# tobiashepp/torch-mednet

Hardware: AMD Instinct MI355X
Metric: 128^3 patches/sec training, 3D U-Net 32-base-ch (higher is better)
Workload: dtype bf16; 1 GPU; ResidualUNet3D f_maps=[32, 64, 128, 256] 4-class, 128^3 patches, batch 4/GPU, fwd+DiceLoss+bwd+allreduce+Adam (BASELINE config 2); global_batch=4, parallelism=dp1, graph_replay=False, gradient_exchange=none (1 rank)

## Files before the change

### include/mednet_hip.h

```cpp
#ifndef MEDNET_HIP_H
#define MEDNET_HIP_H
#include <stddef.h>
#include <stdint.h>
#ifdef __cplusplus
extern "C" {
#endif

typedef void* mednet_stream;

enum { MEDNET_F32 = 0, MEDNET_BF16 = 1,
       MEDNET_F16 = 2,
       MEDNET_U8 = 3,
       MEDNET_I64 = 4   };
enum { MEDNET_NDHWC = 0, MEDNET_NCDHW = 1 };
enum { MEDNET_ACT_NONE = 0, MEDNET_ACT_RELU = 1, MEDNET_ACT_LEAKY = 2, MEDNET_ACT_ELU = 3 };
enum { MEDNET_POOL_MAX = 0, MEDNET_POOL_AVG = 1 };
enum { MEDNET_ALGO_AUTO = 0, MEDNET_ALGO_DIRECT = 1, MEDNET_ALGO_MFMA = 2, MEDNET_ALGO_EXACT = 3,
       MEDNET_ALGO_EXACT_BIT = 4,
       MEDNET_ALGO_SPLITW_BIT = 8 };
enum { MEDNET_PACK_LOW = 0x100,
       MEDNET_PACK_HIGH_ONLY = 0x200 };
enum { MEDNET_REG_L2 = 0, MEDNET_REG_L1 = 1 };
enum { MEDNET_CLASS_DICE = 0, MEDNET_CLASS_CE = 1 };
enum {
// ... 23 lines not shown
int mednet_conv3d_pack_many(const void* table_device, int njobs, unsigned blocks, int elt_dtype, mednet_stream stream);
int mednet_conv3d_stats_plan(int n, int d, int h, int w, int cin, int cout, int dtype, int gnb, int stride, int* out13);
int mednet_conv3d_fused_stats_chunks(int n, int d, int h, int w, int cin, int cout, int ksize, int x_dtype,
                                     int y_dtype, int algo);
int mednet_conv3d_fwd(const void* x, const void* packed, const float* bias, void* y, int n, int d, int h, int w,
                      int cin, int cout, int ksize, int x_dtype, int x_layout, int y_dtype, int y_layout,
                      int dgrad, int algo, float* gn_partial, mednet_stream stream);
int mednet_conv3d_cm_supported(int cin, int cout, int ksize, int x_dtype, int y_dtype, int algo);
int mednet_conv3d_act_supported(int n, int d, int h, int w, int cin, int cout, int algo);
int mednet_conv3d_act_fwd(const void* x, const void* packed, void* y, int n, int d, int h, int w, int cin, int cout,
                          int act, int algo, float* gn_partial, int dtype, mednet_stream stream);
int mednet_conv3d_dgrad_add(const void* dy, const void* packed, const void* add, void* dx, int n, int d, int h, int w,
                            int cin, int cout, int algo, int dtype, mednet_stream stream);
int mednet_conv3d_dgrad_gn_rows(int n, int d, int h, int w, int cin, int cout, int algo);
int mednet_conv3d_dgrad_gn_rows_dt(int n, int d, int h, int w, int cin, int cout, int algo, int dtype);
int mednet_conv3d_dgrad_add_supported(int n, int d, int h, int w, int cin, int cout, int algo, int dtype);
int mednet_conv3d_dgrad_gn(const void* dy, const void* packed, const void* add, void* dx, const void* gn_y,
                           const float* gn_coef, int gn_act, float* gn_partial, int n, int d, int h, int w, int cin,
                           int cout, int algo, int dtype, mednet_stream stream);
int mednet_head_dgrad_gn_rows(int n, int d, int h, int w, int cin, int dtype);
int mednet_head_dgrad_gn(const void* dy, const void* packed, void* dx, const void* gn_y, const void* gn_z, int gn_act,
                         float* gn_partial, int n, int d, int h, int w, int cin, int cout, int dtype, mednet_stream stream);
int mednet_convt3d_dgrad_gn_rows(int n, int d, int h, int w, int cin, int cout, int dtype, int algo);
int mednet_convt3d_dgrad_gn(const void* dy, const void* packed, void* dx, const void* gn_y, const void* gn_z, int gn_act,
                            float* gn_partial, int n, int d, int h, int w, int cin, int cout, int dtype, int algo,
                            mednet_stream stream);
int mednet_pool2_bwd_gn_rows(int n, int d, int h, int w, int c, int dtype);
int mednet_pool2_bwd_gn(const void* dy, const void* x, const void* add, void* dx, const void* gn_y, int gn_act,
                        float* gn_partial, int n, int d, int h, int w, int c, int mode, int dtype, mednet_stream stream);
size_t mednet_conv3d_wgrad_ws_bytes(int n, int d, int h, int w, int cin, int cout, int ksize, int workgroups);
int mednet_conv3d_wgrad_coresident(int n, int d, int h, int w, int cin, int cout, int ksize, int x_dtype, int dy_dtype, int algo);
int mednet_conv3d_wgrad_plan(int n, int d, int h, int w, int cin, int cout, int dtype, int workgroups, int* out10);
int mednet_conv3d_wgrad_c1_gn_supported(int cout, int x_dtype, int dtype);
int mednet_conv3d_wgrad_c1_gn(const void* x, const void* dz, const void* y, const float* coef, const float* bcoef, float* dw,
                              int n, int d, int h, int w, int cout, int act, int x_dtype, int dtype, void* ws, size_t ws_bytes,
                              mednet_stream stream);
int mednet_conv3d_wgrad_cm_gn_supported(int cin, int cout, int x_dtype, int dtype);
int mednet_conv3d_wgrad_cm_plan(int n, int d, int h, int w, int cin, int cout, int dtype, int gn, int* out4);
int mednet_conv3d_wgrad_cm_gn(const void* x, int x_layout, const void* dz, const void* y, const float* coef, const float* bcoef,
                              float* dw, int n, int d, int h, int w, int cin, int cout, int act, int x_dtype, int dtype, void* ws,
                              size_t ws_bytes, mednet_stream stream);
int mednet_conv3d_wgrad(const void* x, const void* dy, float* dw, float* dbias, int n, int d, int h, int w,
                        int cin, int cout, int ksize, int x_dtype, int x_layout, int dy_dtype, int dy_layout,
                        int algo, int workgroups, void* ws, size_t ws_bytes, mednet_stream stream);

int mednet_convt3d_fwd(const void* x, const void* packed, const float* bias, const void* skip, void* y, int n,
                       int d, int h, int w, int cin, int cout, int x_dtype, int y_dtype, int algo,
                       mednet_stream stream);
int mednet_convt3d_dgrad(const void* dy, const void* packed, void* dx, int n, int d, int h, int w, int cin,
                         int cout, int dy_dtype, int dx_dtype, int algo, mednet_stream stream);
size_t mednet_convt3d_wgrad_ws_bytes(int n, int d, int h, int w, int cin, int cout, int workgroups);
int mednet_convt3d_wgrad(const void* x, const void* dy, float* dw, float* dbias, int n, int d, int h, int w,
                         int cin, int cout, int x_dtype, int dy_dtype, int algo, int workgroups, void* ws,
                         size_t ws_bytes, mednet_stream stream);

size_t mednet_gn_ws_bytes(int n, int c, size_t spatial);
int mednet_gn_stats(const void* x, const float* gamma, const float* beta, float* stats, float* coef, int n,
                    size_t spatial, int c, int groups, float eps, int dtype, void* ws, size_t ws_bytes,
                    mednet_stream stream);
int mednet_gn_finalize(const float* partial, int chunks, const float* gamma, const float* beta, float* stats,
                       float* coef, int n, size_t spatial, int c, int groups, float eps, void* ws, size_t ws_bytes,
                       mednet_stream stream);
int mednet_gn_act_fwd(const void* x, const float* coef, const void* residual, void* z, int n, size_t spatial,
                      int c, int act, int x_dtype, int z_dtype, mednet_stream stream);
int mednet_gn_act_bwd(const void* dz, const void* dz2, const void* x, const void* z, const float* coef,
                      const float* stats, const float* gamma, void* dx, void* dres, float* dgamma, float* dbeta, int n,
                      size_t spatial, int c, int groups, int act, int in_act, int dtype, void* ws, size_t ws_bytes,
                      mednet_stream stream);
int mednet_gn_act_bwd_fused(const void* dz, const void* x, const float* coef, const float* stats, const float* gamma,
                            const float* partial, int rows, void* dx, float* dgamma, float* dbeta, int n,
                            size_t spatial, int c, int groups, int act, int in_act, int dtype, void* ws, size_t ws_bytes,
                            mednet_stream stream);
int mednet_gn_bwd_coefficients(const float* stats, const float* gamma, const float* partial, int rows, float* bcoef,
                               float* dgamma, float* dbeta, int n, size_t spatial, int c, int groups, void* ws,
                               size_t ws_bytes, mednet_stream stream);
int mednet_gn_act_bwd_fused_res(const void* dz, const void* x, const void* z, const float* coef, const float* stats,
                                const float* gamma, const float* fused_partial, int rows, void* dx, void* dres,
                                float* dgamma, float* dbeta, int n, size_t spatial, int c, int groups, int act, int dtype,
                                void* ws, size_t ws_bytes, mednet_stream stream);
int mednet_gn_act_bwd_fused_res_pool(const void* dy_pool, const void* skip_grad, const void* x, const void* z, const float* stats,
                                     const float* gamma, const float* fused_partial, int rows, void* dx, void* dres, float* dgamma,
                                     float* dbeta, int n, int d, int h, int w, int c, int groups, int act, int pool_mode, int dtype,
                                     void* ws, size_t ws_bytes, mednet_stream stream);
int mednet_bn_stats(const void* x, const float* gamma, const float* beta, float* running_mean, float* running_var,
                    long long* num_batches_tracked, float momentum, float* stats, float* coef, int n, size_t spatial, int c,
                    float eps, int dtype, void* ws, size_t ws_bytes, mednet_stream stream);
int mednet_bn_eval_coef(const float* running_mean, const float* running_var, const float* gamma, const float* beta, float* stats,
                        float* coef, int n, int c, float eps, mednet_stream stream);
int mednet_bn_act_bwd(const void* dz, const void* x, const void* z, const float* coef, const float* stats, const float* gamma,
                      void* dx, void* dres, float* dgamma, float* dbeta, int n, size_t spatial, int c, int act, int in_act,
                      int frozen, int dtype, void* ws, size_t ws_bytes, mednet_stream stream);
int mednet_bn_act_bwd_fused(const void* dz, const void* x, const float* coef, const float* stats, const float* gamma,
                            const float* partial, int rows, void* dx, float* dgamma, float* dbeta, int n, size_t spatial, int c,
                            int act, int in_act, int frozen, int dtype, void* ws, size_t ws_bytes, mednet_stream stream);

int mednet_act_fwd(const void* x, void* z, size_t count, int act, int dtype, mednet_stream stream);
int mednet_act_bwd(const void* dz, const void* z, void* dx, size_t count, int act, int dtype,
                   mednet_stream stream);
int mednet_add(const void* a, const void* b, void* out, size_t count, int dtype, mednet_stream stream);

int mednet_pool2_fwd(const void* x, void* y, int n, int d, int h, int w, int c, int mode, int dtype,
                     mednet_stream stream);
int mednet_gn_act_pool_supported(int d, int h, int w, int c, int dtype);
int mednet_gn_act_pool_fwd(const void* x, const float* coef, const void* residual, void* z, void* pooled, int n, int d, int h,
                           int w, int c, int act, int mode, int dtype, mednet_stream stream);
int mednet_pool2_bwd(const void* dy, const void* x, const void* add, void* dx, int n, int d, int h, int w, int c,
                     int mode, int dtype, mednet_stream stream);
int mednet_pool2_bwd_act(const void* dy, const void* x, const void* add, int add_channels, void* dx, int n, int d, int h, int w, int c,
                         int mode, int in_act, int dtype, mednet_stream stream);

int mednet_upcat_fwd(const void* enc, const void* x, void* out, int n, int d, int h, int w, int c_enc, int xd,
                     int xh, int xw, int c_x, int dtype, mednet_stream stream);
int mednet_upcat_stats_chunks(int n, int d, int h, int w, int c_enc, int c_x, int dtype);
int mednet_upcat_fwd_stats(const void* enc, const void* x, void* out, float* partial, int n, int d, int h, int w, int c_enc, int xd,
                           int xh, int xw, int c_x, int dtype, mednet_stream stream);
int mednet_upcat_bwd(const void* dout, void* denc, void* dx, int n, int d, int h, int w, int c_enc, int xd, int xh,
                     int xw, int c_x, int dtype, mednet_stream stream);

size_t mednet_loss_ws_bytes(int n, int c, size_t spatial);
int mednet_dice_fwd(const float* logits, const int64_t* labels, const float* weight, float* loss, float* saved,
                    float* dice_out, int n, int c, size_t spatial, int64_t stride_n, int64_t stride_c, float eps,
                    int sigmoid, int ignore_index, void* ws, size_t ws_bytes, mednet_stream stream);
int mednet_dice_bwd(const float* logits, const int64_t* labels, const float* weight, const float* saved,
                    const float* dloss, float* dlogits, int n, int c, size_t spatial, int64_t stride_n,
                    int64_t stride_c, float eps, int sigmoid, int ignore_index, mednet_stream stream);
int mednet_dice_fwd_lt(const float* logits, const void* labels, int label_dtype, int64_t label_stride_n, const float* weight,
                       float* loss, float* saved, float* dice_out, int n, int c, size_t spatial, int64_t stride_n,
                       int64_t stride_c, float eps, int sigmoid, int ignore_index, void* ws, size_t ws_bytes, mednet_stream stream);
int mednet_dice_bwd_lt(const float* logits, const void* labels, int label_dtype, int64_t label_stride_n, const float* weight,
                       const float* saved, const float* dloss, float* dlogits, int n, int c, size_t spatial, int64_t stride_n,
                       int64_t stride_c, float eps, int sigmoid, int ignore_index, mednet_stream stream);
int mednet_head_dice_supported(int cin, int cout, int dtype, int label_dtype);
size_t mednet_head_dice_ws_bytes(int n, size_t spatial, int cin, int cout);
int mednet_head_dice_gn_rows(int n, size_t spatial, int cin);
int mednet_head_dice_fwd(const void* z, const void* packed, const float* bias, const void* labels, int label_dtype,
                         int64_t label_stride_n, const float* weight, float* logits, float* loss, float* saved, int n,
                         size_t spatial, int cin, int cout, float eps, int sigmoid, int ignore_index, int z_dtype, void* ws,
                         size_t ws_bytes, mednet_stream stream);
int mednet_head_dice_bwd(const float* logits, const void* labels, int label_dtype, int64_t label_stride_n, const void* packed,
                         const float* weight, const float* saved, const float* dloss, void* dz, const void* gn_y, const void* z,
                         int gn_act, float* gn_partial, float* dw, float* dbias, int n, size_t spatial, int cin, int cout,
                         float eps, int sigmoid, int ignore_index, int z_dtype, void* ws, size_t ws_bytes, mednet_stream stream);

int mednet_head_landmark_supported(int cin, int nh, int ncls, int dtype, size_t spatial);
size_t mednet_head_landmark_ws_bytes(int n, size_t spatial, int nh, int ncls);
int mednet_head_landmark_gn_rows(size_t spatial);
int mednet_head_landmark_fwd(const void* z, const void* packed, const float* bias, const void* heatmaps, int64_t heatmap_stride_n,
                             const void* labels, int64_t label_stride_n, const float* class_weight, const float* reg_weight,
                             float* logits, float* class_loss, float* reg_loss, float* saved, int n, size_t spatial, int cin, int nh,
                             int ncls, int kind, float eps, int sigmoid, int ignore_index, int z_dtype, void* ws, size_t ws_bytes,
                             mednet_stream stream);
int mednet_head_landmark_bwd(const void* z, const void* packed, const float* bias, const void* heatmaps, int64_t heatmap_stride_n,
                             const void* labels, int64_t label_stride_n, const float* class_weight, const float* reg_weight,
                             const float* saved, const float* dclass_loss, const float* dreg_loss, void* dz, const void* gn_y,
                             int gn_act, float* gn_partial, float* dw, float* dbias, int n, size_t spatial, int cin, int nh, int ncls,
                             int kind, float eps, int sigmoid, int ignore_index, int z_dtype, void* ws, size_t ws_bytes,
                             mednet_stream stream);
int mednet_head_ce_supported(int cin, int cout, int dtype, int label_dtype);
size_t mednet_head_ce_ws_bytes(int n, size_t spatial, int cin, int cout);
int mednet_head_ce_gn_rows(int n, size_t spatial, int cin);
int mednet_head_ce_fwd(const void* z, const void* packed, const float* bias, const void* labels, int label_dtype,
                       int64_t label_stride_n, const float* weight, float* logits, float* loss, float* saved, int n, size_t spatial,
                       int cin, int cout, int ignore_index, int z_dtype, void* ws, size_t ws_bytes, mednet_stream stream);
int mednet_head_ce_bwd(const float* logits, const void* labels, int label_dtype, int64_t label_stride_n, const void* packed,
                       const float* weight, const float* saved, const float* dloss, void* dz, const void* gn_y, const void* z,
                       int gn_act, float* gn_partial, float* dw, float* dbias, int n, size_t spatial, int cin, int cout,
// ... 63 lines not shown
```

### torch-mednet_amd/csrc/conv.h

```cpp
#pragma once
#include "common.h"

namespace mednet {

enum { MAP_CONV = 0, MAP_CT_FWD = 1, MAP_CT_DG = 2 };

struct ConvGeom {
  int n, od, oh, ow;
  int id, ih, iw;
  int k, m;
  int ks;
  int in_planar, out_planar;
};

struct WgradGeom {
  int n, ad, ah, aw;
  int bd, bh, bw;
  int ka, kb, ks, stride2;
  int a_planar, b_planar;
  size_t chunk;
};


template <int MAP>
int launch_direct(const void* x, const float* P, const float* bias, const void* skip, void* y, const ConvGeom& g,
                  int x_dtype, int y_dtype, hipStream_t s);
size_t wgrad_direct_ws_bytes(size_t nvox, int ka, int kb, int ks);
int launch_wgrad_direct(const void* A, const void* B, float* dw, WgradGeom g, int a_dtype, int b_dtype, void* ws,
                        size_t ws_bytes, hipStream_t s);
size_t channel_sum_ws_bytes(int n, size_t spatial, int c);
int launch_channel_sum(const void* x, float* out, int n, size_t spatial, int c, int planar, int dtype, void* ws,
                       size_t ws_bytes, hipStream_t s);
bool head_dgrad_supported(int cin, int cout, int ksize, int x_dtype, int x_layout, int y_layout);
int launch_head_dgrad(const void* dy, const float* Pb, void* dz, int n, size_t spatial, int m, int k, int out_dtype,
                      hipStream_t s);
int head_dgrad_gn_rows(size_t spatial, int k, int dtype);
int launch_head_dgrad_gn(const void* dy, const float* Pb, void* dz, const void* gy, const void* gz, int act, float* partial,
                         int n, size_t spatial, int m, int k, int dtype, hipStream_t s);
bool head_vox_supported(int k);
int launch_head_fwd_vox(const void* z, const float* Pb, const float* bias, float* y, int n, size_t spatial, int k, int m,
                        int z_dtype, hipStream_t s);
bool wgrad_1x1_supported(int cin, int cout, int ksize, int x_layout, int dy_layout, int dy_dtype);
size_t wgrad_1x1_ws_bytes(int n, size_t spatial, int cin, int cout);
int launch_wgrad_1x1(const void* z, const void* dy, float* dw, int n, size_t spatial, int cin, int cout, int z_dtype,
                     void* ws, size_t ws_bytes, hipStream_t s);
bool wgrad_c1_supported(int cin, int cout, int ksize, int x_layout, int dy_layout);
size_t wgrad_c1_ws_bytes(int n, int d, int h, int w, int cout);
bool wgrad_c1_gn_supported(int cout, int x_dtype, int dtype);
int launch_wgrad_c1_gn(const void* x, const void* dz, const void* y, const float* coef, const float* bcoef, int act, float* dw,
                       int n, int d, int h, int w, int cout, int x_dtype, int dtype, void* ws, size_t ws_bytes, hipStream_t s);
int launch_wgrad_c1(const void* x, const void* dy, float* dw, int n, int d, int h, int w, int cout, int x_dtype,
                    int dy_dtype, void* ws, size_t ws_bytes, hipStream_t s, bool split_bf16 = false);
bool wgrad_cm_supported(int cin, int cout, int ksize, int x_dtype, int dy_dtype, int dy_layout);
bool wgrad_cm_gn_supported(int cin, int cout, int x_dtype, int dtype);
size_t wgrad_cm_ws_bytes(int n, int d, int h, int w, int cin, int cout);
int wgrad_cm_plan(int n, int d, int h, int w, int cin, int cout, int dtype, bool gn, int* out4);
int launch_wgrad_cm(const void* x, int x_layout, const void* dz, const void* y, const float* coef, const float* bcoef, int act,
                    float* dw, int n, int d, int h, int w, int cin, int cout, int dtype, void* ws, size_t ws_bytes, hipStream_t s);
int launch_pack_f32(const float* w, float* Pf, float* Pb, int cin, int cout, int T, int transposed_src, hipStream_t s);

int launch_hm_finalize(const float* partial, const float* cweight, float* loss, int n, int c, int nblocks, size_t spatial,
                       hipStream_t s);
int launch_dice_finalize(const float* partial, const float* weight, float* loss, float* saved, int c, int nblocks, float eps,
                         hipStream_t s, float* dice_out = nullptr);
int launch_ce_finalize(const float* partial, float* loss, float* saved, int nblocks, hipStream_t s);

#include "conv_mfma_decl.inc"

bool conv_f32_mfma_enabled();
int launch_conv_f32_mfma(const void* x, const float* P, const float* bias, void* y, int n, int d, int h, int w, int k, int m,
                         hipStream_t s);
int launch_convt_dgrad_f32_mfma(const void* dy, const float* Pb, void* dx, int n, int d, int h, int w, int cin, int cout,
                                hipStream_t s);
int launch_convt_fwd_f32_mfma(const void* x, const float* Pf, const float* bias, const void* skip, void* y, int n, int d, int h,
                              int w, int cin, int cout, hipStream_t s);
size_t wgrad_f32_mfma_ws_bytes(int n, int d, int h, int w, int ka, int kb, int stride2);
int launch_wgrad_f32_mfma(const void* x, const void* dy, float* dw, int n, int d, int h, int w, int cin, int cout, void* ws,
                          size_t ws_bytes, hipStream_t s);
int launch_convt_wgrad_f32_mfma(const void* x, const void* dy, float* dw, int n, int d, int h, int w, int cin, int cout, void* ws,
                                size_t ws_bytes, hipStream_t s);

bool conv_x3_enabled();
bool conv_x3_supported(int cin, int cout, int ksize);
bool conv_x3_fits(int d, int h, int w, int c);
int conv_x3_stats_rows(int n, int d, int h, int w, int cout);
int launch_conv_x3(const void* x, const void* sec_hi, size_t lo_delta, const float* bias, void* y, int n, int d, int h, int w, int k,
                   int m, float* stats, hipStream_t s);
bool conv_c1_x3_supported(int cin, int cout, int ksize);
int conv_c1_x3_stats_rows(int d, int h, int w);
int launch_conv_c1_x3(const void* x, const float* w_pf, const float* bias, void* y, int n, int d, int h, int w, int cout,
                      float* stats, hipStream_t s);
int launch_conv_x3_dgrad(const void* dy, const void* sec_hi, size_t lo_delta, void* dx, int n, int d, int h, int w, int k, int m,
                         const void* add, const void* gn_y, const float* gn_coef, int gn_act, float* gn_partial, hipStream_t s);
int launch_convt_dgrad_x3(const void* dy, const void* sec_hi, size_t lo_delta, void* dx, int n, int d, int h, int w, int cin,
                          int cout, hipStream_t s);
int launch_convt_fwd_x3(const void* x, const void* sec_hi, size_t lo_delta, const float* bias, const void* skip, void* y, int n,
                        int d, int h, int w, int cin, int cout, hipStream_t s);
size_t wgrad_x3_ws_bytes(int n, int d, int h, int w, int cin, int cout, int workgroups);
bool wgrad_c1_x3_supported(int cout, int x_dtype, int dy_dtype);
int wgrad_c1_x3_blocks(int n, int d, int h, int w);
int launch_wgrad_c1_x3(const void* x, const void* dy, float* part, int n, int d, int h, int w, hipStream_t s);
int launch_wgrad_x3(const void* x, const void* dy, float* dw, int n, int d, int h, int w, int cin, int cout, void* ws,
                    size_t ws_bytes, hipStream_t s, int workgroups);

size_t convt_wgrad_x3_ws_bytes(int n, int d, int h, int w, int cin, int cout, int workgroups);
int launch_convt_wgrad_x3(const void* x, const void* dy, float* dw, int n, int d, int h, int w, int cin, int cout, void* ws,
                          size_t ws_bytes, hipStream_t s, int workgroups);

}
```

### torch-mednet_amd/csrc/head_loss.hip

```cpp
#include "common.h"
#include "conv.h"

namespace mednet {

constexpr int HL_BLOCK_VOX = 256 * 8;
constexpr int HL_MAXC = 4;
constexpr int HL_VPT = 32;

template <typename T>
struct Raw8;
template <>
struct Raw8<bf16> {
  bf16x8 r;
  __device__ __forceinline__ void load(const bf16* p, size_t i) { r = *reinterpret_cast<const bf16x8*>(p + i); }
  __device__ __forceinline__ float at(int j) const { return (float)r[j]; }
};
template <>
struct Raw8<f16> {
  f16x8 r;
  __device__ __forceinline__ void load(const f16* p, size_t i) { r = *reinterpret_cast<const f16x8*>(p + i); }
  __device__ __forceinline__ float at(int j) const { return (float)r[j]; }
};
template <>
struct Raw8<float> {
// ... 51 lines not shown
  const size_t v0 = (size_t)blockIdx.x * HL_BLOCK_VOX;
  for (int it = 0; it < 8; ++it) {
    const size_t v = v0 + (size_t)it * 256 + threadIdx.x;
    if (v < spatial) {
      float zv[K];
#pragma unroll
      for (int q = 0; q < K / 8; ++q) {
        const F8 t = ld8(z, ((size_t)n * spatial + v) * K + q * 8);
#pragma unroll
        for (int j = 0; j < 8; ++j) zv[q * 8 + j] = t.v[j];
      }
      const int yl = label_at(lab, (size_t)n * lab_sn + v);
      float lg[HL_MAXC], p[HL_MAXC];
#pragma unroll
      for (int i = 0; i < HL_MAXC; ++i) {
        lg[i] = 0.f;
        if (i < m) {
          float s0 = bias ? bias[i] : 0.f, s1 = 0.f;
#pragma unroll
          for (int j = 0; j < K; j += 2) {
            s0 = fmaf(zv[j], Pb[(size_t)i * K + j], s0);
            s1 = fmaf(zv[j + 1], Pb[(size_t)i * K + j + 1], s1);
          }
          lg[i] = s0 + s1;
          y[((size_t)n * m + i) * spatial + v] = lg[i];
        }
      }
      if constexpr (CE) {
        if (yl != ignore && (unsigned)yl >= (unsigned)m) num = __builtin_nanf("");
        if (yl != ignore && yl >= 0 && yl < m) {
          float mx = -INFINITY, zy = 0.f;
#pragma unroll
          for (int k = 0; k < HL_MAXC; ++k)
            if (k < m) {
              mx = fmaxf(mx, lg[k]);
              if (k == yl) zy = lg[k];
            }
          float s = 0.f;
#pragma unroll
          for (int k = 0; k < HL_MAXC; ++k)
            if (k < m) s += expf(lg[k] - mx);
          const float w = cw ? cw[yl] : 1.f;
          num = fmaf(w, (mx + logf(s)) - zy, num);
          den += w;
        }
        continue;
      }
      probs_reg(lg, m, sigmoid, p);
      bad |= (unsigned)yl >= (unsigned)m;
#pragma unroll
      for (int k = 0; k < HL_MAXC; ++k)
        if (k < m) {
          const float t = (k == yl) ? 1.f : 0.f;
          const float mk = (ignore != MEDNET_NO_IGNORE && t == (float)ignore) ? 0.f : 1.f;
          I[k] = fmaf(p[k] * mk, t * mk, I[k]);
          D[k] += (p[k] + t) * mk;
        }
    }
  }
  if constexpr (CE) {
    num = block_sum<4>(num, scratch);
    den = block_sum<4>(den, scratch);
    if (threadIdx.x == 0) {
      float* o = partial + ((size_t)n * gridDim.x + blockIdx.x) * 2;
      o[0] = num;
      o[1] = den;
    }
    return;
  }
  if (bad) I[0] = D[0] = __builtin_nanf("");
  float* out = partial + ((size_t)n * gridDim.x + blockIdx.x) * m * 2;
#pragma unroll
  for (int k = 0; k < HL_MAXC; ++k)
    if (k < m) {
      const float a = block_sum<4>(I[k], scratch);
      const float b = block_sum<4>(D[k], scratch);
      if (threadIdx.x == 0) {
        out[2 * k] = a;
        out[2 * k + 1] = b;
      }
    }
}

template <typename TO, int K, typename TL, bool FOLD = false, bool CE = false>
__global__ __launch_bounds__(256, (sizeof(TO) == 2 && !FOLD) ? 3 : 2) void head_dice_bwd_kernel(const float* __restrict__ lgs, const TL* __restrict__ lab, int64_t lab_sn,
                                                            const float* __restrict__ Pb , const float* __restrict__ weight,
                                                            const float* __restrict__ saved, const float* __restrict__ dloss,
                                                            float eps, int sigmoid, int ignore, TO* __restrict__ dz,
                                                            const TO* __restrict__ gy , const TO* __restrict__ gz, int act,
                                                            float* __restrict__ gn_partial , float* __restrict__ wpart,
                                                            size_t spatial, int m) {
  constexpr int CG = K / 8, VPW = 256 / CG;
  const int n = blockIdx.y;
  const int cgi = threadIdx.x % CG, vi = threadIdx.x / CG;
  float wreg[HL_MAXC][8];
#pragma unroll
  for (int i = 0; i < HL_MAXC; ++i)
#pragma unroll
    for (int j = 0; j < 8; ++j) wreg[i][j] = i < m ? Pb[(size_t)i * K + cgi * 8 + j] : 0.f;
  const float go = *dloss;
  float gI[HL_MAXC], gD[HL_MAXC];
#pragma unroll
  for (int k = 0; k < HL_MAXC; ++k) {
    gI[k] = gD[k] = 0.f;
    if (CE && k < m) {
      gI[k] = (weight ? weight[k] : 1.f) * (go / saved[0]);
    } else if (k < m) {
      const float w = weight ? weight[k] : 1.f;
      const float I = saved[2 * k], D = saved[2 * k + 1];
      const float Dc = fmaxf(D, eps);
      gI[k] = -2.f * w / ((float)m * Dc) * go + ((I != I || D != D) ? __builtin_nanf("") : 0.f);
      gD[k] = (D >= eps ? 2.f * w * I / ((float)m * Dc * Dc) : 0.f) * go;
    }
  }
  auto dlogits_of = [&](const float* lg, int yl, float* dl) {
    if constexpr (CE) {
      float p[HL_MAXC];
      probs_reg(lg, m, 0, p);
      float w = 0.f;
#pragma unroll
      for (int k = 0; k < HL_MAXC; ++k)
        if (k < m && k == yl) w = gI[k];
      w = (yl != ignore && yl >= 0 && yl < m) ? w : 0.f;
#pragma unroll
      for (int k = 0; k < HL_MAXC; ++k) dl[k] = k < m ? w * (p[k] - (k == yl ? 1.f : 0.f)) : 0.f;
      return;
    }
    float p[HL_MAXC], g[HL_MAXC];
    probs_reg(lg, m, sigmoid, p);
    float dot = 0.f;
#pragma unroll
    for (int k = 0; k < HL_MAXC; ++k)
      if (k < m) {
        const float t = (k == yl) ? 1.f : 0.f;
        const float mk = (ignore != MEDNET_NO_IGNORE && t == (float)ignore) ? 0.f : 1.f;
        g[k] = mk * (gI[k] * t * mk + gD[k]);
        dot = fmaf(p[k], g[k], dot);
      }
#pragma unroll
    for (int k = 0; k < HL_MAXC; ++k) dl[k] = k < m ? (sigmoid ? g[k] * p[k] * (1.f - p[k]) : p[k] * (g[k] - dot)) : 0.f;
  };
  float ss[8], sq[8], wacc[HL_MAXC][8], bacc[HL_MAXC];
#pragma unroll
  for (int j = 0; j < 8; ++j) ss[j] = sq[j] = 0.f;
#pragma unroll
  for (int i = 0; i < HL_MAXC; ++i) {
    bacc[i] = 0.f;
#pragma unroll
    for (int j = 0; j < 8; ++j) wacc[i][j] = 0.f;
  }
  const size_t v0 = (size_t)blockIdx.x * (VPW * HL_VPT) + vi;
  for (int it = 0; it < HL_VPT; it += 2) {
    const size_t v = v0 + (size_t)it * VPW;
    if (v >= spatial) break;
    const size_t vb = v + VPW;
    const bool hb = (it + 1 < HL_VPT) && vb < spatial;
    const size_t vbs = hb ? vb : v;
    float la[HL_MAXC], lb[HL_MAXC];
    if constexpr (CG == 4) {
      const int cq = threadIdx.x & 3;
      const float oa = cq < m ? lgs[((size_t)n * m + cq) * spatial + v] : 0.f;
      const float ob = cq < m ? lgs[((size_t)n * m + cq) * spatial + vbs] : 0.f;
      la[0] = dpp_f32<(0) | (0 << 2) | (0 << 4) | (0 << 6)>(oa);
      la[1] = dpp_f32<(1) | (1 << 2) | (1 << 4) | (1 << 6)>(oa);
      la[2] = dpp_f32<(2) | (2 << 2) | (2 << 4) | (2 << 6)>(oa);
      la[3] = dpp_f32<(3) | (3 << 2) | (3 << 4) | (3 << 6)>(oa);
      lb[0] = dpp_f32<(0) | (0 << 2) | (0 << 4) | (0 << 6)>(ob);
      lb[1] = dpp_f32<(1) | (1 << 2) | (1 << 4) | (1 << 6)>(ob);
      lb[2] = dpp_f32<(2) | (2 << 2) | (2 << 4) | (2 << 6)>(ob);
      lb[3] = dpp_f32<(3) | (3 << 2) | (3 << 4) | (3 << 6)>(ob);
      static_assert(HL_MAXC == 4, "one class per lane of a quad");
    } else {
#pragma unroll
      for (int i = 0; i < HL_MAXC; ++i) {
        la[i] = i < m ? lgs[((size_t)n * m + i) * spatial + v] : 0.f;
        lb[i] = i < m ? lgs[((size_t)n * m + i) * spatial + vbs] : 0.f;
      }
    }
    const int ya = label_at(lab, (size_t)n * lab_sn + v), yb = label_at(lab, (size_t)n * lab_sn + vbs);
    const size_t rowa = ((size_t)n * spatial + v) * K + cgi * 8, rowb = ((size_t)n * spatial + vbs) * K + cgi * 8;
    Raw8<TO> zva, zvb, yva, yvb;
    zva.load(gz, rowa);
    zvb.load(gz, rowb);
    if (gy) {
      yva.load(gy, rowa);
      yvb.load(gy, rowb);
    } else {
      yva = zva;
      yvb = zvb;
    }
    float da[HL_MAXC], db[HL_MAXC];
    dlogits_of(la, ya, da);
    dlogits_of(lb, yb, db);
    if (!hb) {
#pragma unroll
      for (int i = 0; i < HL_MAXC; ++i) db[i] = 0.f;
    }
    F8 t, u;
#pragma unroll
    for (int j = 0; j < 8; ++j) t.v[j] = u.v[j] = 0.f;
#pragma unroll
    for (int i = 0; i < HL_MAXC; ++i) {
      if (i < m) {
#pragma unroll
        for (int j = 0; j < 8; ++j) {
          t.v[j] = fmaf(da[i], wreg[i][j], t.v[j]);
          u.v[j] = fmaf(db[i], wreg[i][j], u.v[j]);
          wacc[i][j] = fmaf(db[i], zvb.at(j), fmaf(da[i], zva.at(j), wacc[i][j]));
        }
        bacc[i] += da[i] + db[i];
      }
    }
#pragma unroll
    for (int j = 0; j < 8; ++j) {
      t.v[j] = (float)(TO)t.v[j];
      u.v[j] = (float)(TO)u.v[j];
    }
    if constexpr (FOLD) {
      float za[8], zb[8];
#pragma unroll
      for (int j = 0; j < 8; ++j) {
        za[j] = zva.at(j);
        zb[j] = zvb.at(j);
      }
      act_grad_n<8>(t.v, za, act);
      act_grad_n<8>(u.v, zb, act);
    }
    st8(dz, rowa, t);
    if (hb) st8(dz, rowb, u);
    if (!FOLD && gy) {
      float za[8], zb[8];
#pragma unroll
      for (int j = 0; j < 8; ++j) {
        za[j] = zva.at(j);
        zb[j] = zvb.at(j);
      }
      act_grad_n<8>(t.v, za, act);
      act_grad_n<8>(u.v, zb, act);
#pragma unroll
      for (int j = 0; j < 8; ++j) {
        ss[j] += t.v[j] + u.v[j];
        sq[j] = fmaf(u.v[j], yvb.at(j), fmaf(t.v[j], yva.at(j), sq[j]));
      }
    }
  }
  const int lane = threadIdx.x & 63, wave = threadIdx.x >> 6;
  const size_t wrow = ((size_t)n * gridDim.x + blockIdx.x) * 4 + wave;
  if (gn_partial) {
    float* out = gn_partial + wrow * K * 2 + cgi * 16;
#pragma unroll
    for (int j = 0; j < 8; ++j) {
      const float a = lane_class_sum<CG>(ss[j]), b = lane_class_sum<CG>(sq[j]);
      if (lane < CG) {
        out[2 * j] = a;
        out[2 * j + 1] = b;
      }
    }
  }
  float* wout = wpart + wrow * ((size_t)m * K + m);
#pragma unroll
  for (int i = 0; i < HL_MAXC; ++i) {
    if (i < m) {
#pragma unroll
      for (int j = 0; j < 8; ++j) {
        const float a = lane_class_sum<CG>(wacc[i][j]);
        if (lane < CG) wout[(size_t)i * K + cgi * 8 + j] = a;
      }
      const float b = lane_class_sum<CG>(bacc[i]);
      if (lane == 0) wout[(size_t)m * K + i] = b;
    }
  }
}

constexpr int HL_WF_GROUPS = 128;
__global__ __launch_bounds__(192) void head_dice_wfinal1_kernel(const float* __restrict__ wpart, double* __restrict__ part2, int rows,
                                                                int width) {
  const int per = (rows + HL_WF_GROUPS - 1) / HL_WF_GROUPS;
  const int r0 = blockIdx.x * per, r1 = r0 + per < rows ? r0 + per : rows;
  for (int e = threadIdx.x; e < width; e += 192) {
    double s0 = 0.0, s1 = 0.0, s2 = 0.0, s3 = 0.0;
    int r = r0;
    for (; r + 3 < r1; r += 4) {
      s0 += (double)wpart[(size_t)r * width + e];
      s1 += (double)wpart[(size_t)(r + 1) * width + e];
      s2 += (double)wpart[(size_t)(r + 2) * width + e];
      s3 += (double)wpart[(size_t)(r + 3) * width + e];
    }
    for (; r < r1; ++r) s0 += (double)wpart[(size_t)r * width + e];
    part2[(size_t)blockIdx.x * width + e] = (s0 + s1) + (s2 + s3);
  }
}
__global__ __launch_bounds__(192) void head_dice_wfinal2_kernel(const double* __restrict__ part2, float* __restrict__ dw,
                                                                float* __restrict__ dbias, int width, int mk) {
  for (int e = threadIdx.x; e < width; e += 192) {
    double s = 0.0;
    for (int g = 0; g < HL_WF_GROUPS; ++g) s += part2[(size_t)g * width + e];
    if (e < mk) dw[e] = (float)s;
    else if (dbias) dbias[e - mk] = (float)s;
  }
}

__global__ void dice_finalize_kernel(const float* __restrict__ partial, const float* __restrict__ weight, float* __restrict__ loss,
                                     float* __restrict__ saved, float* __restrict__ dice_out, int c, int nblocks, float eps);

static inline unsigned hl_fwd_blocks(size_t spatial) { return (unsigned)((spatial + HL_BLOCK_VOX - 1) / HL_BLOCK_VOX); }
static inline unsigned hl_bwd_blocks(size_t spatial, int k) {
  const size_t per_wg = (size_t)(256 / (k / 8)) * HL_VPT;
  return (unsigned)((spatial + per_wg - 1) / per_wg);
}

}

using namespace mednet;

extern "C" int mednet_head_dice_supported(int cin, int cout, int dtype, int label_dtype) {
  return (cin == 16 || cin == 32 || cin == 64) && cout >= 1 && cout <= HL_MAXC && dtype_ok(dtype) &&
         (label_dtype == MEDNET_U8 || label_dtype == MEDNET_I64) && tuning_option("head_loss_fuse", 1);
}
extern "C" size_t mednet_head_dice_ws_bytes(int n, size_t spatial, int cin, int cout) {
  const size_t fwd = ((size_t)n * hl_fwd_blocks(spatial) * cout * 2 + 64) * sizeof(float);
  const size_t width = (size_t)cout * cin + cout;
  const size_t bwd = ((size_t)n * hl_bwd_blocks(spatial, cin) * 4 * width + 64) * sizeof(float) + (size_t)HL_WF_GROUPS * width * sizeof(double) + 16;
  return fwd > bwd ? fwd : bwd;
}
extern "C" int mednet_head_dice_gn_rows(int n, size_t spatial, int cin) {
  (void)n;
  return 4 * (int)hl_bwd_blocks(spatial, cin);
}

template <bool CE>
static int head_loss_fwd(const char* what, const void* z, const void* packed, const float* bias, const void* labels, int label_dtype,
                         int64_t label_stride_n, const float* weight, float* logits, float* loss, float* saved, int n, size_t spatial,
                         int cin, int cout, float eps, int sigmoid, int ignore_index, int z_dtype, void* ws, size_t ws_bytes,
                         mednet_stream stream) {
  MEDNET_REQUIRE(mednet_head_dice_supported(cin, cout, z_dtype, label_dtype), MEDNET_E_UNSUPPORTED,
                 "%s: %d -> %d classes, dtype %d, labels %d", what, cin, cout, z_dtype, label_dtype);
  MEDNET_REQUIRE(n > 0 && spatial > 0 && z && packed && labels && logits && loss && saved, MEDNET_E_SHAPE, "%s: bad arguments", what);
  MEDNET_REQUIRE(ws_bytes >= mednet_head_dice_ws_bytes(n, spatial, cin, cout), MEDNET_E_WORKSPACE, "%s: workspace too small", what);
  const PackLayout L = pack_layout(cin, cout, 1);
  const float* Pb = (const float*)((const char*)packed + L.f32_bwd);
  hipStream_t s = (hipStream_t)stream;
  const unsigned nb = hl_fwd_blocks(spatial);
  float* partial = (float*)ws;
  const dim3 grid(nb, n);
#define HF(TI_, K_, TL_) hipLaunchKernelGGL((head_dice_fwd_kernel<TI_, K_, TL_, CE>), grid, dim3(256), 0, s, (const TI_*)z, Pb, bias, (const TL_*)labels, label_stride_n, logits, partial, spatial, cout, sigmoid, ignore_index, CE ? weight : nullptr)
#define HF_L(TI_, K_) do { if (label_dtype == MEDNET_U8) HF(TI_, K_, uint8_t); else HF(TI_, K_, int64_t); } while (0)
#define HF_K(TI_) do { if (cin == 16) HF_L(TI_, 16); else if (cin == 32) HF_L(TI_, 32); else HF_L(TI_, 64); } while (0)
  if (z_dtype == MEDNET_F32) HF_K(float);
  else if (z_dtype == MEDNET_BF16) HF_K(bf16);
  else HF_K(f16);
#undef HF_K
#undef HF_L
#undef HF
  int rc = check_launch(what);
  if (rc) return rc;
  if (CE) return launch_ce_finalize(partial, loss, saved, (int)(nb * n), s);
  hipLaunchKernelGGL(dice_finalize_kernel, dim3(1), dim3(256), 0, s, partial, weight, loss, saved, (float*)nullptr, cout, (int)(nb * n), eps);
  return check_launch("dice_finalize");
}

template <bool CE>
static int head_loss_bwd(const char* what, const float* logits, const void* labels, int label_dtype, int64_t label_stride_n,
                         const void* packed, const float* weight, const float* saved, const float* dloss, void* dz, const void* gn_y,
                         const void* z, int gn_act, float* gn_partial, float* dw, float* dbias, int n, size_t spatial, int cin, int cout,
                         float eps, int sigmoid, int ignore_index, int z_dtype, void* ws, size_t ws_bytes, mednet_stream stream) {
  MEDNET_REQUIRE(mednet_head_dice_supported(cin, cout, z_dtype, label_dtype), MEDNET_E_UNSUPPORTED,
                 "%s: %d -> %d classes, dtype %d, labels %d", what, cin, cout, z_dtype, label_dtype);
  MEDNET_REQUIRE(n > 0 && spatial > 0 && logits && labels && packed && saved && dloss && dz && z && dw, MEDNET_E_SHAPE, "%s: bad arguments", what);
  MEDNET_REQUIRE((gn_y == nullptr) == (gn_partial == nullptr), MEDNET_E_SHAPE, "%s: gn_y and gn_partial go together", what);
  MEDNET_REQUIRE(ws_bytes >= mednet_head_dice_ws_bytes(n, spatial, cin, cout), MEDNET_E_WORKSPACE, "%s: workspace too small", what);
  const PackLayout L = pack_layout(cin, cout, 1);
  const float* Pb = (const float*)((const char*)packed + L.f32_bwd);
  hipStream_t s = (hipStream_t)stream;
  const unsigned nb = hl_bwd_blocks(spatial, cin);
  float* wpart = (float*)ws;
  const dim3 grid(nb, n);
  const bool fold = gn_y == nullptr && gn_act != MEDNET_ACT_NONE;
#define HB_(TO_, K_, TL_, F_) hipLaunchKernelGGL((head_dice_bwd_kernel<TO_, K_, TL_, F_, CE>), grid, dim3(256), 0, s, logits, (const TL_*)labels, label_stride_n, Pb, weight, saved, dloss, eps, sigmoid, ignore_index, (TO_*)dz, (const TO_*)gn_y, (const TO_*)z, gn_act, gn_partial, wpart, spatial, cout)
#define HB(TO_, K_, TL_) do { if (fold) HB_(TO_, K_, TL_, true); else HB_(TO_, K_, TL_, false); } while (0)
#define HB_L(TO_, K_) do { if (label_dtype == MEDNET_U8) HB(TO_, K_, uint8_t); else HB(TO_, K_, int64_t); } while (0)
#define HB_K(TO_) do { if (cin == 16) HB_L(TO_, 16); else if (cin == 32) HB_L(TO_, 32); else HB_L(TO_, 64); } while (0)
  if (z_dtype == MEDNET_F32) HB_K(float);
  else if (z_dtype == MEDNET_BF16) HB_K(bf16);
  else HB_K(f16);
#undef HB_K
#undef HB_L
#undef HB_
#undef HB
  int rc = check_launch(what);
  if (rc) return rc;
  const int width = cout * cin + cout, rows = (int)(n * nb * 4);
  double* part2 = (double*)((char*)ws + (((size_t)rows * width + 64) * sizeof(float) + 7) / 8 * 8);
  hipLaunchKernelGGL(head_dice_wfinal1_kernel, dim3(HL_WF_GROUPS), dim3(192), 0, s, wpart, part2, rows, width);
  hipLaunchKernelGGL(head_dice_wfinal2_kernel, dim3(1), dim3(192), 0, s, part2, dw, dbias, width, cout * cin);
  return check_launch("head_dice_wfinal");
}

extern "C" int mednet_head_dice_fwd(const void* z, const void* packed, const float* bias, const void* labels, int label_dtype,
                                    int64_t label_stride_n, const float* weight, float* logits, float* loss, float* saved, int n,
                                    size_t spatial, int cin, int cout, float eps, int sigmoid, int ignore_index, int z_dtype,
                                    void* ws, size_t ws_bytes, mednet_stream stream) {
  return head_loss_fwd<false>("head_dice_fwd", z, packed, bias, labels, label_dtype, label_stride_n, weight, logits, loss, saved, n, spatial,
                              cin, cout, eps, sigmoid, ignore_index, z_dtype, ws, ws_bytes, stream);
}

extern "C" int mednet_head_dice_bwd(const float* logits, const void* labels, int label_dtype, int64_t label_stride_n,
                                    const void* packed, const float* weight, const float* saved, const float* dloss, void* dz,
                                    const void* gn_y, const void* z, int gn_act, float* gn_partial, float* dw, float* dbias, int n,
                                    size_t spatial, int cin, int cout, float eps, int sigmoid, int ignore_index, int z_dtype,
                                    void* ws, size_t ws_bytes, mednet_stream stream) {
  return head_loss_bwd<false>("head_dice_bwd", logits, labels, label_dtype, label_stride_n, packed, weight, saved, dloss, dz, gn_y, z, gn_act,
                              gn_partial, dw, dbias, n, spatial, cin, cout, eps, sigmoid, ignore_index, z_dtype, ws, ws_bytes, stream);
}

extern "C" int mednet_head_ce_supported(int cin, int cout, int dtype, int label_dtype) {
  return mednet_head_dice_supported(cin, cout, dtype, label_dtype);
}
extern "C" size_t mednet_head_ce_ws_bytes(int n, size_t spatial, int cin, int cout) {
  return mednet_head_dice_ws_bytes(n, spatial, cin, cout);
}
extern "C" int mednet_head_ce_gn_rows(int n, size_t spatial, int cin) { return mednet_head_dice_gn_rows(n, spatial, cin); }

extern "C" int mednet_head_ce_fwd(const void* z, const void* packed, const float* bias, const void* labels, int label_dtype,
                                  int64_t label_stride_n, const float* weight, float* logits, float* loss, float* saved, int n,
                                  size_t spatial, int cin, int cout, int ignore_index, int z_dtype, void* ws, size_t ws_bytes,
                                  mednet_stream stream) {
  return head_loss_fwd<true>("head_ce_fwd", z, packed, bias, labels, label_dtype, label_stride_n, weight, logits, loss, saved, n, spatial,
                             cin, cout, 0.f, 0, ignore_index, z_dtype, ws, ws_bytes, stream);
}

extern "C" int mednet_head_ce_bwd(const float* logits, const void* labels, int label_dtype, int64_t label_stride_n, const void* packed,
                                  const float* weight, const float* saved, const float* dloss, void* dz, const void* gn_y, const void* z,
                                  int gn_act, float* gn_partial, float* dw, float* dbias, int n, size_t spatial, int cin, int cout,
                                  int ignore_index, int z_dtype, void* ws, size_t ws_bytes, mednet_stream stream) {
  return head_loss_bwd<true>("head_ce_bwd", logits, labels, label_dtype, label_stride_n, packed, weight, saved, dloss, dz, gn_y, z, gn_act,
                             gn_partial, dw, dbias, n, spatial, cin, cout, 0.f, 0, ignore_index, z_dtype, ws, ws_bytes, stream);
}
```

### torch-mednet_amd/csrc/norm_act.hip

```cpp
#include "common.h"

#ifndef GN_NT
#define GN_NT 1
#endif
#ifndef GN_WAVES
#define GN_WAVES 3
#endif
namespace mednet {

template <int VEC>
struct Cols {
  int cols, rows, col, row;
  bool active;
  __device__ __forceinline__ Cols(int c) {
    cols = c / VEC;
    rows = 256 / cols;
    active = (int)threadIdx.x < rows * cols;
    col = threadIdx.x % cols;
    row = threadIdx.x / cols;
  }
};

template <typename T, int VEC>
struct VecIO;
template <typename T>
struct VecIO<T, 8> {
  static __device__ __forceinline__ F8 load(const T* p, size_t i) { return ld8(p, i); }
  static __device__ __forceinline__ F8 load_last(const T* p, size_t i) { return GN_NT ? ld8_nt(p, i) : ld8(p, i); }
  static __device__ __forceinline__ void store(T* p, size_t i, const F8& v) { st8(p, i, v); }
};
template <>
struct VecIO<float, 4> {
  static __device__ __forceinline__ F8 load(const float* p, size_t i) {
    F8 r;
    const f32x4 a = *reinterpret_cast<const f32x4*>(p + i);
#pragma unroll
    for (int k = 0; k < 4; ++k) r.v[k] = a[k];
    return r;
  }
  static __device__ __forceinline__ F8 load_last(const float* p, size_t i) {
    F8 r;
    const f32x4 a = GN_NT ? __builtin_nontemporal_load(reinterpret_cast<const f32x4*>(p + i)) : *reinterpret_cast<const f32x4*>(p + i);
#pragma unroll
    for (int k = 0; k < 4; ++k) r.v[k] = a[k];
    return r;
  }
  static __device__ __forceinline__ void store(float* p, size_t i, const F8& v) {
    const f32x4 a = {v.v[0], v.v[1], v.v[2], v.v[3]};
    *reinterpret_cast<f32x4*>(p + i) = a;
  }
};
template <typename T>
struct VecIO<T, 1> {
  static __device__ __forceinline__ F8 load(const T* p, size_t i) {
    F8 r;
    r.v[0] = ld(p, i);
    return r;
  }
  static __device__ __forceinline__ F8 load_last(const T* p, size_t i) { return load(p, i); }
  static __device__ __forceinline__ void store(T* p, size_t i, const F8& v) { st(p, i, v.v[0]); }
};

static inline void chunk_plan(size_t spatial, int c, int vec, size_t& chunk_vox, unsigned& chunks) {
  const int cols = c / vec;
  const int rows = 256 / cols;
  size_t cv = (spatial + 1023) / 1024;
  if (cv < (size_t)rows * 8) cv = (size_t)rows * 8;
  cv = (cv + rows - 1) / rows * rows;
  chunk_vox = cv;
  chunks = (unsigned)((spatial + cv - 1) / cv);
}

template <int NVAL>
__device__ __forceinline__ void column_reduce(const float* vals, int cols, int rows, int col, int row, bool active,
                                              float* lds, float* out) {
  __syncthreads();
  if (active) {
#pragma unroll
    for (int k = 0; k < NVAL; ++k) lds[(row * cols + col) * NVAL + k] = vals[k];
  }
  __syncthreads();
  if (active && row == 0) {
#pragma unroll
// ... 338 lines not shown
  const float k3 = (float)((rstd * rstd * s2 * mean - rstd * s1) / count);
  for (int i = threadIdx.x; i < cg; i += 64) {
    const int cc = g * cg + i;
    float* o = bcoef + ((size_t)n * c + cc) * 3;
    o[0] = (float)rstd * (gamma ? gamma[cc] : 1.f);
    o[1] = k2;
    o[2] = k3;
  }
}
template <bool DUX>
__global__ __launch_bounds__(256) void gn_bwd_reduce_finalize_kernel(const float* __restrict__ partial, const float* __restrict__ stats,
                                                                     const float* __restrict__ gamma, float* __restrict__ csum,
                                                                     float* __restrict__ bcoef, int c, int groups, int rows,
                                                                     double count) {
  __shared__ double sha[256], shb[256];
  const int n = blockIdx.x / groups, g = blockIdx.x % groups;
  const int cg = c / groups, t = threadIdx.x;
  const int i = t % cg, r0 = t / cg, rstep = 256 / cg;
  const float* base = partial + (size_t)n * rows * c * 2 + (size_t)(g * cg + i) * 2;
  const size_t rs = (size_t)c * 2;
  constexpr int U = 16;
  double a[U], b[U];
#pragma unroll
  for (int k = 0; k < U; ++k) a[k] = b[k] = 0.0;
  int r = r0;
  for (; r + (U - 1) * rstep < rows; r += U * rstep) {
    float2 p[U];
#pragma unroll
    for (int k = 0; k < U; ++k) p[k] = *reinterpret_cast<const float2*>(base + (size_t)(r + k * rstep) * rs);
#pragma unroll
    for (int k = 0; k < U; ++k) {
      a[k] += (double)p[k].x;
      b[k] += (double)p[k].y;
    }
  }
  for (; r < rows; r += rstep) {
    const float2 p0 = *reinterpret_cast<const float2*>(base + (size_t)r * rs);
    a[0] += (double)p0.x;
    b[0] += (double)p0.y;
  }
#pragma unroll
  for (int w = 1; w < U; w *= 2) {
#pragma unroll
    for (int k = 0; k < U; k += 2 * w) {
      a[k] += a[k + w];
      b[k] += b[k + w];
    }
  }
  sha[t] = a[0];
  shb[t] = b[0];
  __syncthreads();
  const double mean = stats[((size_t)n * groups + g) * 2], rstd = stats[((size_t)n * groups + g) * 2 + 1];
  if (t < cg) {
    double a = 0.0, b = 0.0;
    for (int k = 0; k < rstep; ++k) {
      a += sha[k * cg + t];
      b += shb[k * cg + t];
    }
    if (DUX) b = rstd * (b - mean * a);
    const float af = (float)a, bf = (float)b;
    csum[((size_t)n * c + g * cg + t) * 2] = af;
    csum[((size_t)n * c + g * cg + t) * 2 + 1] = bf;
    const double ga = gamma ? (double)gamma[g * cg + t] : 1.0;
    sha[t] = ga * (double)af;
    shb[t] = ga * (double)bf;
  }
  __syncthreads();
  if (t < cg) {
    double s1 = 0.0, s2 = 0.0;
    for (int k = 0; k < cg; ++k) {
      s1 += sha[k];
      s2 += shb[k];
    }
    float* o = bcoef + ((size_t)n * c + g * cg + t) * 3;
    o[0] = (float)rstd * (gamma ? gamma[g * cg + t] : 1.f);
    o[1] = (float)(-rstd * rstd * s2 / count);
    o[2] = (float)((rstd * rstd * s2 * mean - rstd * s1) / count);
  }
}
static bool gn_bwd_one_launch(int c, int groups) {
  const int cg = c / groups;
  return cg >= 1 && cg <= 256 && 256 % cg == 0 && tuning_option("gn_bwd_one_launch", 1);
}
struct GnParamGrad {
  const float* csum = nullptr;
  float* dgamma = nullptr;
  float* dbeta = nullptr;
  int n = 0;
};
__global__ __launch_bounds__(256) void gn_bwd_params_kernel(const float* __restrict__ csum, float* __restrict__ dgamma,
                                                            float* __restrict__ dbeta, int n, int c) {
  const int cc = blockIdx.x * 256 + threadIdx.x;
  if (cc >= c) return;
  double a = 0.0, b = 0.0;
  for (int i = 0; i < n; ++i) {
    a += (double)csum[((size_t)i * c + cc) * 2];
    b += (double)csum[((size_t)i * c + cc) * 2 + 1];
  }
  if (dbeta) dbeta[cc] = (float)a;
  if (dgamma) dgamma[cc] = (float)b;
}
template <typename T, int VEC>
__global__ __launch_bounds__(256, GN_WAVES) void gn_bwd_apply_kernel(const T* __restrict__ dz, const T* __restrict__ dz2,
                                                           const T* __restrict__ x, const T* __restrict__ z,
                                                           const float* __restrict__ coef,
                                                           const float* __restrict__ bcoef, T* __restrict__ dx,
                                                           T* __restrict__ dres, size_t spatial, int c, int act,
                                                           size_t chunk_vox, int in_act, GnParamGrad pg) {
  if (pg.csum && blockIdx.x == 0 && blockIdx.y == 0) {
    for (int cc = threadIdx.x; cc < c; cc += 256) {
      double a = 0.0, b = 0.0;
      for (int i = 0; i < pg.n; ++i) {
        a += (double)pg.csum[((size_t)i * c + cc) * 2];
        b += (double)pg.csum[((size_t)i * c + cc) * 2 + 1];
      }
      if (pg.dbeta) pg.dbeta[cc] = (float)a;
      if (pg.dgamma) pg.dgamma[cc] = (float)b;
    }
  }
  const Cols<VEC> L(c);
  if (!L.active) return;
  const int n = blockIdx.y;
  const size_t v0 = (size_t)blockIdx.x * chunk_vox;
  const size_t v1 = v0 + chunk_vox < spatial ? v0 + chunk_vox : spatial;
  float k1[VEC], k2[VEC], k3[VEC], ca[VEC], cb[VEC];
#pragma unroll
  for (int k = 0; k < VEC; ++k) {
    const float* o = bcoef + ((size_t)n * c + L.col * VEC + k) * 3;
    k1[k] = o[0];
    k2[k] = o[1];
    k3[k] = o[2];
    ca[k] = z ? 0.f : coef[((size_t)n * c + L.col * VEC + k) * 2];
    cb[k] = z ? 0.f : coef[((size_t)n * c + L.col * VEC + k) * 2 + 1];
  }
  const size_t off = (size_t)n * spatial * c + (size_t)L.col * VEC;
  auto one = [&](size_t i) {
    F8 g1 = VecIO<T, VEC>::load_last(dz, i);
    F8 g2, zv;
    if (dz2) g2 = VecIO<T, VEC>::load_last(dz2, i);
    if (act != MEDNET_ACT_NONE && z) zv = VecIO<T, VEC>::load(z, i);
    const F8 xv = VecIO<T, VEC>::load_last(x, i);
    if (dz2) {
#pragma unroll
      for (int k = 0; k < VEC; ++k) g1.v[k] += g2.v[k];
    }
    if (z) {
      act_grad_n<VEC>(g1.v, zv.v, act);
    } else {
#pragma unroll
      for (int k = 0; k < VEC; ++k) zv.v[k] = fmaf(ca[k], xv.v[k], cb[k]);
      act_grad_pre_n<VEC>(g1.v, zv.v, act);
    }
    F8 o;
#pragma unroll
    for (int k = 0; k < VEC; ++k) o.v[k] = fmaf(k1[k], g1.v[k], fmaf(k2[k], xv.v[k], k3[k]));
    if (in_act != MEDNET_ACT_NONE) act_grad_n<VEC>(o.v, xv.v, in_act);
    VecIO<T, VEC>::store(dx, i, o);
    if (dres) VecIO<T, VEC>::store(dres, i, g1);
  };
  size_t v = v0 + L.row;
  for (; v + (size_t)L.rows < v1; v += 2 * (size_t)L.rows) {
    one(off + v * c);
    one(off + (v + L.rows) * c);
  }
  for (; v < v1; v += L.rows) one(off + v * c);
}

template <typename T>
__global__ __launch_bounds__(256) void act_fwd_kernel(const T* __restrict__ x, T* __restrict__ z, size_t count, int act) {
  const size_t stride = (size_t)gridDim.x * 256 * 8;
  for (size_t i = ((size_t)blockIdx.x * 256 + threadIdx.x) * 8; i < count; i += stride) {
    if (i + 8 <= count) {
      F8 v = ld8(x, i);
#pragma unroll
      for (int k = 0; k < 8; ++k) v.v[k] = act_apply(v.v[k], act);
      st8(z, i, v);
    } else {
      for (size_t j = i; j < count; ++j) st(z, j, act_apply(ld(x, j), act));
    }
  }
}
template <typename T>
__global__ __launch_bounds__(256) void act_bwd_kernel(const T* __restrict__ dz, const T* __restrict__ z,
                                                      T* __restrict__ dx, size_t count, int act) {
  const size_t stride = (size_t)gridDim.x * 256 * 8;
  for (size_t i = ((size_t)blockIdx.x * 256 + threadIdx.x) * 8; i < count; i += stride) {
    if (i + 8 <= count) {
      F8 g = ld8(dz, i);
      const F8 zv = ld8(z, i);
#pragma unroll
      for (int k = 0; k < 8; ++k) g.v[k] *= act_grad_from_out(zv.v[k], act);
      st8(dx, i, g);
    } else {
      for (size_t j = i; j < count; ++j) st(dx, j, ld(dz, j) * act_grad_from_out(ld(z, j), act));
    }
  }
}
template <typename T>
__global__ __launch_bounds__(256) void add_kernel(const T* __restrict__ a, const T* __restrict__ b, T* __restrict__ o,
                                                  size_t count) {
  const size_t stride = (size_t)gridDim.x * 256 * 8;
  for (size_t i = ((size_t)blockIdx.x * 256 + threadIdx.x) * 8; i < count; i += stride) {
// ... 167 lines not shown
    }
    VecIO<T, VEC>::store(dx, dst, o);
  }
}

constexpr int POOL_GN_PV = 4;
template <typename T>
__global__ __launch_bounds__(256) void pool2_bwd_gn_kernel(const T* __restrict__ dy, const T* __restrict__ x,
                                                           const T* __restrict__ add, T* __restrict__ dx,
                                                           const T* __restrict__ gy, float* __restrict__ partial, int d,
                                                           int h, int w, int c, int mode, int act) {
  constexpr int VEC = 8;
  const int od = d / 2, oh = h / 2, ow = w / 2, cv = c / VEC;
  const size_t per = (size_t)od * oh * ow * cv;
  const int nn = blockIdx.y;
  const int cc = (int)(threadIdx.x % cv);
  float acc[2 * VEC];
#pragma unroll
  for (int k = 0; k < 2 * VEC; ++k) acc[k] = 0.f;
  for (int it = 0; it < POOL_GN_PV; ++it) {
    const size_t i = ((size_t)blockIdx.x * POOL_GN_PV + it) * 256 + threadIdx.x;
    if (i >= per) break;
    size_t v = i / cv;
    const int ox = (int)(v % ow);
    v /= ow;
    const int oy = (int)(v % oh);
    const int oz = (int)(v / oh);
    const F8 g = VecIO<T, VEC>::load(dy, ((size_t)nn * per + i) * VEC);
    F8 xv[8];
    int arg[VEC];
    float best[VEC];
#pragma unroll
    for (int k = 0; k < VEC; ++k) {
      best[k] = -INFINITY;
      arg[k] = 0;
    }
#pragma unroll
    for (int t = 0; t < 8; ++t) {
      const int iz = 2 * oz + (t >> 2), iy = 2 * oy + ((t >> 1) & 1), ix = 2 * ox + (t & 1);
      const size_t src = ((((size_t)nn * d + iz) * h + iy) * w + ix) * c + (size_t)cc * VEC;
      xv[t] = VecIO<T, VEC>::load(x, src);
#pragma unroll
      for (int k = 0; k < VEC; ++k) {
        if (xv[t].v[k] > best[k] || xv[t].v[k] != xv[t].v[k]) {
          best[k] = xv[t].v[k];
          arg[k] = t;
        }
      }
    }
#pragma unroll
    for (int t = 0; t < 8; ++t) {
      const int iz = 2 * oz + (t >> 2), iy = 2 * oy + ((t >> 1) & 1), ix = 2 * ox + (t & 1);
      const size_t dst = ((((size_t)nn * d + iz) * h + iy) * w + ix) * c + (size_t)cc * VEC;
      F8 o;
#pragma unroll
      for (int k = 0; k < VEC; ++k) o.v[k] = mode == MEDNET_POOL_MAX ? (arg[k] == t ? g.v[k] : 0.f) : 0.125f * g.v[k];
      if (add) {
        const F8 a = VecIO<T, VEC>::load(add, dst);
#pragma unroll
        for (int k = 0; k < VEC; ++k) o.v[k] += a.v[k];
      }
#pragma unroll
      for (int k = 0; k < VEC; ++k) o.v[k] = (float)(T)o.v[k];
      if (dx) VecIO<T, VEC>::store(dx, dst, o);
      const F8 yv = VecIO<T, VEC>::load(gy, dst);
      act_grad_n<VEC>(o.v, xv[t].v, act);
#pragma unroll
      for (int k = 0; k < VEC; ++k) {
        acc[2 * k] += o.v[k];
        acc[2 * k + 1] = fmaf(o.v[k], yv.v[k], acc[2 * k + 1]);
      }
    }
  }
  float* out = partial + (((size_t)nn * gridDim.x + blockIdx.x) * 4) * c * 2;
  column_reduce_lds_free<2 * VEC>(acc, cv, cc, true, out, c * 2);
}

template <typename T, int VEC>
__global__ __launch_bounds__(256) void gn_bwd_apply_pool_kernel(const T* __restrict__ dyp, const T* __restrict__ add,
                                                                const T* __restrict__ x, const T* __restrict__ z,
                                                                const float* __restrict__ bcoef, T* __restrict__ dx,
                                                                T* __restrict__ dres, int n, int d, int h, int w, int c, int act,
                                                                int mode, GnParamGrad pg) {
  if (pg.csum && blockIdx.x == 0) {
    for (int cc = threadIdx.x; cc < c; cc += 256) {
      double a = 0.0, b = 0.0;
      for (int i = 0; i < pg.n; ++i) {
        a += (double)pg.csum[((size_t)i * c + cc) * 2];
        b += (double)pg.csum[((size_t)i * c + cc) * 2 + 1];
      }
      if (pg.dbeta) pg.dbeta[cc] = (float)a;
      if (pg.dgamma) pg.dgamma[cc] = (float)b;
    }
  }
  const int od = d / 2, oh = h / 2, ow = w / 2, cv = c / VEC;
  const size_t total = (size_t)n * od * oh * ow * cv;
  const size_t i = (size_t)blockIdx.x * 256 + threadIdx.x;
  if (i >= total) return;
  const int cc = (int)(i % cv);
  size_t v = i / cv;
  const int ox = (int)(v % ow);
  v /= ow;
  const int oy = (int)(v % oh);
  v /= oh;
  const int oz = (int)(v % od);
  const int nn = (int)(v / od);
  float k1[VEC], k2[VEC], k3[VEC];
#pragma unroll
  for (int k = 0; k < VEC; ++k) {
    const float* o = bcoef + ((size_t)nn * c + cc * VEC + k) * 3;
    k1[k] = o[0];
    k2[k] = o[1];
    k3[k] = o[2];
  }
  const F8 g = VecIO<T, VEC>::load(dyp, i * VEC);
  size_t src[8];
  F8 zv[8];
#pragma unroll
  for (int t = 0; t < 8; ++t) {
    const int iz = 2 * oz + (t >> 2), iy = 2 * oy + ((t >> 1) & 1), ix = 2 * ox + (t & 1);
    src[t] = ((((size_t)nn * d + iz) * h + iy) * w + ix) * c + (size_t)cc * VEC;
    zv[t] = VecIO<T, VEC>::load(z, src[t]);
  }
  int arg[VEC];
  float best[VEC];
#pragma unroll
  for (int k = 0; k < VEC; ++k) {
    best[k] = -INFINITY;
    arg[k] = 0;
  }
#pragma unroll
  for (int t = 0; t < 8; ++t)
#pragma unroll
    for (int k = 0; k < VEC; ++k)
      if (zv[t].v[k] > best[k] || zv[t].v[k] != zv[t].v[k]) {
        best[k] = zv[t].v[k];
        arg[k] = t;
      }
#pragma unroll
  for (int t = 0; t < 8; ++t) {
    const F8 xv = VecIO<T, VEC>::load(x, src[t]);
    F8 g1;
#pragma unroll
    for (int k = 0; k < VEC; ++k) g1.v[k] = mode == MEDNET_POOL_MAX ? (arg[k] == t ? g.v[k] : 0.f) : 0.125f * g.v[k];
    if (add) {
      const F8 a = VecIO<T, VEC>::load(add, src[t]);
#pragma unroll
      for (int k = 0; k < VEC; ++k) g1.v[k] += a.v[k];
    }
#pragma unroll
    for (int k = 0; k < VEC; ++k) g1.v[k] = (float)(T)g1.v[k];
    act_grad_n<VEC>(g1.v, zv[t].v, act);
    F8 o;
#pragma unroll
    for (int k = 0; k < VEC; ++k) {
      float xf = xv.v[k];
      if (sizeof(T) == 2) asm volatile("" : "+v"(xf));
      o.v[k] = fmaf(k1[k], g1.v[k], fmaf(k2[k], xf, k3[k]));
      if (sizeof(T) == 2) asm volatile("" : "+v"(o.v[k]));
    }
    VecIO<T, VEC>::store(dx, src[t], o);
    VecIO<T, VEC>::store(dres, src[t], g1);
  }
}

__device__ __forceinline__ int nearest_src(int dst, int in, int out) {
  const float scale = (float)in / (float)out;
  const int s = (int)floorf((float)dst * scale);
  return s < in - 1 ? s : in - 1;
}
template <typename T, int VEC>
__global__ __launch_bounds__(256) void upcat_fwd_kernel(const T* __restrict__ enc, const T* __restrict__ x,
                                                        T* __restrict__ out, int n, int d, int h, int w, int ce, int xd,
                                                        int xh, int xw, int cx) {
  const int ct = ce + cx, pv = ct / VEC;
  const size_t total = (size_t)n * d * h * w * pv;
  const size_t i = (size_t)blockIdx.x * 256 + threadIdx.x;
// ... 336 lines not shown
  unsigned chunks;
  chunk_plan(spatial, c, vec, cv, chunks);
  float* bcoef = (float*)ws + (size_t)n * gn_partial_rows_max(c) * c * 2;
  float* csum = bcoef + (size_t)n * c * 3;
  hipStream_t s = (hipStream_t)stream;
  const int skip = tuning_option("gn_bwd_skip", 0);
  GnParamGrad pg;
  int rc;
  if (gn_bwd_one_launch(c, groups) && !skip) {
    hipLaunchKernelGGL(gn_bwd_reduce_finalize_kernel<true>, dim3(n * groups), dim3(256), 0, s, fused_partial, stats, gamma, csum, bcoef,
                       c, groups, rows, (double)spatial * (c / groups));
    rc = check_launch("gn_bwd_reduce_finalize");
    if (rc) return rc;
    if (dgamma || dbeta) pg = GnParamGrad{csum, dgamma, dbeta, n};
  } else {
    if (!(skip & 1))
      hipLaunchKernelGGL(reduce_partials_dux_kernel, dim3(n * c), dim3(64), 0, s, fused_partial, stats, csum, c, groups, rows);
    if (!(skip & 2))
      hipLaunchKernelGGL(gn_bwd_finalize_kernel, dim3(n * groups), dim3(64), 0, s, csum, stats, gamma, bcoef, c, groups,
                         (double)spatial * (c / groups));
    rc = check_launch("gn_bwd_finalize");
    if (rc) return rc;
    if (skip & 8) return MEDNET_OK;
    if ((dgamma || dbeta) && !(skip & 4)) {
      hipLaunchKernelGGL(gn_bwd_params_kernel, dim3((c + 255) / 256), dim3(256), 0, s, csum, dgamma, dbeta, n, c);
      rc = check_launch("gn_bwd_params");
      if (rc) return rc;
    }
  }
  const dim3 grid(chunks, n);
#define GO(T, V) hipLaunchKernelGGL((gn_bwd_apply_kernel<T, V>), grid, dim3(256), 0, s, (const T*)dz, (const T*)nullptr, (const T*)x, (const T*)z, coef, bcoef, (T*)dx, (T*)dres, spatial, c, act, cv, in_act, pg)
  if (dtype == MEDNET_F32) { if (vec == 4) GO(float, 4); else if (vec == 8) GO(float, 8); else GO(float, 1); }
  else if (dtype == MEDNET_BF16) { if (vec == 8) GO(bf16, 8); else GO(bf16, 1); }
  else { if (vec == 8) GO(f16, 8); else GO(f16, 1); }
#undef GO
  return check_launch("gn_bwd_apply");
}

extern "C" int mednet_gn_act_bwd_fused(const void* dz, const void* x, const float* coef, const float* stats,
                                       const float* gamma, const float* fused_partial, int rows, void* dx, float* dgamma,
                                       float* dbeta, int n, size_t spatial, int c, int groups, int act, int in_act, int dtype,
                                       void* ws, size_t ws_bytes, mednet_stream stream) {
  return gn_act_bwd_fused_impl(dz, x, nullptr, coef, stats, gamma, fused_partial, rows, dx, nullptr, dgamma, dbeta, n, spatial, c,
                               groups, act, in_act, dtype, ws, ws_bytes, stream);
}
extern "C" int mednet_gn_bwd_coefficients(const float* stats, const float* gamma, const float* fused_partial, int rows,
                                          float* bcoef, float* dgamma, float* dbeta, int n, size_t spatial, int c, int groups,
                                          void* ws, size_t ws_bytes, mednet_stream stream) {
  MEDNET_REQUIRE(c % groups == 0 && rows > 0 && fused_partial && bcoef && stats && gamma, MEDNET_E_SHAPE,
                 "gn_bwd_coefficients: bad arguments");
  MEDNET_REQUIRE(ws_bytes >= mednet_gn_ws_bytes(n, c, spatial), MEDNET_E_WORKSPACE, "gn_bwd_coefficients: workspace too small");
  float* csum = (float*)ws;
  hipStream_t s = (hipStream_t)stream;
  int rc;
  if (gn_bwd_one_launch(c, groups)) {
    hipLaunchKernelGGL(gn_bwd_reduce_finalize_kernel<true>, dim3(n * groups), dim3(256), 0, s, fused_partial, stats, gamma, csum, bcoef,
                       c, groups, rows, (double)spatial * (c / groups));
    rc = check_launch("gn_bwd_reduce_finalize");
    if (rc) return rc;
  } else {
    hipLaunchKernelGGL(reduce_partials_dux_kernel, dim3(n * c), dim3(64), 0, s, fused_partial, stats, csum, c, groups, rows);
    hipLaunchKernelGGL(gn_bwd_finalize_kernel, dim3(n * groups), dim3(64), 0, s, csum, stats, gamma, bcoef, c, groups,
                       (double)spatial * (c / groups));
    rc = check_launch("gn_bwd_finalize");
    if (rc) return rc;
  }
  if (dgamma || dbeta) {
    hipLaunchKernelGGL(gn_bwd_params_kernel, dim3((c + 255) / 256), dim3(256), 0, s, csum, dgamma, dbeta, n, c);
    rc = check_launch("gn_bwd_params");
    if (rc) return rc;
  }
  return MEDNET_OK;
}

extern "C" int mednet_gn_act_bwd_fused_res(const void* dz, const void* x, const void* z, const float* coef, const float* stats,
                                           const float* gamma, const float* fused_partial, int rows, void* dx, void* dres,
                                           float* dgamma, float* dbeta, int n, size_t spatial, int c, int groups, int act,
                                           int dtype, void* ws, size_t ws_bytes, mednet_stream stream) {
  MEDNET_REQUIRE(z && dres, MEDNET_E_SHAPE, "gn_act_bwd_fused_res: z and dres are required");
  return gn_act_bwd_fused_impl(dz, x, z, coef, stats, gamma, fused_partial, rows, dx, dres, dgamma, dbeta, n, spatial, c, groups,
                               act, MEDNET_ACT_NONE, dtype, ws, ws_bytes, stream);
}

extern "C" int mednet_gn_act_bwd_fused_res_pool(const void* dy_pool, const void* skip_grad, const void* x, const void* z,
                                                const float* stats, const float* gamma, const float* fused_partial, int rows,
                                                void* dx, void* dres, float* dgamma, float* dbeta, int n, int d, int h, int w, int c,
                                                int groups, int act, int pool_mode, int dtype, void* ws, size_t ws_bytes,
                                                mednet_stream stream) {
  MEDNET_REQUIRE(dtype_ok(dtype), MEDNET_E_DTYPE, "gn_act_bwd_fused_res_pool: bad dtype");
  MEDNET_REQUIRE(c % groups == 0 && rows > 0 && fused_partial && dy_pool && x && z && dx && dres, MEDNET_E_SHAPE,
                 "gn_act_bwd_fused_res_pool: bad arguments");
  MEDNET_REQUIRE(d % 2 == 0 && h % 2 == 0 && w % 2 == 0 && c % 8 == 0, MEDNET_E_UNSUPPORTED,
                 "gn_act_bwd_fused_res_pool: even extents and C %% 8 == 0 (%dx%dx%d, C=%d)", d, h, w, c);
  const size_t spatial = (size_t)d * h * w;
  MEDNET_REQUIRE(ws_bytes >= mednet_gn_ws_bytes(n, c, spatial), MEDNET_E_WORKSPACE, "gn_act_bwd_fused_res_pool: workspace too small");
  float* bcoef = (float*)ws + (size_t)n * gn_partial_rows_max(c) * c * 2;
  float* csum = bcoef + (size_t)n * c * 3;
  hipStream_t s = (hipStream_t)stream;
  GnParamGrad pg;
  int rc;
  if (gn_bwd_one_launch(c, groups)) {
    hipLaunchKernelGGL(gn_bwd_reduce_finalize_kernel<true>, dim3(n * groups), dim3(256), 0, s, fused_partial, stats, gamma, csum, bcoef,
                       c, groups, rows, (double)spatial * (c / groups));
    rc = check_launch("gn_bwd_reduce_finalize");
    if (rc) return rc;
    if (dgamma || dbeta) pg = GnParamGrad{csum, dgamma, dbeta, n};
  } else {
    hipLaunchKernelGGL(reduce_partials_dux_kernel, dim3(n * c), dim3(64), 0, s, fused_partial, stats, csum, c, groups, rows);
    hipLaunchKernelGGL(gn_bwd_finalize_kernel, dim3(n * groups), dim3(64), 0, s, csum, stats, gamma, bcoef, c, groups,
                       (double)spatial * (c / groups));
    rc = check_launch("gn_bwd_finalize");
    if (rc) return rc;
    if (dgamma || dbeta) {
      hipLaunchKernelGGL(gn_bwd_params_kernel, dim3((c + 255) / 256), dim3(256), 0, s, csum, dgamma, dbeta, n, c);
      rc = check_launch("gn_bwd_params");
      if (rc) return rc;
    }
  }
  const int vec = dtype == MEDNET_F32 ? 4 : 8;
  const size_t total = (size_t)n * (d / 2) * (h / 2) * (w / 2) * (c / vec);
  const dim3 grid((unsigned)((total + 255) / 256));
#define GO(T, V) hipLaunchKernelGGL((gn_bwd_apply_pool_kernel<T, V>), grid, dim3(256), 0, s, (const T*)dy_pool, (const T*)skip_grad, (const T*)x, (const T*)z, bcoef, (T*)dx, (T*)dres, n, d, h, w, c, act, pool_mode, pg)
  if (dtype == MEDNET_F32) GO(float, 4);
  else if (dtype == MEDNET_BF16) GO(bf16, 8);
  else GO(f16, 8);
#undef GO
  return check_launch("gn_bwd_apply_pool");
}


namespace mednet {
constexpr int BN_NT = 1024;
__device__ __forceinline__ void bn_column_sums(const float* __restrict__ partial, int rows, int c, int c0, int cw, double* sha,
                                               double* shb, double& ra, double& rb) {
  const int t = threadIdx.x, i = t % cw, r0 = t / cw, rstep = BN_NT / cw;
  const float* base = partial + (size_t)(c0 + i) * 2;
  const size_t rs = (size_t)c * 2;
  constexpr int U = 8;
  double a[U], b[U];
#pragma unroll
  for (int k = 0; k < U; ++k) a[k] = b[k] = 0.0;
  int r = r0;
  for (; r + (U - 1) * rstep < rows; r += U * rstep) {
    float2 p[U];
#pragma unroll
    for (int k = 0; k < U; ++k) p[k] = *reinterpret_cast<const float2*>(base + (size_t)(r + k * rstep) * rs);
#pragma unroll
    for (int k = 0; k < U; ++k) {
      a[k] += (double)p[k].x;
      b[k] += (double)p[k].y;
    }
  }
  for (; r < rows; r += rstep) {
    const float2 p0 = *reinterpret_cast<const float2*>(base + (size_t)r * rs);
    a[0] += (double)p0.x;
    b[0] += (double)p0.y;
  }
#pragma unroll
  for (int w = 1; w < U; w *= 2) {
#pragma unroll
    for (int k = 0; k < U; k += 2 * w) {
      a[k] += a[k + w];
      b[k] += b[k + w];
    }
  }
  sha[t] = a[0];
  shb[t] = b[0];
  __syncthreads();
  ra = rb = 0.0;
  if (t < cw) {
    for (int k = 0; k < rstep; ++k) {
      ra += sha[k * cw + t];
      rb += shb[k * cw + t];
    }
  }
}
static inline int bn_cw(int c) { return c % 4 == 0 ? 4 : 1; }

__global__ __launch_bounds__(BN_NT) void bn_finalize_kernel(const float* __restrict__ partial, const float* __restrict__ gamma,
                                                            const float* __restrict__ beta, float* __restrict__ running_mean,
                                                            float* __restrict__ running_var, long long* __restrict__ num_batches,
                                                            float* __restrict__ stats, float* __restrict__ coef, int n, int c,
                                                            int cw, int rows, double count, float eps, float momentum) {
  __shared__ double sha[BN_NT], shb[BN_NT];
  const int c0 = blockIdx.x * cw, t = threadIdx.x;
  double s, q;
  bn_column_sums(partial, rows, c, c0, cw, sha, shb, s, q);
  if (t < cw) {
    const int cc = c0 + t;
    const double mean = s / count;
    double var = q / count - mean * mean;
    if (var < 0.0) var = 0.0;
    const float rstd = (float)(1.0 / sqrt(var + (double)eps));
    const float ga = gamma ? gamma[cc] : 1.f, be = beta ? beta[cc] : 0.f;
    const float a = ga * rstd, b = be - (float)mean * a;
    for (int i = 0; i < n; ++i) {
      stats[((size_t)i * c + cc) * 2] = (float)mean;
      stats[((size_t)i * c + cc) * 2 + 1] = rstd;
      coef[((size_t)i * c + cc) * 2] = a;
      coef[((size_t)i * c + cc) * 2 + 1] = b;
    }
// ... 369 lines not shown
```

### torch-mednet_amd/mednet_hip/_lib.py

```python
from __future__ import annotations

import ctypes as C
import os

import torch

_HERE = os.path.dirname(os.path.abspath(__file__))
LIB_PATH = os.environ.get("MEDNET_LIB_PATH") or os.path.join(_HERE, "libmednet_hip.so")

F32, BF16 = 0, 1
NDHWC, NCDHW = 0, 1
ACT_NONE, ACT_RELU, ACT_LEAKY, ACT_ELU = 0, 1, 2, 3
POOL_MAX, POOL_AVG = 0, 1
ALGO_AUTO, ALGO_DIRECT, ALGO_MFMA, ALGO_EXACT = 0, 1, 2, 3
ALGO_EXACT_BIT = 4
ALGO_SPLITW_BIT = 8
PACK_LOW = 0x100
PACK_HIGH_ONLY = 0x200
REG_L2, REG_L1 = 0, 1
CLASS_DICE, CLASS_CE = 0, 1
PAD_CONSTANT, PAD_SYMMETRIC = 0, 1
MIP_MEAN, MIP_MAX = 0, 1
F16, U8, I64 = 2, 3, 4
NO_IGNORE = -(2 ** 31)

_vp, _i, _sz, _f, _i64 = C.c_void_p, C.c_int, C.c_size_t, C.c_float, C.c_int64

SIGNATURES = {
    "mednet_abi_version": (_i, []),
    "mednet_last_error": (C.c_char_p, []),
    "mednet_device_ok": (_i, []),
    "mednet_set_option": (_i, [C.c_char_p, _i]),
    "mednet_get_option": (_i, [C.c_char_p, _i]),
    "mednet_conv3d_pack_bytes": (_sz, [_i, _i, _i]),
    "mednet_conv3d_pack": (_i, [_vp, _vp, _i, _i, _i, _i, _vp]),
    "mednet_conv3d_pack_elt": (_i, [_vp, _vp, _i, _i, _i, _i, _i, _vp]),
    "mednet_conv3d_pack_table_bytes": (_sz, [_i]),
    "mednet_conv3d_pack_table": (_i, [_vp, _i, _vp, _vp]),
    "mednet_conv3d_pack_many": (_i, [_vp, _i, C.c_uint, _i, _vp]),
    "mednet_conv3d_stats_plan": (_i, [_i] * 9 + [_vp]),
    "mednet_conv3d_fused_stats_chunks": (_i, [_i] * 10),
    "mednet_conv3d_fwd": (_i, [_vp, _vp, _vp, _vp] + [_i] * 13 + [_vp, _vp]),
    "mednet_gn_finalize": (_i, [_vp, _i, _vp, _vp, _vp, _vp, _i, _sz, _i, _i, _f, _vp, _sz, _vp]),
    "mednet_conv3d_act_supported": (_i, [_i] * 7),
    "mednet_conv3d_act_fwd": (_i, [_vp, _vp, _vp] + [_i] * 8 + [_vp, _i, _vp]),
    "mednet_conv3d_dgrad_add": (_i, [_vp, _vp, _vp, _vp] + [_i] * 8 + [_vp]),
    "mednet_conv3d_dgrad_gn_rows": (_i, [_i] * 7),
    "mednet_conv3d_dgrad_gn_rows_dt": (_i, [_i] * 8),
    "mednet_conv3d_dgrad_add_supported": (_i, [_i] * 8),
    "mednet_conv3d_dgrad_gn": (_i, [_vp, _vp, _vp, _vp, _vp, _vp, _i, _vp] + [_i] * 8 + [_vp]),
    "mednet_gn_act_bwd_fused": (_i, [_vp] * 6 + [_i, _vp, _vp, _vp, _i, _sz, _i, _i, _i, _i, _i, _vp, _sz, _vp]),
    "mednet_gn_bwd_coefficients": (_i, [_vp, _vp, _vp, _i, _vp, _vp, _vp, _i, _sz, _i, _i, _vp, _sz, _vp]),
    "mednet_gn_act_bwd_fused_res": (_i, [_vp] * 7 + [_i, _vp, _vp, _vp, _vp, _i, _sz, _i, _i, _i, _i, _vp, _sz, _vp]),
    "mednet_gn_act_bwd_fused_res_pool": (_i, [_vp] * 7 + [_i, _vp, _vp, _vp, _vp] + [_i] * 9 + [_vp, _sz, _vp]),
    "mednet_head_dgrad_gn_rows": (_i, [_i] * 6),
    "mednet_head_dgrad_gn": (_i, [_vp] * 5 + [_i, _vp] + [_i] * 7 + [_vp]),
    "mednet_pool2_bwd_gn_rows": (_i, [_i] * 6),
    "mednet_convt3d_dgrad_gn_rows": (_i, [_i] * 8),
    "mednet_convt3d_dgrad_gn": (_i, [_vp] * 5 + [_i, _vp] + [_i] * 8 + [_vp]),
    "mednet_pool2_bwd_gn": (_i, [_vp] * 5 + [_i, _vp] + [_i] * 7 + [_vp]),
    "mednet_conv3d_wgrad_ws_bytes": (_sz, [_i] * 8),
    "mednet_conv3d_wgrad_coresident": (_i, [_i] * 10),
    "mednet_conv3d_wgrad_plan": (_i, [_i] * 8 + [_vp]),
    "mednet_conv3d_wgrad_c1_gn_supported": (_i, [_i] * 3),
    "mednet_conv3d_wgrad_c1_gn": (_i, [_vp] * 6 + [_i] * 8 + [_vp, _sz, _vp]),
    "mednet_conv3d_cm_supported": (_i, [_i] * 6),
    "mednet_conv3d_wgrad_cm_gn_supported": (_i, [_i] * 4),
    "mednet_conv3d_wgrad_cm_plan": (_i, [_i] * 8 + [_vp]),
    "mednet_conv3d_wgrad_cm_gn": (_i, [_vp, _i] + [_vp] * 5 + [_i] * 9 + [_vp, _sz, _vp]),
    "mednet_conv3d_wgrad": (_i, [_vp, _vp, _vp, _vp] + [_i] * 13 + [_vp, _sz, _vp]),
    "mednet_convt3d_fwd": (_i, [_vp, _vp, _vp, _vp, _vp] + [_i] * 9 + [_vp]),
    "mednet_convt3d_dgrad": (_i, [_vp, _vp, _vp] + [_i] * 9 + [_vp]),
    "mednet_convt3d_wgrad_ws_bytes": (_sz, [_i] * 7),
    "mednet_convt3d_wgrad": (_i, [_vp, _vp, _vp, _vp] + [_i] * 10 + [_vp, _sz, _vp]),
    "mednet_gn_ws_bytes": (_sz, [_i, _i, _sz]),
    "mednet_gn_stats": (_i, [_vp, _vp, _vp, _vp, _vp, _i, _sz, _i, _i, _f, _i, _vp, _sz, _vp]),
    "mednet_gn_act_fwd": (_i, [_vp, _vp, _vp, _vp, _i, _sz, _i, _i, _i, _i, _vp]),
    "mednet_gn_act_bwd": (_i, [_vp] * 11 + [_i, _sz, _i, _i, _i, _i, _i, _vp, _sz, _vp]),
    "mednet_act_fwd": (_i, [_vp, _vp, _sz, _i, _i, _vp]),
    "mednet_act_bwd": (_i, [_vp, _vp, _vp, _sz, _i, _i, _vp]),
    "mednet_add": (_i, [_vp, _vp, _vp, _sz, _i, _vp]),
    "mednet_pool2_fwd": (_i, [_vp, _vp] + [_i] * 7 + [_vp]),
    "mednet_bn_stats": (_i, [_vp] * 6 + [_f, _vp, _vp, _i, _sz, _i, _f, _i, _vp, _sz, _vp]),
    "mednet_bn_eval_coef": (_i, [_vp] * 6 + [_i, _i, _f, _vp]),
    "mednet_bn_act_bwd": (_i, [_vp] * 10 + [_i, _sz, _i, _i, _i, _i, _i, _vp, _sz, _vp]),
    "mednet_bn_act_bwd_fused": (_i, [_vp] * 6 + [_i, _vp, _vp, _vp, _i, _sz, _i, _i, _i, _i, _i, _vp, _sz, _vp]),
    "mednet_gn_act_pool_supported": (_i, [_i] * 5),
    "mednet_gn_act_pool_fwd": (_i, [_vp] * 5 + [_i] * 8 + [_vp]),
    "mednet_pool2_bwd": (_i, [_vp, _vp, _vp, _vp] + [_i] * 7 + [_vp]),
    "mednet_pool2_bwd_act": (_i, [_vp, _vp, _vp, _i, _vp] + [_i] * 8 + [_vp]),
    "mednet_upcat_fwd": (_i, [_vp, _vp, _vp] + [_i] * 10 + [_vp]),
    "mednet_upcat_stats_chunks": (_i, [_i] * 7),
    "mednet_upcat_fwd_stats": (_i, [_vp, _vp, _vp, _vp] + [_i] * 10 + [_vp]),
    "mednet_upcat_bwd": (_i, [_vp, _vp, _vp] + [_i] * 10 + [_vp]),
    "mednet_loss_ws_bytes": (_sz, [_i, _i, _sz]),
    "mednet_dice_fwd": (_i, [_vp] * 6 + [_i, _i, _sz, _i64, _i64, _f, _i, _i, _vp, _sz, _vp]),
    "mednet_dice_bwd": (_i, [_vp] * 6 + [_i, _i, _sz, _i64, _i64, _f, _i, _i, _vp]),
    "mednet_head_landmark_supported": (_i, [_i, _i, _i, _i, _sz]),
    "mednet_head_landmark_ws_bytes": (_sz, [_i, _sz, _i, _i]),
    "mednet_head_landmark_gn_rows": (_i, [_sz]),
    "mednet_head_landmark_fwd": (_i, [_vp, _vp, _vp, _vp, _i64, _vp, _i64] + [_vp] * 6 + [_i, _sz, _i, _i, _i, _i, _f, _i, _i, _i,
                                      _vp, _sz, _vp]),
    "mednet_head_landmark_bwd": (_i, [_vp, _vp, _vp, _vp, _i64, _vp, _i64] + [_vp] * 7 + [_i, _vp, _vp, _vp, _i, _sz, _i, _i, _i,
                                      _i, _f, _i, _i, _i, _vp, _sz, _vp]),
    "mednet_head_landmark_cls_fwd": (_i, [_vp, _vp, _vp, _vp, _i64, _vp, _i64] + [_vp] * 7 + [_i, _sz, _i, _i, _i, _i, _i, _f, _i,
                                          _i, _i, _vp, _sz, _vp]),
    "mednet_head_landmark_cls_bwd": (_i, [_vp, _vp, _vp, _vp, _i64, _vp, _i64] + [_vp] * 7 + [_i, _vp, _vp, _vp, _i, _sz, _i, _i,
                                          _i, _i, _i, _f, _i, _i, _i, _vp, _sz, _vp]),
    "mednet_head_ce_supported": (_i, [_i] * 4),
    "mednet_head_ce_ws_bytes": (_sz, [_i, _sz, _i, _i]),
    "mednet_head_ce_gn_rows": (_i, [_i, _sz, _i]),
    "mednet_head_ce_fwd": (_i, [_vp] * 4 + [_i, _i64, _vp, _vp, _vp, _vp, _i, _sz, _i, _i, _i, _i, _vp, _sz, _vp]),
    "mednet_head_ce_bwd": (_i, [_vp, _vp, _i, _i64] + [_vp] * 7 + [_i, _vp, _vp, _vp, _i, _sz, _i, _i, _i, _i, _vp, _sz, _vp]),
    "mednet_head_dice_supported": (_i, [_i] * 4),
    "mednet_head_dice_ws_bytes": (_sz, [_i, _sz, _i, _i]),
    "mednet_head_dice_gn_rows": (_i, [_i, _sz, _i]),
    "mednet_head_dice_fwd": (_i, [_vp] * 4 + [_i, _i64, _vp, _vp, _vp, _vp, _i, _sz, _i, _i, _f, _i, _i, _i, _vp, _sz, _vp]),
    "mednet_head_dice_bwd": (_i, [_vp, _vp, _i, _i64] + [_vp] * 7 + [_i, _vp, _vp, _vp, _i, _sz, _i, _i, _f, _i, _i, _i, _vp, _sz, _vp]),
    "mednet_dice_fwd_lt": (_i, [_vp, _vp, _i, _i64] + [_vp] * 4 + [_i, _i, _sz, _i64, _i64, _f, _i, _i, _vp, _sz, _vp]),
    "mednet_dice_bwd_lt": (_i, [_vp, _vp, _i, _i64] + [_vp] * 4 + [_i, _i, _sz, _i64, _i64, _f, _i, _i, _vp]),
    "mednet_heatmap_loss_fwd_strided": (_i, [_vp, _vp, _i64, _vp, _vp] + [_i, _i, _sz, _i64, _i64, _i, _i, _vp, _sz, _vp]),
    "mednet_heatmap_loss_bwd_strided": (_i, [_vp, _vp, _i64, _vp, _vp, _vp] + [_i, _i, _sz, _i64, _i64, _i, _i, _vp]),
    "mednet_ce_fwd": (_i, [_vp] * 5 + [_i, _i, _sz, _i64, _i64, _i, _vp, _sz, _vp]),
    "mednet_ce_bwd": (_i, [_vp] * 6 + [_i, _i, _sz, _i64, _i64, _i, _vp]),
    "mednet_heatmap_loss_fwd": (_i, [_vp] * 4 + [_i, _i, _sz, _i64, _i64, _i, _i, _vp, _sz, _vp]),
    "mednet_heatmap_loss_bwd": (_i, [_vp] * 5 + [_i, _i, _sz, _i64, _i64, _i, _i, _vp]),
    "mednet_adam_step": (_i, [_vp, _vp, _vp, _vp, _sz, _f, _f, _f, _f, _f, _i, _f, _vp]),
    "mednet_adam_step_scaled": (_i, [_vp, _vp, _vp, _vp, _sz, _f, _f, _f, _f, _f, _f, _vp, _f, _f, _i, _vp]),
    "mednet_grid_gather": (_i, [_vp, _vp, _vp] + [_i] * 12 + [_vp]),
    "mednet_predict_assemble": (_i, [_vp, _vp, _vp] + [_i] * 15 + [_vp]),
    "mednet_crop_patches": (_i, [_vp, _i, _vp, _vp, _i, _vp] + [_i] * 10 + [_vp]),
    "mednet_augment_ws_bytes": (_sz, [_i, _i, _sz]),
    "mednet_augment_patches": (_i, [_vp, _vp, _i, _i, _sz, _vp, _sz, _vp]),
    "mednet_sample_panels_ws_bytes": (_sz, [_i] * 5),
    "mednet_sample_panels": (_i, [_vp, _i64, _i, _i, _vp, _i, _vp, _i, _vp] + [_vp] * 5 + [_i] * 5 + [_vp, _sz, _vp]),
}

# ... 68 lines not shown
```

### torch-mednet_amd/mednet_hip/block.py

```python
from __future__ import annotations

import torch
from torch.autograd import Function

import os

from . import _lib as L
from . import config, debug, ops

ENABLED = os.environ.get("MEDNET_BLOCK_NODE", "1") == "1"
WGRAD_FIRST = os.environ.get("MEDNET_WGRAD_FIRST", "1") == "1"


def _conv_fwd(x, packed, cout, want_stats, x_layout=L.NDHWC):
    n, cin, d, h, w = x.shape
    lib = L.lib()
    y = ops.empty_cl(n, cout, d, h, w, config.act_dtype(), x.device)
    partial = None
    if want_stats:
        chunks = lib.mednet_conv3d_fused_stats_chunks(n, d, h, w, cin, cout, 3, L.dt(x), L.dt(y), config.conv_algo())
        if chunks > 0:
            partial = torch.empty((n, chunks, cout, 2), dtype=torch.float32, device=x.device)
    with ops.profiled_conv(3, cin, cout, n, d, h, w):
        L.check(lib.mednet_conv3d_fwd(x.data_ptr(), packed.data_ptr(), None, y.data_ptr(), n, d, h, w, cin, cout, 3, L.dt(x),
                                      x_layout, L.dt(y), L.NDHWC, 0, config.conv_algo(), L.ptr(partial), L.stream()), "conv3d_fwd")
    return y, partial


FUSE_POOL = os.environ.get("MEDNET_FUSE_POOL", "1") == "1"


def _gn_fwd(y, partial, gamma, beta, groups, eps, act, residual, pool_mode=None):
    n, c, d, h, w = y.shape
    spatial = d * h * w
    lib = L.lib()
    stats = torch.empty((n, groups, 2), dtype=torch.float32, device=y.device)
    coef = torch.empty((n, c, 2), dtype=torch.float32, device=y.device)
    ws = L.workspace(lib.mednet_gn_ws_bytes(n, c, spatial), y.device)
    if partial is not None:
        L.check(lib.mednet_gn_finalize(partial.data_ptr(), partial.shape[1], gamma.data_ptr(), beta.data_ptr(), stats.data_ptr(),
                                       coef.data_ptr(), n, spatial, c, groups, eps, ws.data_ptr(), ws.numel(), L.stream()),
                "gn_finalize")
    else:
        L.check(lib.mednet_gn_stats(y.data_ptr(), gamma.data_ptr(), beta.data_ptr(), stats.data_ptr(), coef.data_ptr(), n,
                                    spatial, c, groups, eps, L.dt(y), ws.data_ptr(), ws.numel(), L.stream()), "gn_stats")
    z = torch.empty_like(y, memory_format=ops.CL)
    if pool_mode is not None and FUSE_POOL and lib.mednet_gn_act_pool_supported(d, h, w, c, L.dt(y)):
        pooled = ops.empty_cl(n, c, d // 2, h // 2, w // 2, y.dtype, y.device)
        L.check(lib.mednet_gn_act_pool_fwd(y.data_ptr(), coef.data_ptr(), L.ptr(residual), z.data_ptr(), pooled.data_ptr(), n, d, h, w,
                                           c, act, pool_mode, L.dt(y), L.stream()), "gn_act_pool_fwd")
        return z, stats, coef, pooled
    L.check(lib.mednet_gn_act_fwd(y.data_ptr(), coef.data_ptr(), L.ptr(residual), z.data_ptr(), n, spatial, c, act, L.dt(y),
                                  L.dt(z), L.stream()), "gn_act_fwd")
    return (z, stats, coef, None) if pool_mode is not None else (z, stats, coef)


def _gn_bwd(dz, dz2, y, z, coef, stats, gamma_p, beta_p, groups, act, want_dres, partial=None, lazy=None):
    n, c, d, h, w = y.shape
    spatial = d * h * w
    lib = L.lib()
    dy = torch.empty_like(y, memory_format=ops.CL)
    dres = torch.empty_like(y, memory_format=ops.CL) if want_dres else None
    dgamma, dg_direct = ops._grad_target(gamma_p, (c,))
    dbeta, db_direct = ops._grad_target(beta_p, (c,))
    ws = L.workspace(lib.mednet_gn_ws_bytes(n, c, spatial), y.device)
    if partial is not None and z is not None and lazy is not None:
        dy_pool, dskip, pool_mode = lazy
        assert dz2 is None and want_dres
        L.check(lib.mednet_gn_act_bwd_fused_res_pool(dy_pool.data_ptr(), L.ptr(dskip), y.data_ptr(), z.data_ptr(), stats.data_ptr(),
                                                     gamma_p.data_ptr(), partial.data_ptr(), partial.shape[1], dy.data_ptr(),
                                                     dres.data_ptr(), dgamma.data_ptr(), dbeta.data_ptr(), n, d, h, w, c, groups,
                                                     act, pool_mode, L.dt(y), ws.data_ptr(), ws.numel(), L.stream()),
                "gn_act_bwd_fused_res_pool")
        return dy, dres, (None if dg_direct else dgamma), (None if db_direct else dbeta)
    if partial is not None and z is not None:
        assert dz2 is None and want_dres
        L.check(lib.mednet_gn_act_bwd_fused_res(dz.data_ptr(), y.data_ptr(), z.data_ptr(), coef.data_ptr(), stats.data_ptr(),
                                                gamma_p.data_ptr(), partial.data_ptr(), partial.shape[1], dy.data_ptr(),
                                                dres.data_ptr(), dgamma.data_ptr(), dbeta.data_ptr(), n, spatial, c, groups, act,
                                                L.dt(y), ws.data_ptr(), ws.numel(), L.stream()), "gn_act_bwd_fused_res")
        return dy, dres, (None if dg_direct else dgamma), (None if db_direct else dbeta)
    if partial is not None:
        assert dz2 is None and z is None and not want_dres
        L.check(lib.mednet_gn_act_bwd_fused(dz.data_ptr(), y.data_ptr(), coef.data_ptr(), stats.data_ptr(), gamma_p.data_ptr(),
                                            partial.data_ptr(), partial.shape[1], dy.data_ptr(), dgamma.data_ptr(),
                                            dbeta.data_ptr(), n, spatial, c, groups, act, L.ACT_NONE, L.dt(y), ws.data_ptr(),
                                            ws.numel(), L.stream()), "gn_act_bwd_fused")
        return dy, None, (None if dg_direct else dgamma), (None if db_direct else dbeta)
    L.check(lib.mednet_gn_act_bwd(dz.data_ptr(), L.ptr(dz2), y.data_ptr(), L.ptr(z), coef.data_ptr(), stats.data_ptr(),
                                  gamma_p.data_ptr(), dy.data_ptr(), L.ptr(dres), dgamma.data_ptr(), dbeta.data_ptr(), n,
                                  spatial, c, groups, act, L.ACT_NONE, L.dt(y), ws.data_ptr(), ws.numel(), L.stream()),
            "gn_act_bwd")
    return dy, dres, (None if dg_direct else dgamma), (None if db_direct else dbeta)


FUSE_C1GN = os.environ.get("MEDNET_FUSE_C1GN", "1") == "1"
C1GN_COUNT = {"fused": 0}


def _c1_gn_applies(xin, y, partial, need_dx):
    if not (FUSE_C1GN and partial is not None and not need_dx and y.dtype != torch.float32 and config.conv_algo() != L.ALGO_DIRECT):
        return False
    cin = xin.shape[1]
    if cin == 1:
        return bool(L.lib().mednet_conv3d_wgrad_c1_gn_supported(y.shape[1], L.dt(xin), L.dt(y)))
    return bool(L.lib().mednet_conv3d_wgrad_cm_gn_supported(cin, y.shape[1], L.dt(xin), L.dt(y)))


def _c1_gn_bwd(xin, dz, y, coef, stats, gamma_p, beta_p, weight_p, groups, act, partial, x_layout=L.NDHWC):
    n, c, d, h, w = y.shape
    cin = xin.shape[1]
    lib = L.lib()
    C1GN_COUNT["fused"] += 1
    dgamma, dg_direct = ops._grad_target(gamma_p, (c,))
    dbeta, db_direct = ops._grad_target(beta_p, (c,))
    dw, dw_direct = ops._grad_target(weight_p, (c, cin, 3, 3, 3))
    bcoef = torch.empty((n, c, 3), dtype=torch.float32, device=y.device)
    ws = L.workspace(max(lib.mednet_gn_ws_bytes(n, c, d * h * w), lib.mednet_conv3d_wgrad_ws_bytes(n, d, h, w, cin, c, 3, 0)), y.device)
    L.check(lib.mednet_gn_bwd_coefficients(stats.data_ptr(), gamma_p.data_ptr(), partial.data_ptr(), partial.shape[1],
                                           bcoef.data_ptr(), dgamma.data_ptr(), dbeta.data_ptr(), n, d * h * w, c, groups,
                                           ws.data_ptr(), ws.numel(), L.stream()), "gn_bwd_coefficients")
    if cin == 1:
        L.check(lib.mednet_conv3d_wgrad_c1_gn(xin.data_ptr(), dz.data_ptr(), y.data_ptr(), coef.data_ptr(), bcoef.data_ptr(),
                                              dw.data_ptr(), n, d, h, w, c, act, L.dt(xin), L.dt(y), ws.data_ptr(), ws.numel(),
                                              L.stream()), "conv3d_wgrad_c1_gn")
    else:
        L.check(lib.mednet_conv3d_wgrad_cm_gn(xin.data_ptr(), x_layout, dz.data_ptr(), y.data_ptr(), coef.data_ptr(), bcoef.data_ptr(),
                                              dw.data_ptr(), n, d, h, w, cin, c, act, L.dt(xin), L.dt(y), ws.data_ptr(), ws.numel(),
                                              L.stream()), "conv3d_wgrad_cm_gn")
    return (None if dw_direct else dw), (None if dg_direct else dgamma), (None if db_direct else dbeta)


FUSE_DRES = os.environ.get("MEDNET_FUSE_DRES", "1") == "1"


FUSE_GNB = os.environ.get("MEDNET_FUSE_GNB", "1") == "1"


def _conv_bwd(x, dy, packed, weight_p, need_dx, add=None, gnb=None, x_layout=L.NDHWC):
    n, cin, d, h, w = x.shape
    cout = dy.shape[1]
    lib = L.lib()
    dx = None
    partial = None

    def dgrad():
        nonlocal dx, partial
        if need_dx:
            dx = ops.empty_cl(n, cin, d, h, w, x.dtype if x.dtype in (torch.float32, config.act_dtype()) else config.act_dtype(), dy.device)
            rows = 0
# ... 114 lines not shown
```

### torch-mednet_amd/mednet_hip/ops.py

```python
from __future__ import annotations

import os

import torch
from torch.autograd import Function

from . import _lib as L
from . import config, debug

CL = torch.channels_last_3d

PROFILE = {"enabled": False, "events": [], "match": None}


SIDE = {"enabled": False, "stream": None, "keepalive": [], "wgrad_wgs": int(os.environ.get("MEDNET_SIDE_WGRAD_WGS", "128"))}


SIDE_MIN_VOXELS = int(os.environ.get("MEDNET_SIDE_MIN_VOXELS", "0"))
SIDE_CORESIDENT = os.environ.get("MEDNET_SIDE_CORESIDENT", "1") == "1"


def wgrad_coresident(n, d, h, w, cin, cout, ksize, x, dy) -> bool:
    return bool(L.lib().mednet_conv3d_wgrad_coresident(n, d, h, w, cin, cout, ksize, L.dt(x), L.dt(dy), config.conv_algo()))

# ... 114 lines not shown
            PROFILE["dgrad_events"].append((self.e0, self.e1, self.flops, self.variant))
        return False


def _with_algo(backward):
    def wrapped(ctx, *grads):
        with config.algo_scope(getattr(ctx, "algo", None)):
            return backward(ctx, *grads)
    return wrapped


def _grad_target(param, shape):
    tgt = getattr(param, "_mednet_grad", None)
    if tgt is not None:
        assert tuple(tgt.shape) == tuple(shape) and tgt.dtype == torch.float32 and tgt.is_contiguous()
        return tgt, True
    return torch.empty(shape, dtype=torch.float32, device=param.device), False


def to_cl(x: torch.Tensor) -> torch.Tensor:
    return x.contiguous(memory_format=CL)


def empty_cl(n, c, d, h, w, dtype, device):
    return torch.empty((n, c, d, h, w), dtype=dtype, device=device, memory_format=CL)


def _storage_dtype(x: torch.Tensor) -> torch.dtype:
    return config.act_dtype()


def _as_act(x: torch.Tensor) -> torch.Tensor:
    if x.dtype == torch.float32 or x.dtype == config.act_dtype():
        return x
    return x.to(config.act_dtype())


def first_layer_input(x, cout, ksize, out_dtype, plain=True):
    cin = x.shape[1]
    if cin == 1:
        return x.contiguous(), L.NDHWC
    if (plain and 2 <= cin <= 4 and x.dtype == torch.float32 and out_dtype in config.HALF_TYPES
            and L.lib().mednet_conv3d_cm_supported(cin, cout, ksize, L.F32, L.dt_of(out_dtype), config.conv_algo())):
        if x.is_contiguous(memory_format=CL) and not x.is_contiguous():
            return x, L.NDHWC
        return x.contiguous(), L.NCDHW
    return to_cl(x), L.NDHWC


def pack_conv_weight(weight: torch.Tensor, ksize: int, transposed: bool, out: torch.Tensor = None) -> torch.Tensor:
    L.require_gpu(weight, "pack_conv_weight")
    w = weight.detach()
    if w.dtype != torch.float32 or not w.is_contiguous():
        w = w.float().contiguous()
    cin, cout = (w.shape[0], w.shape[1]) if transposed else (w.shape[1], w.shape[0])
    nbytes = L.lib().mednet_conv3d_pack_bytes(cin, cout, ksize)
    if out is not None and (out.numel() != nbytes or out.device != w.device):
        raise RuntimeError("pack_conv_weight: `out` is not this layer's pack buffer")
    buf = out if out is not None else torch.empty(nbytes, dtype=torch.uint8, device=w.device)
    elt = config.pack_elt()
    L.check(L.lib().mednet_conv3d_pack_elt(w.data_ptr(), buf.data_ptr(), cin, cout, ksize, int(transposed), elt, L.stream()),
            "conv3d_pack")
    return buf


class GN3Hook:
    __slots__ = ("gn_in", "act", "partial", "dx", "version", "lazy")

    def __init__(self):
        self.gn_in = None
        self.act = 0
        self.partial = self.dx = None
        self.version = -1
        self.lazy = None

    def offer(self, dx, partial, lazy=None):
        self.dx, self.partial, self.version, self.lazy = dx, partial, dx._version, lazy

    def take(self, dout):
        partial, dx, version, lazy = self.partial, self.dx, self.version, self.lazy
        self.partial = self.dx = self.lazy = None
        ok = partial is not None and dout is dx and dout._version == version
        if lazy is not None and not ok:
            raise RuntimeError("mednet_hip: the block output handed to skip_pool2(sole_consumer=True) has another consumer (or its "
                               "gradient was replaced by a hook): the pooling backward did not materialise its gradient (MEDNET_LAZY_POOL=0 turns "
                               "the optimisation off)")
        GN3_COUNT["taken" if ok else ("declined" if partial is not None else "absent")] += 1
        self.lazy = lazy if ok else None
        return partial if ok else None


FUSE_GN3 = os.environ.get("MEDNET_FUSE_GN3", "1") == "1"


class GNBHook(GN3Hook):
    __slots__ = ("coef",)

    def __init__(self):
        super().__init__()
        self.coef = None


class BNBHook(GNBHook):
    __slots__ = ()


class ActMaskHook:
    __slots__ = ("act", "dx", "version")

    def __init__(self, act):
        self.act, self.dx, self.version = act, None, -1

    def offer(self, dx):
        self.dx, self.version = dx, dx._version

    def take(self, dz):
        dx, version = self.dx, self.version
        self.dx = None
        ok = dx is not None and dz is dx and dz._version == version
        GN3_COUNT["masked"] += int(ok)
        return ok


def _gnb_hook_of(x, dtype):
    h = getattr(x, "_mednet_gnb", None) if FUSE_GN3 else None
    if h is None or h.gn_in is None or h.gn_in.shape != x.shape or h.gn_in.dtype != dtype or dtype not in config.HALF_TYPES:
        return None
    return h
GN3_COUNT = {"taken": 0, "declined": 0, "absent": 0, "masked": 0}


def _gn3_hook_of(x, dtype):
    h = getattr(x, "_mednet_gn3", None) if FUSE_GN3 else None
    if h is None or h.gn_in is None or h.gn_in.shape != x.shape or h.gn_in.dtype != dtype:
        return None
    return h


class Conv3dFn(Function):

    @staticmethod
    def forward(ctx, x, weight, bias, packed, ksize, out_planar, out_dtype, want_stats=False):
        L.require_gpu(x, "conv3d")
        ctx.algo = config.conv_algo()
        x = _as_act(x)
        n, cin, d, h, w = x.shape
        cout = weight.shape[0]
        xin, x_layout = first_layer_input(x, cout, ksize, out_dtype, plain=bias is None and not out_planar)
        if out_planar:
            y = torch.empty((n, cout, d, h, w), dtype=out_dtype, device=x.device)
        else:
            y = empty_cl(n, cout, d, h, w, out_dtype, x.device)
        partial = None
        if want_stats and bias is None and not out_planar:
            chunks = L.lib().mednet_conv3d_fused_stats_chunks(n, d, h, w, cin, cout, ksize, L.dt(xin), L.dt(y), config.conv_algo())
            if chunks > 0:
                partial = torch.empty((n, chunks, cout, 2), dtype=torch.float32, device=x.device)
        with profiled_conv(ksize, cin, cout, n, d, h, w):
            L.check(L.lib().mednet_conv3d_fwd(xin.data_ptr(), packed.data_ptr(), L.ptr(bias), y.data_ptr(), n, d, h, w, cin,
                                              cout, ksize, L.dt(xin), x_layout, L.dt(y), L.NCDHW if out_planar else L.NDHWC,
                                              0, config.conv_algo(), L.ptr(partial), L.stream()), "conv3d_fwd")
        ctx.save_for_backward(xin, packed)
        ctx.x_layout = x_layout
        ctx.meta = (ksize, out_planar, cin, cout, bias is not None, x.dtype)
        ctx.params = (weight, bias)
        ctx.gn3 = _gn3_hook_of(x, xin.dtype) if (ksize == 1 and out_planar and xin is x) else None
        ctx.gnb = None
        if ksize == 3 and not out_planar and xin is x:
            hook = _gnb_hook_of(x, xin.dtype)
            ctx.gnb = hook if isinstance(hook, BNBHook) else None
        if debug.TRACE is not None:
            debug.trace(f"conv3d.fwd k{ksize} {cin}->{cout}", y, partial)
        if not want_stats:
            return y
        if partial is None:
            partial = torch.empty(0, device=x.device)
        ctx.mark_non_differentiable(partial)
        return y, partial

    @staticmethod
    @_with_algo
    def backward(ctx, dy, _dpartial=None):
        xin, packed = ctx.saved_tensors
        ksize, out_planar, cin, cout, has_bias, x_dtype = ctx.meta
        n, _, d, h, w = xin.shape
        dy = dy.contiguous() if out_planar else to_cl(dy)
        lib = L.lib()
        dx = dw = db = None
        if ctx.needs_input_grad[0]:
            dx = empty_cl(n, cin, d, h, w, x_dtype, dy.device)
            hook = ctx.gn3
            rows = 0
            if hook is not None and dy.dtype == torch.float32 and dx.dtype == xin.dtype and config.conv_algo() != L.ALGO_DIRECT:
                rows = lib.mednet_head_dgrad_gn_rows(n, d, h, w, cin, L.dt(dx))
            bnb = ctx.gnb
            bn_rows = 0
            if bnb is not None and dx.dtype == dy.dtype:
                bn_rows = lib.mednet_conv3d_dgrad_gn_rows_dt(n, d, h, w, cin, cout, config.conv_algo(), L.dt(dy))
            if rows > 0:
                partial = torch.empty((n, rows, cin, 2), dtype=torch.float32, device=dy.device)
                L.check(lib.mednet_head_dgrad_gn(dy.data_ptr(), packed.data_ptr(), dx.data_ptr(), hook.gn_in.data_ptr(),
                                                 xin.data_ptr(), hook.act, partial.data_ptr(), n, d, h, w, cin, cout, L.dt(dx),
                                                 L.stream()), "head_dgrad_gn")
                hook.offer(dx, partial)
            elif bn_rows > 0:
                partial = torch.empty((n, bn_rows, cin, 2), dtype=torch.float32, device=dy.device)
                L.check(lib.mednet_conv3d_dgrad_gn(dy.data_ptr(), packed.data_ptr(), None, dx.data_ptr(), bnb.gn_in.data_ptr(),
                                                   bnb.coef.data_ptr(), bnb.act, partial.data_ptr(), n, d, h, w, cin, cout,
                                                   config.conv_algo(), L.dt(dy), L.stream()), "conv3d_dgrad_gn")
                bnb.offer(dx, partial)
            else:
                L.check(lib.mednet_conv3d_fwd(dy.data_ptr(), packed.data_ptr(), None, dx.data_ptr(), n, d, h, w, cout, cin,
# ... 446 lines not shown


class Pool2Fn(Function):

    @staticmethod
    def forward(ctx, x, mode):
        L.require_gpu(x, "pool3d")
        x0 = x
        x = to_cl(_as_act(x))
        n, c, d, h, w = x.shape
        stash = getattr(x0, "_mednet_pooled", None) if x is x0 else None
        if (stash is not None and stash.mode == mode and stash.pooled is not None and stash.pooled.dtype == x.dtype
                and stash.version == x0._version):
            y, stash.pooled = stash.pooled, None
        else:
            y = empty_cl(n, c, d // 2, h // 2, w // 2, x.dtype, x.device)
            L.check(L.lib().mednet_pool2_fwd(x.data_ptr(), y.data_ptr(), n, d, h, w, c, mode, L.dt(x), L.stream()), "pool2_fwd")
        ctx.save_for_backward(x)
        ctx.mode = mode
        return y

    @staticmethod
    def backward(ctx, dy):
        (x,) = ctx.saved_tensors
        n, c, d, h, w = x.shape
        dy = to_cl(dy.to(x.dtype))
        dx = torch.empty_like(x, memory_format=CL)
        L.check(L.lib().mednet_pool2_bwd(dy.data_ptr(), x.data_ptr(), None, dx.data_ptr(), n, d, h, w, c, ctx.mode, L.dt(x),
                                         L.stream()), "pool2_bwd")
        return dx, None


def pool2(x, mode=L.POOL_MAX):
    return Pool2Fn.apply(x, mode)


class SkipPool2Fn(Function):

    @staticmethod
    def forward(ctx, x, mode, sole_consumer=False):
        L.require_gpu(x, "pool3d")
        x0 = x
        x = to_cl(_as_act(x))
        n, c, d, h, w = x.shape
        stash = getattr(x0, "_mednet_pooled", None) if x is x0 else None
        if (stash is not None and stash.mode == mode and stash.pooled is not None and stash.pooled.dtype == x.dtype
                and stash.version == x0._version):
            y, stash.pooled = stash.pooled, None
        else:
            y = empty_cl(n, c, d // 2, h // 2, w // 2, x.dtype, x.device)
            L.check(L.lib().mednet_pool2_fwd(x.data_ptr(), y.data_ptr(), n, d, h, w, c, mode, L.dt(x), L.stream()), "pool2_fwd")
        ctx.save_for_backward(x)
        ctx.mode = mode
        ctx.gn3 = _gn3_hook_of(x0, x.dtype) if x is x0 else None
        ctx.inmask = getattr(x0, "_mednet_actmask", None) if (x is x0 and FUSE_GN3 and POOL_ACT_MASK and not ((d | h | w) & 1)) else None
        ctx.lazy_ok = (bool(sole_consumer) and LAZY_POOL and ctx.gn3 is not None and not x0._backward_hooks
                       and not getattr(x0, "retains_grad", False))
        if debug.TRACE is not None:
            debug.trace(f"skip_pool2.fwd c{c}", y)
        return x.view_as(x), y

    @staticmethod
    def backward(ctx, dskip, dy):
        (x,) = ctx.saved_tensors
        n, c, d, h, w = x.shape
        if dy is None:
            return dskip, None, None
        dy = to_cl(dy.to(x.dtype))
        hook = ctx.gn3
        add_c = 0
        if dskip is not None:
            add_c = _channel_slice_of_cl(dskip, c) if (hook is None and dskip.dtype == x.dtype and c % 8 == 0 and not ((d | h | w) & 1)) else 0
            if add_c == 0 or add_c % 8:
                add_c = 0
                dskip = to_cl(dskip.to(x.dtype))
        dx = torch.empty_like(x, memory_format=CL)
        rows = L.lib().mednet_pool2_bwd_gn_rows(n, d, h, w, c, L.dt(x)) if hook is not None else 0
        if rows > 0:
            partial = torch.empty((n, rows, c, 2), dtype=torch.float32, device=x.device)
            lazy = ctx.lazy_ok and bool(L.lib().mednet_gn_act_pool_supported(d, h, w, c, L.dt(x)))
            L.check(L.lib().mednet_pool2_bwd_gn(dy.data_ptr(), x.data_ptr(), L.ptr(dskip), None if lazy else dx.data_ptr(),
                                                hook.gn_in.data_ptr(), hook.act, partial.data_ptr(), n, d, h, w, c, ctx.mode, L.dt(x),
                                                L.stream()), "pool2_bwd_gn")
            hook.offer(dx, partial, (dy, dskip, ctx.mode) if lazy else None)
            if debug.TRACE is not None:
                debug.trace(f"skip_pool2.bwd c{c}", None if lazy else dx, partial)
            return dx, None, None
        mask = ctx.inmask
        L.check(L.lib().mednet_pool2_bwd_act(dy.data_ptr(), x.data_ptr(), L.ptr(dskip), add_c, dx.data_ptr(), n, d, h, w, c, ctx.mode,
                                             L.ACT_NONE if mask is None else mask.act, L.dt(x), L.stream()), "pool2_bwd")
        if mask is not None:
            mask.offer(dx)
        if debug.TRACE is not None:
            debug.trace(f"skip_pool2.bwd c{c}", dx)
        return dx, None, None


POOL_ACT_MASK = os.environ.get("MEDNET_POOL_ACT_MASK", "1") == "1"
LAZY_POOL = os.environ.get("MEDNET_LAZY_POOL", "1") == "1"


def skip_pool2(x, mode=L.POOL_MAX, sole_consumer=False):
    return SkipPool2Fn.apply(x, mode, sole_consumer)


class UpCatFn(Function):

    @staticmethod
    def forward(ctx, enc, x, want_stats=False):
        L.require_gpu(x, "upsample_concat")
        enc = to_cl(_as_act(enc))
        x = to_cl(_as_act(x)).to(enc.dtype)
        n, ce, d, h, w = enc.shape
        _, cx, xd, xh, xw = x.shape
        out = empty_cl(n, ce + cx, d, h, w, enc.dtype, enc.device)
        lib = L.lib()
        chunks = lib.mednet_upcat_stats_chunks(n, d, h, w, ce, cx, L.dt(enc)) if want_stats else 0
        if chunks > 0:
            partial = torch.empty((n, chunks, ce + cx, 2), dtype=torch.float32, device=enc.device)
            L.check(lib.mednet_upcat_fwd_stats(enc.data_ptr(), x.data_ptr(), out.data_ptr(), partial.data_ptr(), n, d, h, w, ce, xd, xh,
                                               xw, cx, L.dt(enc), L.stream()), "upcat_fwd_stats")
        else:
            partial = torch.empty(0, device=enc.device)
            L.check(lib.mednet_upcat_fwd(enc.data_ptr(), x.data_ptr(), out.data_ptr(), n, d, h, w, ce, xd, xh, xw, cx,
                                         L.dt(enc), L.stream()), "upcat_fwd")
        ctx.dims = (n, ce, d, h, w, cx, xd, xh, xw)
        if not want_stats:
            return out
        ctx.mark_non_differentiable(partial)
        return out, partial

    @staticmethod
    def backward(ctx, dout, _dpartial=None):
        n, ce, d, h, w, cx, xd, xh, xw = ctx.dims
        dout = to_cl(dout)
        view = UPCAT_VIEW and ce % 8 == 0 and cx % 8 == 0
        denc = dout.narrow(1, 0, ce) if view else empty_cl(n, ce, d, h, w, dout.dtype, dout.device)
        dx = empty_cl(n, cx, xd, xh, xw, dout.dtype, dout.device)
        L.check(L.lib().mednet_upcat_bwd(dout.data_ptr(), None if view else denc.data_ptr(), dx.data_ptr(), n, d, h, w, ce, xd, xh,
                                         xw, cx, L.dt(dout), L.stream()), "upcat_bwd")
        return denc, dx, None


UPCAT_VIEW = os.environ.get("MEDNET_UPCAT_VIEW", "1") == "1"


def _channel_slice_of_cl(t, c):
    if t.dim() != 5 or t.shape[1] != c:
        return 0
    n, _, d, h, w = t.shape
    sn, sc, sd, sh, sw = t.stride()
    ct = sw
    if sc == 1 and ct > c and sh == w * ct and sd == h * w * ct and sn == d * h * w * ct:
        return ct
    return 0


def upsample_concat(enc, x, want_stats=False):
    if not want_stats:
        return UpCatFn.apply(enc, x)
    out, partial = UpCatFn.apply(enc, x, True)
    return out, (partial if partial.numel() else None)


def _planar_logits(logits: torch.Tensor):
    t = logits if logits.dtype == torch.float32 else logits.float()
    sp = t.shape[2:]
    dense = []
    acc = 1
    for s in reversed(sp):
        dense.insert(0, acc)
        acc *= s
    if tuple(t.stride()[2:]) != tuple(dense):
        t = t.contiguous()
    return t, t.stride(0), t.stride(1)


def _labels_i64(labels: torch.Tensor, shape):
    if labels.dtype != torch.int64:
        labels = labels.long()
    if tuple(labels.shape) != tuple(shape):
        raise AssertionError("'input' and 'target' must have the same shape")
    return labels.contiguous()


class DiceLossFn(Function):

    @staticmethod
    def forward(ctx, logits, labels, weight, eps, sigmoid, ignore_index):
        L.require_gpu(logits, "dice_loss")
        lg, sn, sc = _planar_logits(logits)
        n, c = lg.shape[:2]
        spatial = lg[0, 0].numel()
        lab, lab_sn, lab_dt = _label_view(labels, n, tuple(lg.shape[2:]))
        wt = None if weight is None else weight.to(device=lg.device, dtype=torch.float32).contiguous()
        loss = torch.empty((), dtype=torch.float32, device=lg.device)
        saved = torch.empty((c, 2), dtype=torch.float32, device=lg.device)
        lib = L.lib()
        ws = L.workspace(lib.mednet_loss_ws_bytes(n, c, spatial), lg.device)
        ii = L.NO_IGNORE if ignore_index is None else int(ignore_index)
        L.check(lib.mednet_dice_fwd_lt(lg.data_ptr(), lab.data_ptr(), lab_dt, lab_sn, L.ptr(wt), loss.data_ptr(), saved.data_ptr(),
                                       None, n, c, spatial, sn, sc, eps, int(sigmoid), ii, ws.data_ptr(), ws.numel(), L.stream()),
                "dice_fwd")
        ctx.save_for_backward(lg, lab, wt, saved)
        ctx.meta = (eps, int(sigmoid), ii, sn, sc, logits.dtype, lab_sn, lab_dt)
        ctx.split = getattr(logits, "_mednet_split", None) if lg is logits else None
        if debug.TRACE is not None:
            debug.trace("dice.fwd", lg, loss, saved)
        return loss

    @staticmethod
    def backward(ctx, dloss):
        lg, lab, wt, saved = ctx.saved_tensors
        eps, sigmoid, ii, sn, sc, in_dtype, lab_sn, lab_dt = ctx.meta
        n, c = lg.shape[:2]
        spatial = lg[0, 0].numel()
        dl = dloss.to(torch.float32).contiguous()
        dlogits = _loss_grad_like(lg, ctx.split)
        L.check(L.lib().mednet_dice_bwd_lt(lg.data_ptr(), lab.data_ptr(), lab_dt, lab_sn, L.ptr(wt), saved.data_ptr(), dl.data_ptr(),
                                           dlogits.data_ptr(), n, c, spatial, sn, sc, eps, sigmoid, ii, L.stream()),
                "dice_bwd")
        if debug.TRACE is not None:
            debug.trace("dice.bwd", dlogits)
        return dlogits.to(in_dtype), None, None, None, None, None


def dice_loss(logits, labels, weight=None, eps=1e-5, sigmoid=False, ignore_index=None):
    return DiceLossFn.apply(logits, labels, weight, eps, sigmoid, ignore_index)


FUSE_HEAD_LOSS = os.environ.get("MEDNET_FUSE_HEAD_LOSS", "1") == "1"


def _label_view(labels: torch.Tensor, n: int, spatial_shape):
    if labels.dtype not in (torch.uint8, torch.int64):
        labels = labels.long()
    if tuple(labels.shape) != (n,) + tuple(spatial_shape):
        raise AssertionError("'input' and 'target' must have the same shape")
    dense, acc = [], 1
    for sdim in reversed(spatial_shape):
        dense.insert(0, acc)
        acc *= sdim
    if tuple(labels.stride()[1:]) != tuple(dense) or (n > 1 and labels.stride(0) < acc):
        labels = labels.contiguous()
    return labels, (labels.stride(0) if n > 1 else acc), (L.U8 if labels.dtype == torch.uint8 else L.I64)


def head_dice_supported(x: torch.Tensor, cin: int, cout: int, labels: torch.Tensor) -> bool:
    if not (FUSE_HEAD_LOSS and x.is_cuda and x.dim() == 5 and labels.is_cuda):
        return False
    if x.dtype != config.act_dtype() or not x.is_contiguous(memory_format=CL):
        return False
    ld = L.U8 if labels.dtype == torch.uint8 else L.I64
    return bool(L.lib().mednet_head_dice_supported(cin, cout, L.dt(x), ld))


class HeadDiceFn(Function):

    @staticmethod
    def forward(ctx, x, weight, bias, packed, labels, loss_weight, eps, sigmoid, ignore_index):
        L.require_gpu(x, "head_dice")
        n, cin, d, h, w = x.shape
        cout = weight.shape[0]
        spatial = d * h * w
        lab, lab_sn, lab_dt = _label_view(labels, n, (d, h, w))
        wt = None if loss_weight is None else loss_weight.to(device=x.device, dtype=torch.float32).contiguous()
        logits = torch.empty((n, cout, d, h, w), dtype=torch.float32, device=x.device)
        loss = torch.empty((), dtype=torch.float32, device=x.device)
        saved = torch.empty((cout, 2), dtype=torch.float32, device=x.device)
        lib = L.lib()
        ws = L.workspace(lib.mednet_head_dice_ws_bytes(n, spatial, cin, cout), x.device)
        ii = L.NO_IGNORE if ignore_index is None else int(ignore_index)
        L.check(lib.mednet_head_dice_fwd(x.data_ptr(), packed.data_ptr(), L.ptr(bias), lab.data_ptr(), lab_dt, lab_sn, L.ptr(wt),
                                         logits.data_ptr(), loss.data_ptr(), saved.data_ptr(), n, spatial, cin, cout, eps,
                                         int(sigmoid), ii, L.dt(x), ws.data_ptr(), ws.numel(), L.stream()), "head_dice_fwd")
        ctx.save_for_backward(x, packed, logits, lab, wt, saved)
        ctx.meta = (eps, int(sigmoid), ii, lab_sn, lab_dt, cin, cout)
        ctx.params = (weight, bias)
        ctx.gn3 = _gn3_hook_of(x, x.dtype)
        ctx.inmask = getattr(x, "_mednet_actmask", None) if (ctx.gn3 is None and FUSE_GN3 and POOL_ACT_MASK) else None
        ctx.mark_non_differentiable(logits)
        if debug.TRACE is not None:
            debug.trace("head_dice.fwd", logits, loss, saved)
        return logits, loss

    @staticmethod
    def backward(ctx, _dlogits, dloss):
        x, packed, logits, lab, wt, saved = ctx.saved_tensors
        eps, sigmoid, ii, lab_sn, lab_dt, cin, cout = ctx.meta
        weight, bias = ctx.params
        n, _, d, h, w = x.shape
        spatial = d * h * w
        lib = L.lib()
        dl = dloss.to(torch.float32).contiguous()
        dx = torch.empty_like(x, memory_format=CL)
        dw, direct_w = _grad_target(weight, (cout, cin, 1, 1, 1))
        db, direct_b = (None, True) if bias is None else _grad_target(bias, (cout,))
        hook = ctx.gn3
        partial = None
        if hook is not None:
            partial = torch.empty((n, lib.mednet_head_dice_gn_rows(n, spatial, cin), cin, 2), dtype=torch.float32, device=x.device)
        ws = L.workspace(lib.mednet_head_dice_ws_bytes(n, spatial, cin, cout), x.device)
        L.check(lib.mednet_head_dice_bwd(logits.data_ptr(), lab.data_ptr(), lab_dt, lab_sn, packed.data_ptr(), L.ptr(wt),
                                         saved.data_ptr(), dl.data_ptr(), dx.data_ptr(),
                                         None if hook is None else hook.gn_in.data_ptr(), x.data_ptr(),
                                         hook.act if hook is not None else (ctx.inmask.act if ctx.inmask is not None else 0),
                                         L.ptr(partial), dw.data_ptr(), L.ptr(db), n, spatial, cin,
                                         cout, eps, sigmoid, ii, L.dt(x), ws.data_ptr(), ws.numel(), L.stream()), "head_dice_bwd")
        if hook is not None:
            hook.offer(dx, partial)
        elif ctx.inmask is not None:
            ctx.inmask.offer(dx)
        if debug.TRACE is not None:
            debug.trace("head_dice.bwd", dx, partial, dw, db)
        return dx, (None if direct_w else dw), (None if (bias is None or direct_b) else db), None, None, None, None, None, None


def head_dice(x, weight, bias, packed, labels, loss_weight=None, eps=1e-5, sigmoid=False, ignore_index=None):
    return HeadDiceFn.apply(x, weight, bias, packed, labels, loss_weight, eps, sigmoid, ignore_index)


def head_ce_supported(x: torch.Tensor, cin: int, cout: int, labels: torch.Tensor) -> bool:
    if not (FUSE_HEAD_LOSS and x.is_cuda and x.dim() == 5 and labels.is_cuda):
        return False
    if x.dtype != config.act_dtype() or not x.is_contiguous(memory_format=CL):
        return False
    ld = L.U8 if labels.dtype == torch.uint8 else L.I64
    return bool(L.lib().mednet_head_ce_supported(cin, cout, L.dt(x), ld))


class HeadCEFn(Function):

    @staticmethod
    def forward(ctx, x, weight, bias, packed, labels, loss_weight, ignore_index):
        L.require_gpu(x, "head_ce")
        n, cin, d, h, w = x.shape
        cout = weight.shape[0]
        spatial = d * h * w
        lab, lab_sn, lab_dt = _label_view(labels, n, (d, h, w))
        wt = None if loss_weight is None else loss_weight.to(device=x.device, dtype=torch.float32).contiguous()
        logits = torch.empty((n, cout, d, h, w), dtype=torch.float32, device=x.device)
        loss = torch.empty((), dtype=torch.float32, device=x.device)
        saved = torch.empty((2,), dtype=torch.float32, device=x.device)
        lib = L.lib()
        ws = L.workspace(lib.mednet_head_ce_ws_bytes(n, spatial, cin, cout), x.device)
        ii = int(ignore_index)
        L.check(lib.mednet_head_ce_fwd(x.data_ptr(), packed.data_ptr(), L.ptr(bias), lab.data_ptr(), lab_dt, lab_sn, L.ptr(wt),
                                       logits.data_ptr(), loss.data_ptr(), saved.data_ptr(), n, spatial, cin, cout, ii, L.dt(x),
                                       ws.data_ptr(), ws.numel(), L.stream()), "head_ce_fwd")
        ctx.save_for_backward(x, packed, logits, lab, wt, saved)
        ctx.meta = (ii, lab_sn, lab_dt, cin, cout)
        ctx.params = (weight, bias)
        ctx.gn3 = _gn3_hook_of(x, x.dtype)
        ctx.inmask = getattr(x, "_mednet_actmask", None) if (ctx.gn3 is None and FUSE_GN3 and POOL_ACT_MASK) else None
        ctx.mark_non_differentiable(logits)
        if debug.TRACE is not None:
            debug.trace("head_ce.fwd", logits, loss, saved)
        return logits, loss

    @staticmethod
    def backward(ctx, _dlogits, dloss):
        x, packed, logits, lab, wt, saved = ctx.saved_tensors
        ii, lab_sn, lab_dt, cin, cout = ctx.meta
        weight, bias = ctx.params
        n, _, d, h, w = x.shape
        spatial = d * h * w
        lib = L.lib()
        dl = dloss.to(torch.float32).contiguous()
        dx = torch.empty_like(x, memory_format=CL)
        dw, direct_w = _grad_target(weight, (cout, cin, 1, 1, 1))
        db, direct_b = (None, True) if bias is None else _grad_target(bias, (cout,))
        hook = ctx.gn3
        partial = None
        if hook is not None:
            partial = torch.empty((n, lib.mednet_head_ce_gn_rows(n, spatial, cin), cin, 2), dtype=torch.float32, device=x.device)
        ws = L.workspace(lib.mednet_head_ce_ws_bytes(n, spatial, cin, cout), x.device)
        L.check(lib.mednet_head_ce_bwd(logits.data_ptr(), lab.data_ptr(), lab_dt, lab_sn, packed.data_ptr(), L.ptr(wt),
                                       saved.data_ptr(), dl.data_ptr(), dx.data_ptr(),
                                       None if hook is None else hook.gn_in.data_ptr(), x.data_ptr(),
                                       hook.act if hook is not None else (ctx.inmask.act if ctx.inmask is not None else 0),
                                       L.ptr(partial), dw.data_ptr(), L.ptr(db), n, spatial, cin, cout, ii, L.dt(x),
                                       ws.data_ptr(), ws.numel(), L.stream()), "head_ce_bwd")
        if hook is not None:
            hook.offer(dx, partial)
        elif ctx.inmask is not None:
            ctx.inmask.offer(dx)
        if debug.TRACE is not None:
            debug.trace("head_ce.bwd", dx, partial, dw, db)
        return dx, (None if direct_w else dw), (None if (bias is None or direct_b) else db), None, None, None, None


def head_ce(x, weight, bias, packed, labels, loss_weight=None, ignore_index=-100):
    return HeadCEFn.apply(x, weight, bias, packed, labels, loss_weight, ignore_index)


def _heatmap_view(heatmaps: torch.Tensor, n: int, nh: int, spatial_shape):
    if tuple(heatmaps.shape) != (n, nh) + tuple(spatial_shape):
        raise RuntimeError(f"heatmap_loss: target shape {tuple(heatmaps.shape)} != output {(n, nh) + tuple(spatial_shape)}")
    dense, acc = [], 1
    for sdim in reversed((nh,) + tuple(spatial_shape)):
        dense.insert(0, acc)
        acc *= sdim
    if tuple(heatmaps.stride()[1:]) != tuple(dense) or (n > 1 and heatmaps.stride(0) < acc):
        heatmaps = heatmaps.contiguous()
    return heatmaps, (heatmaps.stride(0) if n > 1 else acc)


def head_landmark_supported(x: torch.Tensor, cin: int, nh: int, ncls: int, heatmaps: torch.Tensor, labels: torch.Tensor) -> bool:
    if not (FUSE_HEAD_LOSS and x.is_cuda and x.dim() == 5 and labels.is_cuda and heatmaps.is_cuda):
        return False
    if x.dtype != config.act_dtype() or x.dtype == torch.float32 or not x.is_contiguous(memory_format=CL):
        return False
    if heatmaps.dtype != torch.uint8 or labels.dtype != torch.uint8:
        return False
    if getattr(x, "_mednet_actmask", None) is not None and _gn3_hook_of(x, x.dtype) is None:
        return False
    return bool(L.lib().mednet_head_landmark_supported(cin, nh, ncls, L.dt(x), x[0, 0].numel()))


class HeadLandmarkFn(Function):

    @staticmethod
    def forward(ctx, x, weight, bias, packed, heatmaps, labels, class_weight, reg_weight, kind, eps, sigmoid, ignore_index,
                class_kind=L.CLASS_DICE):
        L.require_gpu(x, "head_landmark")
        n, cin = x.shape[:2]
        nh = heatmaps.shape[1]
        ncls = weight.shape[0] - nh
        hm, hm_sn, lab, lab_sn, cw, rw, ii = _landmark_operands(x, heatmaps, labels, class_weight, reg_weight, ignore_index)
        closs, rloss, saved, _ = _landmark_fwd(x, packed, bias, hm, hm_sn, lab, lab_sn, cw, rw, nh, ncls, kind, eps, sigmoid, ii,
                                               class_kind, False)
        ctx.save_for_backward(x, packed, hm, lab, cw, rw, saved)
        ctx.meta = (kind, eps, int(sigmoid), ii, hm_sn, lab_sn, cin, nh, ncls, class_kind)
        ctx.params = (weight, bias)
        ctx.gn3 = _gn3_hook_of(x, x.dtype)
        if debug.TRACE is not None:
            debug.trace("head_landmark.fwd", closs, rloss, saved)
        return closs, rloss

    @staticmethod
    def backward(ctx, dclass, dreg):
        x, packed, hm, lab, cw, rw, saved = ctx.saved_tensors
        kind, eps, sigmoid, ii, hm_sn, lab_sn, cin, nh, ncls, class_kind = ctx.meta
        weight, bias = ctx.params
        n, _, d, h, w = x.shape
        spatial = d * h * w
        lib = L.lib()
        zero = None
        if dclass is None or dreg is None:
            zero = torch.zeros((), dtype=torch.float32, device=x.device)
        dc = zero if dclass is None else dclass.to(torch.float32).contiguous()
        dr = zero if dreg is None else dreg.to(torch.float32).contiguous()
        dx = torch.empty_like(x, memory_format=CL)
        dw, direct_w = _grad_target(weight, (nh + ncls, cin, 1, 1, 1))
        db, direct_b = (None, True) if bias is None else _grad_target(bias, (nh + ncls,))
        hook = ctx.gn3
        partial = None
        if hook is not None:
            partial = torch.empty((n, lib.mednet_head_landmark_gn_rows(spatial), cin, 2), dtype=torch.float32, device=x.device)
        ws = L.workspace(lib.mednet_head_landmark_ws_bytes(n, spatial, nh, ncls), x.device)
        if class_kind == L.CLASS_DICE:
            L.check(lib.mednet_head_landmark_bwd(x.data_ptr(), packed.data_ptr(), L.ptr(bias), hm.data_ptr(), hm_sn, lab.data_ptr(), lab_sn,
                                                 L.ptr(cw), L.ptr(rw), saved.data_ptr(), dc.data_ptr(), dr.data_ptr(), dx.data_ptr(),
                                                 None if hook is None else hook.gn_in.data_ptr(), hook.act if hook is not None else 0,
                                                 L.ptr(partial), dw.data_ptr(), L.ptr(db), n, spatial, cin, nh, ncls, kind, eps, sigmoid,
                                                 ii, L.dt(x), ws.data_ptr(), ws.numel(), L.stream()), "head_landmark_bwd")
        else:
            L.check(lib.mednet_head_landmark_cls_bwd(x.data_ptr(), packed.data_ptr(), L.ptr(bias), hm.data_ptr(), hm_sn, lab.data_ptr(),
                                                     lab_sn, L.ptr(cw), L.ptr(rw), saved.data_ptr(), dc.data_ptr(), dr.data_ptr(),
                                                     dx.data_ptr(), None if hook is None else hook.gn_in.data_ptr(),
                                                     hook.act if hook is not None else 0, L.ptr(partial), dw.data_ptr(), L.ptr(db), n,
                                                     spatial, cin, nh, ncls, kind, class_kind, eps, sigmoid, ii, L.dt(x), ws.data_ptr(),
                                                     ws.numel(), L.stream()), "head_landmark_cls_bwd")
        if hook is not None:
            hook.offer(dx, partial)
        if debug.TRACE is not None:
# ... 174 lines not shown
```

### torch-mednet_amd/mednet_hip/train.py

```python
from __future__ import annotations

import os

import torch
import torch.distributed as dist

from . import ops, vis
from .unet import loss as HL


class FlatParams:

    def __init__(self, module: torch.nn.Module):
        self.params = [p for p in module.parameters() if p.requires_grad]
        dev = self.params[0].device
        self.offsets = []
        total = 0
        for p in self.params:
            self.offsets.append(total)
            total += (p.numel() + 63) // 64 * 64
        self.total = total
        self.flat = torch.zeros(total, dtype=torch.float32, device=dev)
        self.grad = torch.zeros(total, dtype=torch.float32, device=dev)
        for p, off in zip(self.params, self.offsets):
# ... 229 lines not shown
                 and not torch.cuda.is_current_stream_capturing())
        if timed:
            e0, e1 = torch.cuda.Event(enable_timing=True), torch.cuda.Event(enable_timing=True)
            e0.record()
        scale = self._finish()
        if timed:
            e1.record()
            BucketedExchange.TIMING.append((e0, e1))
        return scale

    def _finish(self):
        if self.work is not None:
            dist.all_reduce(self.flat.grad[:self.split], op=dist.ReduceOp.SUM)
            self.work.wait()
            self.work = None
        elif self.world > 1 or self.force:
            dist.all_reduce(self.flat.grad, op=dist.ReduceOp.SUM)
        return 1.0 / self.world


class _GraphedStep:

    GRAPH_DEFAULT = os.environ.get("MEDNET_GRAPH", "0") == "1"

    def _init_graph(self, graph, warm=2):
        self.use_graph = self.GRAPH_DEFAULT if graph is None else bool(graph)
        self._calls, self._warm, self._graph, self._static = 0, warm, None, None

    def _run(self, batch):
        if not self.use_graph:
            return self._fwd_bwd(batch)
        self._calls += 1
        if self._graph is None:
            if self._calls <= self._warm:
                return self._fwd_bwd(batch)
            ops.PROFILE["enabled"] = False
            self._static = {k: v for k, v in batch.items()}
            torch.cuda.synchronize()
            self._graph = torch.cuda.CUDAGraph()
            with torch.cuda.graph(self._graph):
                self._out = self._fwd_bwd(self._static)
        for k, v in batch.items():
            if v is not self._static[k]:
                self._static[k].copy_(v)
        self._graph.replay()
        return self._out


def use_side_stream():
    ops.SIDE["enabled"] = os.environ.get("MEDNET_SIDE_STREAM", "1") == "1"


def _call_is_hooked(model, final_conv) -> bool:
    import torch.nn.modules.module as M
    for name in ("_global_forward_hooks", "_global_forward_pre_hooks", "_global_forward_hooks_always_called"):
        if getattr(M, name, None):
            return True
    return any(bool(getattr(mod, attr, None)) for mod in (model, final_conv) for attr in ("_forward_hooks", "_forward_pre_hooks"))


class SegmentationStep(_GraphedStep):

    def __init__(self, model, loss_weight=None, lr=1e-3, loss="DICE", world_size=1, graph=None):
        self.model = model
        dev = next(model.parameters()).device
        w = None if loss_weight is None else torch.tensor(loss_weight, dtype=torch.float32, device=dev)
        self.loss = (HL.DiceLoss(weight=w) if loss == "DICE" else HL.CrossEntropyLoss(weight=w)).to(dev)
        self.flat = FlatParams(model)
        self.opt = FlatAdam(self.flat, lr=lr)
        self.repack = BatchedRepack(model)
        self.world = world_size
        use_side_stream()
        self.scaler = make_scaler(dev)
        self._init_graph(graph)
        self._exchange = None

    def _head_loss(self, inputs, label_u8):
        from .unet.model import _UNetCore
        m, fc = self.model, getattr(self.model, "final_conv", None)
        dice = isinstance(self.loss, HL.DiceLoss)
        if (isinstance(m, _UNetCore) and not m.testing and (isinstance(self.loss, HL.CrossEntropyLoss) or (dice and not self.loss.skip_last_target))
                and fc is not None and getattr(fc, "planar_output", False) and fc.kernel_size[0] == 1 and inputs.is_cuda
                and not _call_is_hooked(m, fc)):
            feats = m.forward_features(inputs)
            if dice and ops.head_dice_supported(feats, fc.in_channels, fc.out_channels, label_u8):
                return ops.head_dice(feats, fc.weight, fc.bias, fc._packed(), label_u8, self.loss.weight, self.loss.epsilon,
                                     self.loss.sigmoid_normalization, self.loss.ignore_index)
            if not dice and ops.head_ce_supported(feats, fc.in_channels, fc.out_channels, label_u8):
                return ops.head_ce(feats, fc.weight, fc.bias, fc._packed(), label_u8, self.loss.weight, self.loss.ignore_index)
            outputs = fc(feats)
        else:
            outputs = m(inputs)
        return outputs, self.loss(outputs, label_u8.long())

    def _fwd_bwd(self, batch):
        inputs = batch["data"].float()
        _, loss = self._head_loss(inputs, batch["label"][:, -1, ...])
        (loss if self.scaler is None else self.scaler.scale_loss(loss)).backward()
        finish_backward()
        return (loss.detach(),)

    def __call__(self, batch):
        force = getattr(self, "force_allreduce", False)
        if self._exchange is None:
            self._exchange = BucketedExchange(self.model, self.flat, self.world, force)
        (loss,) = self._run(batch)
        scale = self._exchange.finish()
        if self.scaler is None:
            self.opt.step(grad_scale=scale)
        else:
            self.opt.step_scaled(self.scaler, inv_world=scale)
        self.repack.run()
        return loss


class SegmentationValidation:

    def __init__(self, model, loss_weight=None, loss="DICE", log_interval=None, log_vis_mip="mean", on_samples=None):
        self.model = model
        dev = next(model.parameters()).device
        w = None if loss_weight is None else torch.tensor(loss_weight, dtype=torch.float32, device=dev)
        self.loss = (HL.DiceLoss(weight=w) if loss == "DICE" else HL.CrossEntropyLoss(weight=w)).to(dev)
        self.log_interval, self.log_vis_mip, self.on_samples = log_interval, log_vis_mip, on_samples

    @torch.no_grad()
    def validation_step(self, batch, batch_nb=0):
        inputs = batch["data"].float()
        labels = batch["label"][:, -1, ...].long()
        was_training = self.model.training
        self.model.eval()
        try:
            outputs = self.model(inputs)
        finally:
            self.model.train(was_training)
        if _logs_samples(self, batch_nb):
            self.on_samples(vis.sample_panels(outputs, _class_map(batch["label"], labels), inputs, 0,
                                              projection_type=self.log_vis_mip), batch_nb)
        results = {"val_loss": self.loss(outputs, labels)}
        per_channel_dice = HL.dice_metric(outputs, labels)
        for c in range(outputs.shape[1]):
            results[f"val_dice{c}"] = per_channel_dice[c]
        return results

    @staticmethod
    def validation_epoch_end(outputs):
        logs = {k: torch.stack([o[k] for o in outputs]).mean() for k in outputs[0]}
        return {"val_loss": logs["val_loss"], "log": logs, "progress_bar": logs}


def _logs_samples(validation, batch_nb) -> bool:
    return bool(validation.log_interval) and validation.on_samples is not None and batch_nb % validation.log_interval == 0


def _class_map(label, labels_long):
    return label[:, -1, ...] if label.dtype in (torch.uint8, torch.int64) else labels_long


def _landmark_losses(class_weight, regression_weight, class_loss, regression, dev):
    if class_loss not in ("DICE", "CE"):
        raise ValueError(f"class_loss must be 'DICE' or 'CE', not {class_loss!r}")
    w = torch.tensor(class_weight, dtype=torch.float32, device=dev)
    loss_class = (HL.DiceLoss(weight=w) if class_loss == "DICE" else HL.CrossEntropyLoss(weight=w)).to(dev)
    return loss_class, HL.HeatmapRegressionLoss(regression_weight, regression).to(dev)


def _landmark_head_fusable(model, loss_class, loss_reg, inputs) -> bool:
    from .unet.model import _UNetCore
    fc = getattr(model, "final_conv", None)
    return (isinstance(model, _UNetCore) and not model.testing and fc is not None and getattr(fc, "planar_output", False)
            and fc.kernel_size[0] == 1 and inputs.is_cuda and not getattr(loss_class, "skip_last_target", False)
            and loss_reg.kind in ("L1", "L2") and not _call_is_hooked(model, fc))

# ... 123 lines not shown
```

Before: 210.2 patches/s.

## Recompute head dice/CE gradient inside GN backward apply instead of storing dx

The head loss backward can now skip writing the full-resolution dx tensor when the final decoder output is consumed only by the head. A new GN-backward apply kernel recomputes the logit gradient and the 1x1 head projection per voxel from logits and labels, then applies the GN coefficients directly. This removes one large bf16 write and one read of a 32-channel 128^3 activation, at the cost of recomputing softmax and projection work and adding a lazy-offer path with more code complexity.

```diff
diff --git a/include/mednet_hip.h b/include/mednet_hip.h
--- a/include/mednet_hip.h
+++ b/include/mednet_hip.h
@@ -129,6 +129,13 @@
                                      const float* gamma, const float* fused_partial, int rows, void* dx, void* dres, float* dgamma,
                                      float* dbeta, int n, int d, int h, int w, int c, int groups, int act, int pool_mode, int dtype,
                                      void* ws, size_t ws_bytes, mednet_stream stream);
+int mednet_gn_act_bwd_fused_res_head_supported(int cin, int cout, int dtype, int label_dtype);
+int mednet_gn_act_bwd_fused_res_head(const float* logits, const void* labels, int label_dtype, int64_t label_stride_n,
+                                     const void* packed, const float* weight, const float* saved, const float* dloss, float eps,
+                                     int sigmoid, int ignore_index, int loss_kind, const void* x, const void* z, const float* stats,
+                                     const float* gamma, const float* fused_partial, int rows, void* dx, void* dres, float* dgamma,
+                                     float* dbeta, int n, size_t spatial, int cin, int cout, int groups, int act, int dtype, void* ws,
+                                     size_t ws_bytes, mednet_stream stream);
 int mednet_bn_stats(const void* x, const float* gamma, const float* beta, float* running_mean, float* running_var,
                     long long* num_batches_tracked, float momentum, float* stats, float* coef, int n, size_t spatial, int c,
                     float eps, int dtype, void* ws, size_t ws_bytes, mednet_stream stream);
diff --git a/torch-mednet_amd/csrc/conv.h b/torch-mednet_amd/csrc/conv.h
--- a/torch-mednet_amd/csrc/conv.h
+++ b/torch-mednet_amd/csrc/conv.h
@@ -59,6 +59,27 @@
                     float* dw, int n, int d, int h, int w, int cin, int cout, int dtype, void* ws, size_t ws_bytes, hipStream_t s);
 int launch_pack_f32(const float* w, float* Pf, float* Pb, int cin, int cout, int T, int transposed_src, hipStream_t s);
 
+struct GnParamGrad {
+  const float* csum = nullptr;
+  float* dgamma = nullptr;
+  float* dbeta = nullptr;
+  int n = 0;
+};
+int gn_bwd_fused_coefficients(const float* fused_partial, int rows, const float* stats, const float* gamma, float* dgamma,
+                              float* dbeta, int n, size_t spatial, int c, int groups, void* ws, hipStream_t s, float** bcoef,
+                              GnParamGrad* pg);
+__device__ __forceinline__ void gn_param_grad_tail(const GnParamGrad& pg, int c) {
+  for (int cc = threadIdx.x; cc < c; cc += 256) {
+    double a = 0.0, b = 0.0;
+    for (int i = 0; i < pg.n; ++i) {
+      a += (double)pg.csum[((size_t)i * c + cc) * 2];
+      b += (double)pg.csum[((size_t)i * c + cc) * 2 + 1];
+    }
+    if (pg.dbeta) pg.dbeta[cc] = (float)a;
+    if (pg.dgamma) pg.dgamma[cc] = (float)b;
+  }
+}
+
 int launch_hm_finalize(const float* partial, const float* cweight, float* loss, int n, int c, int nblocks, size_t spatial,
                        hipStream_t s);
 int launch_dice_finalize(const float* partial, const float* weight, float* loss, float* saved, int c, int nblocks, float eps,
diff --git a/torch-mednet_amd/csrc/head_loss.hip b/torch-mednet_amd/csrc/head_loss.hip
--- a/torch-mednet_amd/csrc/head_loss.hip
+++ b/torch-mednet_amd/csrc/head_loss.hip
@@ -157,8 +157,117 @@
     }
 }
 
-template <typename TO, int K, typename TL, bool FOLD = false, bool CE = false>
-__global__ __launch_bounds__(256, (sizeof(TO) == 2 && !FOLD) ? 3 : 2) void head_dice_bwd_kernel(const float* __restrict__ lgs, const TL* __restrict__ lab, int64_t lab_sn,
+__device__ __forceinline__ void probs_quad(const float* lg, int c, int sigmoid, float* p) {
+  static_assert(HL_MAXC == 4, "one class per lane of a quad");
+  const int q = threadIdx.x & 3;
+  const float own = q == 0 ? lg[0] : q == 1 ? lg[1] : q == 2 ? lg[2] : lg[3];
+  float e;
+  if (sigmoid) {
+    e = 1.f / (1.f + expf(-own));
+  } else {
+    float mx = -INFINITY;
+#pragma unroll
+    for (int k = 0; k < HL_MAXC; ++k)
+      if (k < c) mx = fmaxf(mx, lg[k]);
+    e = expf(own - mx);
+  }
+  p[0] = dpp_f32<(0) | (0 << 2) | (0 << 4) | (0 << 6)>(e);
+  p[1] = dpp_f32<(1) | (1 << 2) | (1 << 4) | (1 << 6)>(e);
+  p[2] = dpp_f32<(2) | (2 << 2) | (2 << 4) | (2 << 6)>(e);
+  p[3] = dpp_f32<(3) | (3 << 2) | (3 << 4) | (3 << 6)>(e);
+  if (!sigmoid) {
+    float den = 0.f;
+#pragma unroll
+    for (int k = 0; k < HL_MAXC; ++k)
+      if (k < c) den += p[k];
+    const float inv = 1.f / den;
+#pragma unroll
+    for (int k = 0; k < HL_MAXC; ++k)
+      if (k < c) p[k] *= inv;
+  }
+}
+
+template <bool CE>
+struct HeadLogitGrad {
+  float gI[HL_MAXC], gD[HL_MAXC];
+  int m, sigmoid, ignore;
+  __device__ __forceinline__ HeadLogitGrad(const float* __restrict__ weight, const float* __restrict__ saved,
+                                           const float* __restrict__ dloss, float eps, int m_, int sigmoid_, int ignore_)
+      : m(m_), sigmoid(CE ? 0 : sigmoid_), ignore(ignore_) {
+    const float go = *dloss;
+#pragma unroll
+    for (int k = 0; k < HL_MAXC; ++k) {
+      gI[k] = gD[k] = 0.f;
+      if (CE && k < m) {
+        gI[k] = (weight ? weight[k] : 1.f) * (go / saved[0]);
+      } else if (k < m) {
+        const float w = weight ? weight[k] : 1.f;
+        const float I = saved[2 * k], D = saved[2 * k + 1];
+        const float Dc = fmaxf(D, eps);
+        gI[k] = -2.f * w / ((float)m * Dc) * go + ((I != I || D != D) ? __builtin_nanf("") : 0.f);
+        gD[k] = (D >= eps ? 2.f * w * I / ((float)m * Dc * Dc) : 0.f) * go;
+      }
+      gI[k] = __builtin_bit_cast(float, __builtin_amdgcn_readfirstlane(__builtin_bit_cast(int, gI[k])));
+      gD[k] = __builtin_bit_cast(float, __builtin_amdgcn_readfirstlane(__builtin_bit_cast(int, gD[k])));
+    }
+  }
+  template <bool QUAD>
+  __device__ __forceinline__ void at(const float* lg, int yl, float* dl) const {
+    float p[HL_MAXC];
+    if constexpr (QUAD) probs_quad(lg, m, sigmoid, p);
+    else probs_reg(lg, m, sigmoid, p);
+    if constexpr (CE) {
+      float w = 0.f;
+#pragma unroll
+      for (int k = 0; k < HL_MAXC; ++k)
+        if (k < m && k == yl) w = gI[k];
+      w = (yl != ignore && yl >= 0 && yl < m) ? w : 0.f;
+#pragma unroll
+      for (int k = 0; k < HL_MAXC; ++k) dl[k] = k < m ? w * (p[k] - (k == yl ? 1.f : 0.f)) : 0.f;
+      return;
+    }
+    float g[HL_MAXC];
+    float dot = 0.f;
+#pragma unroll
+    for (int k = 0; k < HL_MAXC; ++k)
+      if (k < m) {
+        const float t = (k == yl) ? 1.f : 0.f;
+        const float mk = (ignore != MEDNET_NO_IGNORE && t == (float)ignore) ? 0.f : 1.f;
+        g[k] = mk * (gI[k] * t * mk + gD[k]);
+        dot = fmaf(p[k], g[k], dot);
+      }
+#pragma unroll
+    for (int k = 0; k < HL_MAXC; ++k) dl[k] = k < m ? (sigmoid ? g[k] * p[k] * (1.f - p[k]) : p[k] * (g[k] - dot)) : 0.f;
+  }
+};
+
+template <bool QUAD>
+__device__ __forceinline__ void load_logits2(const float* __restrict__ lgs, size_t spatial, int m, size_t v, size_t vbs, float* la,
+                                             float* lb) {
+  if constexpr (QUAD) {
+    const int cq = threadIdx.x & 3;
+    const float oa = cq < m ? lgs[(size_t)cq * spatial + v] : 0.f;
+    const float ob = cq < m ? lgs[(size_t)cq * spatial + vbs] : 0.f;
+    la[0] = dpp_f32<(0) | (0 << 2) | (0 << 4) | (0 << 6)>(oa);
+    la[1] = dpp_f32<(1) | (1 << 2) | (1 << 4) | (1 << 6)>(oa);
+    la[2] = dpp_f32<(2) | (2 << 2) | (2 << 4) | (2 << 6)>(oa);
+    la[3] = dpp_f32<(3) | (3 << 2) | (3 << 4) | (3 << 6)>(oa);
+    lb[0] = dpp_f32<(0) | (0 << 2) | (0 << 4) | (0 << 6)>(ob);
+    lb[1] = dpp_f32<(1) | (1 << 2) | (1 << 4) | (1 << 6)>(ob);
+    lb[2] = dpp_f32<(2) | (2 << 2) | (2 << 4) | (2 << 6)>(ob);
+    lb[3] = dpp_f32<(3) | (3 << 2) | (3 << 4) | (3 << 6)>(ob);
+    static_assert(HL_MAXC == 4, "one class per lane of a quad");
+  } else {
+#pragma unroll
+    for (int i = 0; i < HL_MAXC; ++i) {
+      la[i] = i < m ? lgs[(size_t)i * spatial + v] : 0.f;
+      lb[i] = i < m ? lgs[(size_t)i * spatial + vbs] : 0.f;
+    }
+  }
+}
+
+template <typename TO, int K, typename TL, bool FOLD = false, bool CE = false, bool STORE = true>
+__global__ __launch_bounds__(256, (sizeof(TO) == 2 && !FOLD && STORE) ? 3 : 2) void head_dice_bwd_kernel(const float* __restrict__ lgs, const TL* __restrict__ lab, int64_t lab_sn,
                                                             const float* __restrict__ Pb , const float* __restrict__ weight,
                                                             const float* __restrict__ saved, const float* __restrict__ dloss,
                                                             float eps, int sigmoid, int ignore, TO* __restrict__ dz,
@@ -166,6 +275,7 @@
                                                             float* __restrict__ gn_partial , float* __restrict__ wpart,
                                                             size_t spatial, int m) {
   constexpr int CG = K / 8, VPW = 256 / CG;
+  constexpr bool QS = CG == 4 && !FOLD;
   const int n = blockIdx.y;
   const int cgi = threadIdx.x % CG, vi = threadIdx.x / CG;
   float wreg[HL_MAXC][8];
@@ -173,48 +283,7 @@
   for (int i = 0; i < HL_MAXC; ++i)
 #pragma unroll
     for (int j = 0; j < 8; ++j) wreg[i][j] = i < m ? Pb[(size_t)i * K + cgi * 8 + j] : 0.f;
-  const float go = *dloss;
-  float gI[HL_MAXC], gD[HL_MAXC];
-#pragma unroll
-  for (int k = 0; k < HL_MAXC; ++k) {
-    gI[k] = gD[k] = 0.f;
-    if (CE && k < m) {
-      gI[k] = (weight ? weight[k] : 1.f) * (go / saved[0]);
-    } else if (k < m) {
-      const float w = weight ? weight[k] : 1.f;
-      const float I = saved[2 * k], D = saved[2 * k + 1];
-      const float Dc = fmaxf(D, eps);
-      gI[k] = -2.f * w / ((float)m * Dc) * go + ((I != I || D != D) ? __builtin_nanf("") : 0.f);
-      gD[k] = (D >= eps ? 2.f * w * I / ((float)m * Dc * Dc) : 0.f) * go;
-    }
-  }
-  auto dlogits_of = [&](const float* lg, int yl, float* dl) {
-    if constexpr (CE) {
-      float p[HL_MAXC];
-      probs_reg(lg, m, 0, p);
-      float w = 0.f;
-#pragma unroll
-      for (int k = 0; k < HL_MAXC; ++k)
-        if (k < m && k == yl) w = gI[k];
-      w = (yl != ignore && yl >= 0 && yl < m) ? w : 0.f;
-#pragma unroll
-      for (int k = 0; k < HL_MAXC; ++k) dl[k] = k < m ? w * (p[k] - (k == yl ? 1.f : 0.f)) : 0.f;
-      return;
-    }
-    float p[HL_MAXC], g[HL_MAXC];
-    probs_reg(lg, m, sigmoid, p);
-    float dot = 0.f;
-#pragma unroll
-    for (int k = 0; k < HL_MAXC; ++k)
-      if (k < m) {
-        const float t = (k == yl) ? 1.f : 0.f;
-        const float mk = (ignore != MEDNET_NO_IGNORE && t == (float)ignore) ? 0.f : 1.f;
-        g[k] = mk * (gI[k] * t * mk + gD[k]);
-        dot = fmaf(p[k], g[k], dot);
-      }
-#pragma unroll
-    for (int k = 0; k < HL_MAXC; ++k) dl[k] = k < m ? (sigmoid ? g[k] * p[k] * (1.f - p[k]) : p[k] * (g[k] - dot)) : 0.f;
-  };
+  const HeadLogitGrad<CE> dlogits_of(weight, saved, dloss, eps, m, sigmoid, ignore);
   float ss[8], sq[8], wacc[HL_MAXC][8], bacc[HL_MAXC];
 #pragma unroll
   for (int j = 0; j < 8; ++j) ss[j] = sq[j] = 0.f;
@@ -232,26 +301,7 @@
     const bool hb = (it + 1 < HL_VPT) && vb < spatial;
     const size_t vbs = hb ? vb : v;
     float la[HL_MAXC], lb[HL_MAXC];
-    if constexpr (CG == 4) {
-      const int cq = threadIdx.x & 3;
-      const float oa = cq < m ? lgs[((size_t)n * m + cq) * spatial + v] : 0.f;
-      const float ob = cq < m ? lgs[((size_t)n * m + cq) * spatial + vbs] : 0.f;
-      la[0] = dpp_f32<(0) | (0 << 2) | (0 << 4) | (0 << 6)>(oa);
-      la[1] = dpp_f32<(1) | (1 << 2) | (1 << 4) | (1 << 6)>(oa);
-      la[2] = dpp_f32<(2) | (2 << 2) | (2 << 4) | (2 << 6)>(oa);
-      la[3] = dpp_f32<(3) | (3 << 2) | (3 << 4) | (3 << 6)>(oa);
-      lb[0] = dpp_f32<(0) | (0 << 2) | (0 << 4) | (0 << 6)>(ob);
-      lb[1] = dpp_f32<(1) | (1 << 2) | (1 << 4) | (1 << 6)>(ob);
-      lb[2] = dpp_f32<(2) | (2 << 2) | (2 << 4) | (2 << 6)>(ob);
-      lb[3] = dpp_f32<(3) | (3 << 2) | (3 << 4) | (3 << 6)>(ob);
-      static_assert(HL_MAXC == 4, "one class per lane of a quad");
-    } else {
-#pragma unroll
-      for (int i = 0; i < HL_MAXC; ++i) {
-        la[i] = i < m ? lgs[((size_t)n * m + i) * spatial + v] : 0.f;
-        lb[i] = i < m ? lgs[((size_t)n * m + i) * spatial + vbs] : 0.f;
-      }
-    }
+    load_logits2<CG == 4>(lgs + (size_t)n * m * spatial, spatial, m, v, vbs, la, lb);
     const int ya = label_at(lab, (size_t)n * lab_sn + v), yb = label_at(lab, (size_t)n * lab_sn + vbs);
     const size_t rowa = ((size_t)n * spatial + v) * K + cgi * 8, rowb = ((size_t)n * spatial + vbs) * K + cgi * 8;
     Raw8<TO> zva, zvb, yva, yvb;
@@ -265,8 +315,8 @@
       yvb = zvb;
     }
     float da[HL_MAXC], db[HL_MAXC];
-    dlogits_of(la, ya, da);
-    dlogits_of(lb, yb, db);
+    dlogits_of.template at<QS>(la, ya, da);
+    dlogits_of.template at<QS>(lb, yb, db);
     if (!hb) {
 #pragma unroll
       for (int i = 0; i < HL_MAXC; ++i) db[i] = 0.f;
@@ -301,8 +351,10 @@
       act_grad_n<8>(t.v, za, act);
       act_grad_n<8>(u.v, zb, act);
     }
-    st8(dz, rowa, t);
-    if (hb) st8(dz, rowb, u);
+    if constexpr (STORE) {
+      st8(dz, rowa, t);
+      if (hb) st8(dz, rowb, u);
+    }
     if (!FOLD && gy) {
       float za[8], zb[8];
 #pragma unroll
@@ -343,6 +395,98 @@
       }
       const float b = lane_class_sum<CG>(bacc[i]);
       if (lane == 0) wout[(size_t)m * K + i] = b;
+    }
+  }
+}
+
+template <typename T, int K, typename TL, bool CE>
+__global__ __launch_bounds__(256) void gn_bwd_apply_head_kernel(const float* __restrict__ lgs, const TL* __restrict__ lab, int64_t lab_sn,
+                                                                const float* __restrict__ Pb , const float* __restrict__ weight,
+                                                                const float* __restrict__ saved, const float* __restrict__ dloss,
+                                                                float eps, int sigmoid, int ignore, const T* __restrict__ gy,
+                                                                const T* __restrict__ gz, int act, const float* __restrict__ bcoef,
+                                                                T* __restrict__ dy3, T* __restrict__ dres, size_t spatial, int m,
+                                                                GnParamGrad pg) {
+  static_assert(sizeof(T) == 2, "16-bit storage");
+  if (pg.csum && blockIdx.x == 0 && blockIdx.y == 0) gn_param_grad_tail(pg, K);
+  constexpr int CG = K / 8, VPW = 256 / CG;
+  const int n = blockIdx.y;
+  const int cgi = threadIdx.x % CG, vi = threadIdx.x / CG;
+  float wreg[HL_MAXC][8], k1[8], k2[8], k3[8];
+#pragma unroll
+  for (int i = 0; i < HL_MAXC; ++i)
+#pragma unroll
+    for (int j = 0; j < 8; ++j) wreg[i][j] = i < m ? Pb[(size_t)i * K + cgi * 8 + j] : 0.f;
+#pragma unroll
+  for (int j = 0; j < 8; ++j) {
+    const float* o = bcoef + ((size_t)n * K + cgi * 8 + j) * 3;
+    k1[j] = o[0];
+    k2[j] = o[1];
+    k3[j] = o[2];
+  }
+  const HeadLogitGrad<CE> dlogits_of(weight, saved, dloss, eps, m, sigmoid, ignore);
+  const size_t v0 = (size_t)blockIdx.x * (VPW * HL_VPT) + vi;
+  for (int it = 0; it < HL_VPT; it += 2) {
+    const size_t v = v0 + (size_t)it * VPW;
+    if (v >= spatial) break;
+    const size_t vb = v + VPW;
+    const bool hb = (it + 1 < HL_VPT) && vb < spatial;
+    const size_t vbs = hb ? vb : v;
+    float la[HL_MAXC], lb[HL_MAXC];
+    load_logits2<CG == 4>(lgs + (size_t)n * m * spatial, spatial, m, v, vbs, la, lb);
+    const int ya = label_at(lab, (size_t)n * lab_sn + v), yb = label_at(lab, (size_t)n * lab_sn + vbs);
+    const size_t rowa = ((size_t)n * spatial + v) * K + cgi * 8, rowb = ((size_t)n * spatial + vbs) * K + cgi * 8;
+    Raw8<T> zva, zvb, yva, yvb;
+    zva.load(gz, rowa);
+    zvb.load(gz, rowb);
+    yva.load(gy, rowa);
+    yvb.load(gy, rowb);
+    float da[HL_MAXC], db[HL_MAXC];
+    dlogits_of.template at<CG == 4>(la, ya, da);
+    dlogits_of.template at<CG == 4>(lb, yb, db);
+    F8 t, u;
+#pragma unroll
+    for (int j = 0; j < 8; ++j) t.v[j] = u.v[j] = 0.f;
+#pragma unroll
+    for (int i = 0; i < HL_MAXC; ++i) {
+      if (i < m) {
+#pragma unroll
+        for (int j = 0; j < 8; ++j) {
+          t.v[j] = fmaf(da[i], wreg[i][j], t.v[j]);
+          u.v[j] = fmaf(db[i], wreg[i][j], u.v[j]);
+        }
+      }
+    }
+    float za[8], zb[8];
+#pragma unroll
+    for (int j = 0; j < 8; ++j) {
+      asm volatile("" : "+v"(t.v[j]));
+      asm volatile("" : "+v"(u.v[j]));
+      t.v[j] = (float)(T)t.v[j];
+      u.v[j] = (float)(T)u.v[j];
+      za[j] = zva.at(j);
+      zb[j] = zvb.at(j);
+    }
+    act_grad_n<8>(t.v, za, act);
+    act_grad_n<8>(u.v, zb, act);
+    F8 oa8, ob8;
+#pragma unroll
+    for (int j = 0; j < 8; ++j) {
+      float xa = yva.at(j), xb = yvb.at(j);
+      asm volatile("" : "+v"(xa));
+      asm volatile("" : "+v"(xb));
+      asm volatile("" : "+v"(t.v[j]));
+      asm volatile("" : "+v"(u.v[j]));
+      oa8.v[j] = fmaf(k1[j], t.v[j], fmaf(k2[j], xa, k3[j]));
+      ob8.v[j] = fmaf(k1[j], u.v[j], fmaf(k2[j], xb, k3[j]));
+      asm volatile("" : "+v"(oa8.v[j]));
+      asm volatile("" : "+v"(ob8.v[j]));
+    }
+    st8(dy3, rowa, oa8);
+    st8(dres, rowa, t);
+    if (hb) {
+      st8(dy3, rowb, ob8);
+      st8(dres, rowb, u);
     }
   }
 }
@@ -441,8 +585,9 @@
                          float eps, int sigmoid, int ignore_index, int z_dtype, void* ws, size_t ws_bytes, mednet_stream stream) {
   MEDNET_REQUIRE(mednet_head_dice_supported(cin, cout, z_dtype, label_dtype), MEDNET_E_UNSUPPORTED,
                  "%s: %d -> %d classes, dtype %d, labels %d", what, cin, cout, z_dtype, label_dtype);
-  MEDNET_REQUIRE(n > 0 && spatial > 0 && logits && labels && packed && saved && dloss && dz && z && dw, MEDNET_E_SHAPE, "%s: bad arguments", what);
+  MEDNET_REQUIRE(n > 0 && spatial > 0 && logits && labels && packed && saved && dloss && z && dw, MEDNET_E_SHAPE, "%s: bad arguments", what);
   MEDNET_REQUIRE((gn_y == nullptr) == (gn_partial == nullptr), MEDNET_E_SHAPE, "%s: gn_y and gn_partial go together", what);
+  MEDNET_REQUIRE(dz || gn_y, MEDNET_E_SHAPE, "%s: dz == NULL (sums only) needs gn_y and gn_partial", what);
   MEDNET_REQUIRE(ws_bytes >= mednet_head_dice_ws_bytes(n, spatial, cin, cout), MEDNET_E_WORKSPACE, "%s: workspace too small", what);
   const PackLayout L = pack_layout(cin, cout, 1);
   const float* Pb = (const float*)((const char*)packed + L.f32_bwd);
@@ -451,8 +596,8 @@
   float* wpart = (float*)ws;
   const dim3 grid(nb, n);
   const bool fold = gn_y == nullptr && gn_act != MEDNET_ACT_NONE;
-#define HB_(TO_, K_, TL_, F_) hipLaunchKernelGGL((head_dice_bwd_kernel<TO_, K_, TL_, F_, CE>), grid, dim3(256), 0, s, logits, (const TL_*)labels, label_stride_n, Pb, weight, saved, dloss, eps, sigmoid, ignore_index, (TO_*)dz, (const TO_*)gn_y, (const TO_*)z, gn_act, gn_partial, wpart, spatial, cout)
-#define HB(TO_, K_, TL_) do { if (fold) HB_(TO_, K_, TL_, true); else HB_(TO_, K_, TL_, false); } while (0)
+#define HB_(TO_, K_, TL_, F_, S_) hipLaunchKernelGGL((head_dice_bwd_kernel<TO_, K_, TL_, F_, CE, S_>), grid, dim3(256), 0, s, logits, (const TL_*)labels, label_stride_n, Pb, weight, saved, dloss, eps, sigmoid, ignore_index, (TO_*)dz, (const TO_*)gn_y, (const TO_*)z, gn_act, gn_partial, wpart, spatial, cout)
+#define HB(TO_, K_, TL_) do { if (fold) HB_(TO_, K_, TL_, true, true); else if (dz) HB_(TO_, K_, TL_, false, true); else HB_(TO_, K_, TL_, false, false); } while (0)
 #define HB_L(TO_, K_) do { if (label_dtype == MEDNET_U8) HB(TO_, K_, uint8_t); else HB(TO_, K_, int64_t); } while (0)
 #define HB_K(TO_) do { if (cin == 16) HB_L(TO_, 16); else if (cin == 32) HB_L(TO_, 32); else HB_L(TO_, 64); } while (0)
   if (z_dtype == MEDNET_F32) HB_K(float);
@@ -511,3 +656,43 @@
   return head_loss_bwd<true>("head_ce_bwd", logits, labels, label_dtype, label_stride_n, packed, weight, saved, dloss, dz, gn_y, z, gn_act,
                              gn_partial, dw, dbias, n, spatial, cin, cout, 0.f, 0, ignore_index, z_dtype, ws, ws_bytes, stream);
 }
+
+extern "C" int mednet_gn_act_bwd_fused_res_head_supported(int cin, int cout, int dtype, int label_dtype) {
+  return mednet_head_dice_supported(cin, cout, dtype, label_dtype) && (dtype == MEDNET_BF16 || dtype == MEDNET_F16);
+}
+
+extern "C" int mednet_gn_act_bwd_fused_res_head(const float* logits, const void* labels, int label_dtype, int64_t label_stride_n,
+                                                const void* packed, const float* weight, const float* saved, const float* dloss,
+                                                float eps, int sigmoid, int ignore_index, int loss_kind, const void* x, const void* z,
+                                                const float* stats, const float* gamma, const float* fused_partial, int rows, void* dx,
+                                                void* dres, float* dgamma, float* dbeta, int n, size_t spatial, int cin, int cout,
+                                                int groups, int act, int dtype, void* ws, size_t ws_bytes, mednet_stream stream) {
+  MEDNET_REQUIRE(mednet_gn_act_bwd_fused_res_head_supported(cin, cout, dtype, label_dtype), MEDNET_E_UNSUPPORTED,
+                 "gn_act_bwd_fused_res_head: %d -> %d classes, dtype %d, labels %d", cin, cout, dtype, label_dtype);
+  MEDNET_REQUIRE(loss_kind == MEDNET_CLASS_DICE || loss_kind == MEDNET_CLASS_CE, MEDNET_E_SHAPE, "gn_act_bwd_fused_res_head: loss kind %d",
+                 loss_kind);
+  MEDNET_REQUIRE(n > 0 && spatial > 0 && groups > 0 && cin % groups == 0 && rows > 0 && logits && labels && packed && saved && dloss &&
+                     x && z && stats && fused_partial && dx && dres,
+                 MEDNET_E_SHAPE, "gn_act_bwd_fused_res_head: bad arguments");
+  MEDNET_REQUIRE(ws_bytes >= mednet_gn_ws_bytes(n, cin, spatial), MEDNET_E_WORKSPACE, "gn_act_bwd_fused_res_head: workspace too small");
+  hipStream_t s = (hipStream_t)stream;
+  float* bcoef;
+  GnParamGrad pg;
+  const int rc = gn_bwd_fused_coefficients(fused_partial, rows, stats, gamma, dgamma, dbeta, n, spatial, cin, groups, ws, s, &bcoef, &pg);
+  if (rc) return rc;
+  const PackLayout L = pack_layout(cin, cout, 1);
+  const float* Pb = (const float*)((const char*)packed + L.f32_bwd);
+  const dim3 grid(hl_bwd_blocks(spatial, cin), n);
+  const bool ce = loss_kind == MEDNET_CLASS_CE;
+#define GA_(T_, K_, TL_, CE_) hipLaunchKernelGGL((gn_bwd_apply_head_kernel<T_, K_, TL_, CE_>), grid, dim3(256), 0, s, logits, (const TL_*)labels, label_stride_n, Pb, weight, saved, dloss, eps, sigmoid, ignore_index, (const T_*)x, (const T_*)z, act, bcoef, (T_*)dx, (T_*)dres, spatial, cout, pg)
+#define GA(T_, K_, TL_) do { if (ce) GA_(T_, K_, TL_, true); else GA_(T_, K_, TL_, false); } while (0)
+#define GA_L(T_, K_) do { if (label_dtype == MEDNET_U8) GA(T_, K_, uint8_t); else GA(T_, K_, int64_t); } while (0)
+#define GA_K(T_) do { if (cin == 16) GA_L(T_, 16); else if (cin == 32) GA_L(T_, 32); else GA_L(T_, 64); } while (0)
+  if (dtype == MEDNET_BF16) GA_K(bf16);
+  else GA_K(f16);
+#undef GA_K
+#undef GA_L
+#undef GA
+#undef GA_
+  return check_launch("gn_bwd_apply_head");
+}
diff --git a/torch-mednet_amd/csrc/norm_act.hip b/torch-mednet_amd/csrc/norm_act.hip
--- a/torch-mednet_amd/csrc/norm_act.hip
+++ b/torch-mednet_amd/csrc/norm_act.hip
@@ -1,4 +1,5 @@
 #include "common.h"
+#include "conv.h"
 
 #ifndef GN_NT
 #define GN_NT 1
@@ -503,12 +504,6 @@
   const int cg = c / groups;
   return cg >= 1 && cg <= 256 && 256 % cg == 0 && tuning_option("gn_bwd_one_launch", 1);
 }
-struct GnParamGrad {
-  const float* csum = nullptr;
-  float* dgamma = nullptr;
-  float* dbeta = nullptr;
-  int n = 0;
-};
 __global__ __launch_bounds__(256) void gn_bwd_params_kernel(const float* __restrict__ csum, float* __restrict__ dgamma,
                                                             float* __restrict__ dbeta, int n, int c) {
   const int cc = blockIdx.x * 256 + threadIdx.x;
@@ -528,17 +523,7 @@
                                                            const float* __restrict__ bcoef, T* __restrict__ dx,
                                                            T* __restrict__ dres, size_t spatial, int c, int act,
                                                            size_t chunk_vox, int in_act, GnParamGrad pg) {
-  if (pg.csum && blockIdx.x == 0 && blockIdx.y == 0) {
-    for (int cc = threadIdx.x; cc < c; cc += 256) {
-      double a = 0.0, b = 0.0;
-      for (int i = 0; i < pg.n; ++i) {
-        a += (double)pg.csum[((size_t)i * c + cc) * 2];
-        b += (double)pg.csum[((size_t)i * c + cc) * 2 + 1];
-      }
-      if (pg.dbeta) pg.dbeta[cc] = (float)a;
-      if (pg.dgamma) pg.dgamma[cc] = (float)b;
-    }
-  }
+  if (pg.csum && blockIdx.x == 0 && blockIdx.y == 0) gn_param_grad_tail(pg, c);
   const Cols<VEC> L(c);
   if (!L.active) return;
   const int n = blockIdx.y;
@@ -872,17 +857,7 @@
                                                                 const float* __restrict__ bcoef, T* __restrict__ dx,
                                                                 T* __restrict__ dres, int n, int d, int h, int w, int c, int act,
                                                                 int mode, GnParamGrad pg) {
-  if (pg.csum && blockIdx.x == 0) {
-    for (int cc = threadIdx.x; cc < c; cc += 256) {
-      double a = 0.0, b = 0.0;
-      for (int i = 0; i < pg.n; ++i) {
-        a += (double)pg.csum[((size_t)i * c + cc) * 2];
-        b += (double)pg.csum[((size_t)i * c + cc) * 2 + 1];
-      }
-      if (pg.dbeta) pg.dbeta[cc] = (float)a;
-      if (pg.dgamma) pg.dgamma[cc] = (float)b;
-    }
-  }
+  if (pg.csum && blockIdx.x == 0) gn_param_grad_tail(pg, c);
   const int od = d / 2, oh = h / 2, ow = w / 2, cv = c / VEC;
   const size_t total = (size_t)n * od * oh * ow * cv;
   const size_t i = (size_t)blockIdx.x * 256 + threadIdx.x;
@@ -1385,6 +1360,37 @@
                                act, MEDNET_ACT_NONE, dtype, ws, ws_bytes, stream);
 }
 
+namespace mednet {
+int gn_bwd_fused_coefficients(const float* fused_partial, int rows, const float* stats, const float* gamma, float* dgamma,
+                              float* dbeta, int n, size_t spatial, int c, int groups, void* ws, hipStream_t s, float** bcoef_out,
+                              GnParamGrad* pg) {
+  float* bcoef = (float*)ws + (size_t)n * gn_partial_rows_max(c) * c * 2;
+  float* csum = bcoef + (size_t)n * c * 3;
+  *bcoef_out = bcoef;
+  *pg = GnParamGrad();
+  int rc;
+  if (gn_bwd_one_launch(c, groups)) {
+    hipLaunchKernelGGL(gn_bwd_reduce_finalize_kernel<true>, dim3(n * groups), dim3(256), 0, s, fused_partial, stats, gamma, csum, bcoef,
+                       c, groups, rows, (double)spatial * (c / groups));
+    rc = check_launch("gn_bwd_reduce_finalize");
+    if (rc) return rc;
+    if (dgamma || dbeta) *pg = GnParamGrad{csum, dgamma, dbeta, n};
+    return MEDNET_OK;
+  }
+  hipLaunchKernelGGL(reduce_partials_dux_kernel, dim3(n * c), dim3(64), 0, s, fused_partial, stats, csum, c, groups, rows);
+  hipLaunchKernelGGL(gn_bwd_finalize_kernel, dim3(n * groups), dim3(64), 0, s, csum, stats, gamma, bcoef, c, groups,
+                     (double)spatial * (c / groups));
+  rc = check_launch("gn_bwd_finalize");
+  if (rc) return rc;
+  if (dgamma || dbeta) {
+    hipLaunchKernelGGL(gn_bwd_params_kernel, dim3((c + 255) / 256), dim3(256), 0, s, csum, dgamma, dbeta, n, c);
+    rc = check_launch("gn_bwd_params");
+    if (rc) return rc;
+  }
+  return MEDNET_OK;
+}
+}
+
 extern "C" int mednet_gn_act_bwd_fused_res_pool(const void* dy_pool, const void* skip_grad, const void* x, const void* z,
                                                 const float* stats, const float* gamma, const float* fused_partial, int rows,
                                                 void* dx, void* dres, float* dgamma, float* dbeta, int n, int d, int h, int w, int c,
@@ -1397,29 +1403,11 @@
                  "gn_act_bwd_fused_res_pool: even extents and C %% 8 == 0 (%dx%dx%d, C=%d)", d, h, w, c);
   const size_t spatial = (size_t)d * h * w;
   MEDNET_REQUIRE(ws_bytes >= mednet_gn_ws_bytes(n, c, spatial), MEDNET_E_WORKSPACE, "gn_act_bwd_fused_res_pool: workspace too small");
-  float* bcoef = (float*)ws + (size_t)n * gn_partial_rows_max(c) * c * 2;
-  float* csum = bcoef + (size_t)n * c * 3;
-  hipStream_t s = (hipStream_t)stream;
+  hipStream_t s = (hipStream_t)stream;
+  float* bcoef;
   GnParamGrad pg;
-  int rc;
-  if (gn_bwd_one_launch(c, groups)) {
-    hipLaunchKernelGGL(gn_bwd_reduce_finalize_kernel<true>, dim3(n * groups), dim3(256), 0, s, fused_partial, stats, gamma, csum, bcoef,
-                       c, groups, rows, (double)spatial * (c / groups));
-    rc = check_launch("gn_bwd_reduce_finalize");
-    if (rc) return rc;
-    if (dgamma || dbeta) pg = GnParamGrad{csum, dgamma, dbeta, n};
-  } else {
-    hipLaunchKernelGGL(reduce_partials_dux_kernel, dim3(n * c), dim3(64), 0, s, fused_partial, stats, csum, c, groups, rows);
-    hipLaunchKernelGGL(gn_bwd_finalize_kernel, dim3(n * groups), dim3(64), 0, s, csum, stats, gamma, bcoef, c, groups,
-                       (double)spatial * (c / groups));
-    rc = check_launch("gn_bwd_finalize");
-    if (rc) return rc;
-    if (dgamma || dbeta) {
-      hipLaunchKernelGGL(gn_bwd_params_kernel, dim3((c + 255) / 256), dim3(256), 0, s, csum, dgamma, dbeta, n, c);
-      rc = check_launch("gn_bwd_params");
-      if (rc) return rc;
-    }
-  }
+  const int rc = gn_bwd_fused_coefficients(fused_partial, rows, stats, gamma, dgamma, dbeta, n, spatial, c, groups, ws, s, &bcoef, &pg);
+  if (rc) return rc;
   const int vec = dtype == MEDNET_F32 ? 4 : 8;
   const size_t total = (size_t)n * (d / 2) * (h / 2) * (w / 2) * (c / vec);
   const dim3 grid((unsigned)((total + 255) / 256));
diff --git a/torch-mednet_amd/mednet_hip/_lib.py b/torch-mednet_amd/mednet_hip/_lib.py
--- a/torch-mednet_amd/mednet_hip/_lib.py
+++ b/torch-mednet_amd/mednet_hip/_lib.py
@@ -53,6 +53,9 @@
     "mednet_gn_bwd_coefficients": (_i, [_vp, _vp, _vp, _i, _vp, _vp, _vp, _i, _sz, _i, _i, _vp, _sz, _vp]),
     "mednet_gn_act_bwd_fused_res": (_i, [_vp] * 7 + [_i, _vp, _vp, _vp, _vp, _i, _sz, _i, _i, _i, _i, _vp, _sz, _vp]),
     "mednet_gn_act_bwd_fused_res_pool": (_i, [_vp] * 7 + [_i, _vp, _vp, _vp, _vp] + [_i] * 9 + [_vp, _sz, _vp]),
+    "mednet_gn_act_bwd_fused_res_head_supported": (_i, [_i] * 4),
+    "mednet_gn_act_bwd_fused_res_head": (_i, [_vp, _vp, _i, _i64] + [_vp] * 4 + [_f, _i, _i, _i] + [_vp] * 5 + [_i, _vp, _vp, _vp, _vp,
+                                              _i, _sz, _i, _i, _i, _i, _i, _vp, _sz, _vp]),
     "mednet_head_dgrad_gn_rows": (_i, [_i] * 6),
     "mednet_head_dgrad_gn": (_i, [_vp] * 5 + [_i, _vp] + [_i] * 7 + [_vp]),
     "mednet_pool2_bwd_gn_rows": (_i, [_i] * 6),
diff --git a/torch-mednet_amd/mednet_hip/block.py b/torch-mednet_amd/mednet_hip/block.py
--- a/torch-mednet_amd/mednet_hip/block.py
+++ b/torch-mednet_amd/mednet_hip/block.py
@@ -64,8 +64,20 @@
     dgamma, dg_direct = ops._grad_target(gamma_p, (c,))
     dbeta, db_direct = ops._grad_target(beta_p, (c,))
     ws = L.workspace(lib.mednet_gn_ws_bytes(n, c, spatial), y.device)
+    if partial is not None and z is not None and lazy is not None and lazy[0] == "head":
+        hl = lazy[1]
+        assert dz2 is None and want_dres
+        L.check(lib.mednet_gn_act_bwd_fused_res_head(hl.logits.data_ptr(), hl.lab.data_ptr(), hl.lab_dt, hl.lab_sn, hl.packed.data_ptr(),
+                                                     L.ptr(hl.wt), hl.saved.data_ptr(), hl.dloss.data_ptr(), hl.eps, hl.sigmoid,
+                                                     hl.ignore, hl.kind, y.data_ptr(), z.data_ptr(), stats.data_ptr(),
+                                                     gamma_p.data_ptr(), partial.data_ptr(), partial.shape[1], dy.data_ptr(),
+                                                     dres.data_ptr(), dgamma.data_ptr(), dbeta.data_ptr(), n, spatial, c, hl.cout,
+                                                     groups, act, L.dt(y), ws.data_ptr(), ws.numel(), L.stream()),
+                "gn_act_bwd_fused_res_head")
+        ops.LAZY_HEAD_COUNT["lazy"] += 1
+        return dy, dres, (None if dg_direct else dgamma), (None if db_direct else dbeta)
     if partial is not None and z is not None and lazy is not None:
-        dy_pool, dskip, pool_mode = lazy
+        dy_pool, dskip, pool_mode = lazy[1]
         assert dz2 is None and want_dres
         L.check(lib.mednet_gn_act_bwd_fused_res_pool(dy_pool.data_ptr(), L.ptr(dskip), y.data_ptr(), z.data_ptr(), stats.data_ptr(),
                                                      gamma_p.data_ptr(), partial.data_ptr(), partial.shape[1], dy.data_ptr(),
diff --git a/torch-mednet_amd/mednet_hip/ops.py b/torch-mednet_amd/mednet_hip/ops.py
--- a/torch-mednet_amd/mednet_hip/ops.py
+++ b/torch-mednet_amd/mednet_hip/ops.py
@@ -220,8 +220,10 @@
         self.partial = self.dx = self.lazy = None
         ok = partial is not None and dout is dx and dout._version == version
         if lazy is not None and not ok:
-            raise RuntimeError("mednet_hip: the block output handed to skip_pool2(sole_consumer=True) has another consumer (or its "
-                               "gradient was replaced by a hook): the pooling backward did not materialise its gradient (MEDNET_LAZY_POOL=0 turns "
+            who, what, knob = (("skip_pool2", "pooling", "MEDNET_LAZY_POOL") if lazy[0] == "pool" else
+                               ("head_dice / head_ce", "head", "MEDNET_LAZY_HEAD"))
+            raise RuntimeError(f"mednet_hip: the block output handed to {who}(sole_consumer=True) has another consumer (or its "
+                               f"gradient was replaced by a hook): the {what} backward did not materialise its gradient ({knob}=0 turns "
                                "the optimisation off)")
         GN3_COUNT["taken" if ok else ("declined" if partial is not None else "absent")] += 1
         self.lazy = lazy if ok else None
@@ -266,6 +268,7 @@
         return None
     return h
 GN3_COUNT = {"taken": 0, "declined": 0, "absent": 0, "masked": 0}
+LAZY_HEAD_COUNT = {"lazy": 0}
 
 
 def _gn3_hook_of(x, dtype):
@@ -878,7 +881,7 @@
             L.check(L.lib().mednet_pool2_bwd_gn(dy.data_ptr(), x.data_ptr(), L.ptr(dskip), None if lazy else dx.data_ptr(),
                                                 hook.gn_in.data_ptr(), hook.act, partial.data_ptr(), n, d, h, w, c, ctx.mode, L.dt(x),
                                                 L.stream()), "pool2_bwd_gn")
-            hook.offer(dx, partial, (dy, dskip, ctx.mode) if lazy else None)
+            hook.offer(dx, partial, ("pool", (dy, dskip, ctx.mode)) if lazy else None)
             if debug.TRACE is not None:
                 debug.trace(f"skip_pool2.bwd c{c}", None if lazy else dx, partial)
             return dx, None, None
@@ -1042,6 +1045,23 @@
     return labels, (labels.stride(0) if n > 1 else acc), (L.U8 if labels.dtype == torch.uint8 else L.I64)
 
 
+LAZY_HEAD = os.environ.get("MEDNET_LAZY_HEAD", "1") == "1"
+
+
+class HeadLazy:
+    __slots__ = ("kind", "logits", "lab", "lab_dt", "lab_sn", "packed", "wt", "saved", "dloss", "eps", "sigmoid", "ignore", "cout")
+
+    def __init__(self, kind, logits, lab, lab_dt, lab_sn, packed, wt, saved, dloss, eps, sigmoid, ignore, cout):
+        self.kind, self.logits, self.lab, self.lab_dt, self.lab_sn, self.packed = kind, logits, lab, lab_dt, lab_sn, packed
+        self.wt, self.saved, self.dloss, self.eps, self.sigmoid, self.ignore, self.cout = wt, saved, dloss, eps, sigmoid, ignore, cout
+
+
+def _head_lazy_ok(x, hook, sole_consumer, cin, cout, lab_dt) -> bool:
+    return (bool(sole_consumer) and LAZY_HEAD and hook is not None and not x._backward_hooks
+            and not getattr(x, "retains_grad", False) and x.dtype in config.HALF_TYPES
+            and bool(L.lib().mednet_gn_act_bwd_fused_res_head_supported(cin, cout, L.dt(x), lab_dt)))
+
+
 def head_dice_supported(x: torch.Tensor, cin: int, cout: int, labels: torch.Tensor) -> bool:
     if not (FUSE_HEAD_LOSS and x.is_cuda and x.dim() == 5 and labels.is_cuda):
         return False
@@ -1054,7 +1074,7 @@
 class HeadDiceFn(Function):
 
     @staticmethod
-    def forward(ctx, x, weight, bias, packed, labels, loss_weight, eps, sigmoid, ignore_index):
+    def forward(ctx, x, weight, bias, packed, labels, loss_weight, eps, sigmoid, ignore_index, sole_consumer=False):
         L.require_gpu(x, "head_dice")
         n, cin, d, h, w = x.shape
         cout = weight.shape[0]
@@ -1074,6 +1094,7 @@
         ctx.meta = (eps, int(sigmoid), ii, lab_sn, lab_dt, cin, cout)
         ctx.params = (weight, bias)
         ctx.gn3 = _gn3_hook_of(x, x.dtype)
+        ctx.lazy_ok = _head_lazy_ok(x, ctx.gn3, sole_consumer, cin, cout, lab_dt)
         ctx.inmask = getattr(x, "_mednet_actmask", None) if (ctx.gn3 is None and FUSE_GN3 and POOL_ACT_MASK) else None
         ctx.mark_non_differentiable(logits)
         if debug.TRACE is not None:
@@ -1097,23 +1118,25 @@
         if hook is not None:
             partial = torch.empty((n, lib.mednet_head_dice_gn_rows(n, spatial, cin), cin, 2), dtype=torch.float32, device=x.device)
         ws = L.workspace(lib.mednet_head_dice_ws_bytes(n, spatial, cin, cout), x.device)
+        lazy = ctx.lazy_ok
         L.check(lib.mednet_head_dice_bwd(logits.data_ptr(), lab.data_ptr(), lab_dt, lab_sn, packed.data_ptr(), L.ptr(wt),
-                                         saved.data_ptr(), dl.data_ptr(), dx.data_ptr(),
+                                         saved.data_ptr(), dl.data_ptr(), None if lazy else dx.data_ptr(),
                                          None if hook is None else hook.gn_in.data_ptr(), x.data_ptr(),
                                          hook.act if hook is not None else (ctx.inmask.act if ctx.inmask is not None else 0),
                                          L.ptr(partial), dw.data_ptr(), L.ptr(db), n, spatial, cin,
                                          cout, eps, sigmoid, ii, L.dt(x), ws.data_ptr(), ws.numel(), L.stream()), "head_dice_bwd")
         if hook is not None:
-            hook.offer(dx, partial)
+            hook.offer(dx, partial, ("head", HeadLazy(L.CLASS_DICE, logits, lab, lab_dt, lab_sn, packed, wt, saved, dl, eps, sigmoid, ii,
+                                                      cout)) if lazy else None)
         elif ctx.inmask is not None:
             ctx.inmask.offer(dx)
         if debug.TRACE is not None:
-            debug.trace("head_dice.bwd", dx, partial, dw, db)
-        return dx, (None if direct_w else dw), (None if (bias is None or direct_b) else db), None, None, None, None, None, None
-
-
-def head_dice(x, weight, bias, packed, labels, loss_weight=None, eps=1e-5, sigmoid=False, ignore_index=None):
-    return HeadDiceFn.apply(x, weight, bias, packed, labels, loss_weight, eps, sigmoid, ignore_index)
+            debug.trace("head_dice.bwd", None if lazy else dx, partial, dw, db)
+        return dx, (None if direct_w else dw), (None if (bias is None or direct_b) else db), None, None, None, None, None, None, None
+
+
+def head_dice(x, weight, bias, packed, labels, loss_weight=None, eps=1e-5, sigmoid=False, ignore_index=None, sole_consumer=False):
+    return HeadDiceFn.apply(x, weight, bias, packed, labels, loss_weight, eps, sigmoid, ignore_index, sole_consumer)
 
 
 def head_ce_supported(x: torch.Tensor, cin: int, cout: int, labels: torch.Tensor) -> bool:
@@ -1128,7 +1151,7 @@
 class HeadCEFn(Function):
 
     @staticmethod
-    def forward(ctx, x, weight, bias, packed, labels, loss_weight, ignore_index):
+    def forward(ctx, x, weight, bias, packed, labels, loss_weight, ignore_index, sole_consumer=False):
         L.require_gpu(x, "head_ce")
         n, cin, d, h, w = x.shape
         cout = weight.shape[0]
@@ -1148,6 +1171,7 @@
         ctx.meta = (ii, lab_sn, lab_dt, cin, cout)
         ctx.params = (weight, bias)
         ctx.gn3 = _gn3_hook_of(x, x.dtype)
+        ctx.lazy_ok = _head_lazy_ok(x, ctx.gn3, sole_consumer, cin, cout, lab_dt)
         ctx.inmask = getattr(x, "_mednet_actmask", None) if (ctx.gn3 is None and FUSE_GN3 and POOL_ACT_MASK) else None
         ctx.mark_non_differentiable(logits)
         if debug.TRACE is not None:
@@ -1171,23 +1195,25 @@
         if hook is not None:
             partial = torch.empty((n, lib.mednet_head_ce_gn_rows(n, spatial, cin), cin, 2), dtype=torch.float32, device=x.device)
         ws = L.workspace(lib.mednet_head_ce_ws_bytes(n, spatial, cin, cout), x.device)
+        lazy = ctx.lazy_ok
         L.check(lib.mednet_head_ce_bwd(logits.data_ptr(), lab.data_ptr(), lab_dt, lab_sn, packed.data_ptr(), L.ptr(wt),
-                                       saved.data_ptr(), dl.data_ptr(), dx.data_ptr(),
+                                       saved.data_ptr(), dl.data_ptr(), None if lazy else dx.data_ptr(),
                                        None if hook is None else hook.gn_in.data_ptr(), x.data_ptr(),
                                        hook.act if hook is not None else (ctx.inmask.act if ctx.inmask is not None else 0),
                                        L.ptr(partial), dw.data_ptr(), L.ptr(db), n, spatial, cin, cout, ii, L.dt(x),
                                        ws.data_ptr(), ws.numel(), L.stream()), "head_ce_bwd")
         if hook is not None:
-            hook.offer(dx, partial)
+            hook.offer(dx, partial, ("head", HeadLazy(L.CLASS_CE, logits, lab, lab_dt, lab_sn, packed, wt, saved, dl, 0.0, 0, ii,
+                                                      cout)) if lazy else None)
         elif ctx.inmask is not None:
             ctx.inmask.offer(dx)
         if debug.TRACE is not None:
-            debug.trace("head_ce.bwd", dx, partial, dw, db)
-        return dx, (None if direct_w else dw), (None if (bias is None or direct_b) else db), None, None, None, None
-
-
-def head_ce(x, weight, bias, packed, labels, loss_weight=None, ignore_index=-100):
-    return HeadCEFn.apply(x, weight, bias, packed, labels, loss_weight, ignore_index)
+            debug.trace("head_ce.bwd", None if lazy else dx, partial, dw, db)
+        return dx, (None if direct_w else dw), (None if (bias is None or direct_b) else db), None, None, None, None, None
+
+
+def head_ce(x, weight, bias, packed, labels, loss_weight=None, ignore_index=-100, sole_consumer=False):
+    return HeadCEFn.apply(x, weight, bias, packed, labels, loss_weight, ignore_index, sole_consumer)
 
 
 def _heatmap_view(heatmaps: torch.Tensor, n: int, nh: int, spatial_shape):
diff --git a/torch-mednet_amd/mednet_hip/train.py b/torch-mednet_amd/mednet_hip/train.py
--- a/torch-mednet_amd/mednet_hip/train.py
+++ b/torch-mednet_amd/mednet_hip/train.py
@@ -335,12 +335,16 @@
         if (isinstance(m, _UNetCore) and not m.testing and (isinstance(self.loss, HL.CrossEntropyLoss) or (dice and not self.loss.skip_last_target))
                 and fc is not None and getattr(fc, "planar_output", False) and fc.kernel_size[0] == 1 and inputs.is_cuda
                 and not _call_is_hooked(m, fc)):
+            from .unet.model import _has_forward_hooks
             feats = m.forward_features(inputs)
+            last = m.decoders[-1] if len(m.decoders) else m.encoders[-1]
+            sole = not _has_forward_hooks(last)
             if dice and ops.head_dice_supported(feats, fc.in_channels, fc.out_channels, label_u8):
                 return ops.head_dice(feats, fc.weight, fc.bias, fc._packed(), label_u8, self.loss.weight, self.loss.epsilon,
-                                     self.loss.sigmoid_normalization, self.loss.ignore_index)
+                                     self.loss.sigmoid_normalization, self.loss.ignore_index, sole_consumer=sole)
             if not dice and ops.head_ce_supported(feats, fc.in_channels, fc.out_channels, label_u8):
-                return ops.head_ce(feats, fc.weight, fc.bias, fc._packed(), label_u8, self.loss.weight, self.loss.ignore_index)
+                return ops.head_ce(feats, fc.weight, fc.bias, fc._packed(), label_u8, self.loss.weight, self.loss.ignore_index,
+                                   sole_consumer=sole)
             outputs = fc(feats)
         else:
             outputs = m(inputs)
```

Measured after the change: 212.1 patches/s (median of 6 runs). About the same (+0.9%).
